# phcavelar/graph-odenet

Hardware: AMD Instinct MI355X
Metric: full-graph ODE-GCN forward+backward steps/sec at 64 RK4 evals (higher is better)
Workload: dtype f32; 1 GPU; RMAT scale-20 / 10000000 edges (+self loops, dedup) row-normalised, d=128, ODEGCN3 rk4(3/8) 16 steps = 64 f-evals fwd, adjoint bwd, Adam; one graph per GPU; nodes=1048576, nnz=10758918, nfeat=128, hidden=128, nclass=16, parallelism=dp1 (one graph per rank, 1 gradient all-reduce/step)

## Files before the change

### graph_odenet_amd/_lib.py

```python
import ctypes
import os

import torch

_HERE = os.path.dirname(os.path.abspath(__file__))
LIB_PATH = os.path.join(_HERE, "libgraphode.so")

GODE_MAX_TERMS = 8


class LinComb(ctypes.Structure):
    _fields_ = [("n", ctypes.c_int32),
                ("coef", ctypes.c_float * GODE_MAX_TERMS),
                ("ptr", ctypes.c_void_p * GODE_MAX_TERMS)]


class SpmmEpilogue(ctypes.Structure):
    _fields_ = [("bias", ctypes.c_void_p), ("relu", ctypes.c_int32), ("alpha", ctypes.c_float),
                ("pre", LinComb), ("cot", LinComb), ("Y2", ctypes.c_void_p), ("Y2_colsum", ctypes.c_void_p),
                ("cot_out", ctypes.c_void_p), ("cot_out_coef", ctypes.c_float * GODE_MAX_TERMS)]


class Graph(ctypes.Structure):
    _fields_ = [("rowptr", ctypes.c_void_p), ("col", ctypes.c_void_p), ("val", ctypes.c_void_p),
                ("items", ctypes.c_void_p), ("n_items", ctypes.c_int64),
                ("long_rows", ctypes.c_void_p), ("n_long", ctypes.c_int64), ("partial", ctypes.c_void_p),
                ("n_rows", ctypes.c_int64), ("nnz", ctypes.c_int64)]


class GcnOdeFunc(ctypes.Structure):
    _fields_ = [("A", Graph), ("AT", Graph), ("n", ctypes.c_int64), ("d", ctypes.c_int64),
                ("groups", ctypes.c_int32), ("eps", ctypes.c_float),
                ("W", ctypes.c_void_p), ("b", ctypes.c_void_p), ("gamma", ctypes.c_void_p), ("beta", ctypes.c_void_p)]


class GatProj(ctypes.Structure):
    _fields_ = [("ps", ctypes.c_void_p), ("ld_s", ctypes.c_int64), ("pt", ctypes.c_void_p), ("ld_t", ctypes.c_int64),
                ("as_", ctypes.c_void_p), ("at", ctypes.c_void_p), ("ld_a", ctypes.c_int64)]


class Rk4Workspace(ctypes.Structure):
    _fields_ = [("S", ctypes.c_void_p), ("dZ", ctypes.c_void_p), ("dS", ctypes.c_void_p), ("S2", ctypes.c_void_p),
                ("ky", ctypes.c_void_p * 4), ("ka", ctypes.c_void_p * 4), ("ktheta", ctypes.c_void_p * 4),
                ("wpart", ctypes.c_void_p), ("gpart", ctypes.c_void_p), ("bpart", ctypes.c_void_p),
                ("colsum_scratch", ctypes.c_void_p), ("X", ctypes.c_void_p * 2), ("small_part", ctypes.c_void_p),
                ("y2_colsum", ctypes.c_void_p)]


class ReduceSeg(ctypes.Structure):
    _fields_ = [("out", ctypes.c_void_p), ("part", ctypes.c_void_p), ("n_part", ctypes.c_int64), ("ld", ctypes.c_int64),
                ("col0", ctypes.c_int64), ("col_stride", ctypes.c_int64), ("len", ctypes.c_int64),
                ("w_row0", ctypes.c_void_p), ("time_len", ctypes.c_int64)]


class GatOdeFunc(ctypes.Structure):
    _fields_ = [("mt", Graph), ("ms_inc", Graph), ("mt_inc", Graph), ("src", ctypes.c_void_p), ("tgt", ctypes.c_void_p),
                ("n_edges", ctypes.c_int64), ("n", ctypes.c_int64), ("d", ctypes.c_int64), ("groups", ctypes.c_int32),
                ("eps_gn", ctypes.c_float), ("eps", ctypes.c_float), ("Wsrc", ctypes.c_void_p), ("Wtgt", ctypes.c_void_p),
                ("Wlog", ctypes.c_void_p), ("bf", ctypes.c_void_p), ("bw", ctypes.c_void_p), ("gamma", ctypes.c_void_p),
                ("beta", ctypes.c_void_p), ("heads", ctypes.c_int32), ("Wpacked", ctypes.c_void_p)]


class GatWorkspace(ctypes.Structure):
    _fields_ = [(k, ctypes.c_void_p) for k in ("X", "Ps", "Pt", "A2", "a", "amax", "wgt", "den", "logits_scratch", "dz", "da",
                                               "dPs", "dPt", "dA2", "pair", "gp", "bp")] + \
               [("wp", ctypes.c_void_p * 3), ("maxpath_scratch", ctypes.c_void_p), ("colsum_scratch", ctypes.c_void_p),
                ("zeros", ctypes.c_void_p), ("heads_scratch", ctypes.c_void_p), ("colsum_scratch2", ctypes.c_void_p),
                ("small_part", ctypes.c_void_p)]


GODE_ADAM_MAX_TENSORS = 64


class AdamArgs(ctypes.Structure):
    _fields_ = [("param", ctypes.c_void_p * GODE_ADAM_MAX_TENSORS), ("grad", ctypes.c_void_p * GODE_ADAM_MAX_TENSORS),
                ("exp_avg", ctypes.c_void_p * GODE_ADAM_MAX_TENSORS), ("exp_avg_sq", ctypes.c_void_p * GODE_ADAM_MAX_TENSORS),
                ("len", ctypes.c_int64 * GODE_ADAM_MAX_TENSORS)]


c_i64 = ctypes.c_int64
c_p = ctypes.c_void_p
c_f = ctypes.c_float
c_i = ctypes.c_int

SIGNATURES = {
    "gode_abi_version": (c_i, []),
    "gode_error_string": (ctypes.c_char_p, [c_i]),
    "gode_set_option": (c_i, [ctypes.c_char_p, c_i]),
    "gode_get_option": (c_i, [ctypes.c_char_p]),
    "gode_spmm_csr_f32": (c_i, [c_p, c_p, c_p, c_p, c_i64, c_p, c_i64, c_p, c_p, c_i64, c_p, c_i64,
                                c_i64, c_i64, ctypes.POINTER(SpmmEpilogue), c_p]),
    "gode_spmm_csr_save_f32": (c_i, [c_p, c_p, c_p, c_p, c_i64, c_p, c_i64, c_p, c_p, c_i64, c_p, c_i64,
                                     c_i64, c_i64, ctypes.POINTER(SpmmEpilogue), c_p, c_p]),
    "gode_masked_cot_parts": (c_i64, [c_i64, c_i64]),
    "gode_masked_cot_f32": (c_i, [ctypes.POINTER(LinComb), c_p, c_p, c_i64, c_i64, c_p, c_p]),
    "gode_lincomb_f32": (c_i, [c_p, ctypes.POINTER(LinComb), c_i64, c_p]),
    "gode_lincomb_multi_f32": (c_i, [c_p, c_p, c_p, ctypes.c_int32, c_p]),
    "gode_rk_errnorm_multi_f32": (c_i, [c_p, c_p, c_p, c_p, c_p, ctypes.c_int32, c_f, c_f, c_p, c_p]),
    "gode_rk_errnorm_scratch_bytes": (c_i64, []),
    "gode_rk_errnorm_f32": (c_i, [c_p, c_p, c_p, ctypes.POINTER(LinComb), c_f, c_f, c_i64, c_p, c_p]),
    "gode_rk_scaled_sumsq_f32": (c_i, [c_p, ctypes.POINTER(LinComb), c_p, c_f, c_f, c_i64, c_p, c_p]),
    "gode_gn_time_gemm_f32": (c_i, [ctypes.POINTER(LinComb), c_i64, c_i64, ctypes.c_int32, c_f, c_p, c_p,
                                    c_p, c_i64, c_i, c_f, c_p, c_p]),
    "gode_gn_time_gemm_xout_f32": (c_i, [ctypes.POINTER(LinComb), c_i64, c_i64, ctypes.c_int32, c_f, c_p, c_p,
                                         c_p, c_i64, c_i, c_f, c_p, c_p, c_p]),
    "gode_gn_time_gemm_xout_aux_f32": (c_i, [ctypes.POINTER(LinComb), c_i64, c_i64, ctypes.c_int32, c_f, c_p, c_p,
                                             c_p, c_i64, c_i, c_f, c_p, c_p, c_p, c_p, c_p]),
    "gode_gn_time_gemm_pair_f32": (c_i, [ctypes.POINTER(LinComb), c_i64, c_i64, ctypes.c_int32, c_f, c_p, c_p, c_p, c_p,
                                         c_i, c_f, c_p, c_p, c_p, c_p]),
    "gode_gemm_bwd_parts": (c_i64, [c_i64]),
    "gode_gn_time_gemm_bwd_f32": (c_i, [ctypes.POINTER(LinComb), c_i64, c_i64, ctypes.c_int32, c_f, c_p,
                                        c_p, c_i64, c_i, c_p, c_f, ctypes.POINTER(LinComb), c_p, c_p, c_p, c_p]),
    "gode_bwd_wgrad_supported": (c_i, [c_i64, c_i64, c_i64, ctypes.c_int32]),
    "gode_bwd_wgrad_parts": (c_i64, [c_i64]),
    "gode_gn_time_gemm_bwd_wgrad_f32": (c_i, [ctypes.POINTER(LinComb), c_i64, c_i64, ctypes.c_int32, c_f, c_p, c_p, c_p, c_i64, c_i,
                                              c_p, c_f, ctypes.POINTER(LinComb), c_p, c_p, c_p, c_p, c_p]),
    "gode_group_norm_parts": (c_i64, [c_i64]),
    "gode_group_norm_f32_fwd": (c_i, [c_p, c_i64, c_i64, ctypes.c_int32, c_f, c_p, c_p, c_p, c_p]),
    "gode_group_norm_f32_bwd": (c_i, [c_p, c_i64, c_i64, ctypes.c_int32, c_f, c_p, c_p, c_p, c_p, c_p, c_p]),
    "gode_rect_gemm_f32": (c_i, [c_p, c_i64, c_i64, c_i64, c_p, c_i64, c_p, c_i64, c_p]),
    "gode_rect_gemm_nt_f32": (c_i, [c_p, c_i64, c_i64, c_i64, c_p, c_i64, c_p, c_i64, c_p]),
    "gode_rect_wgrad_parts": (c_i64, [c_i64]),
    "gode_rect_wgrad_f32": (c_i, [c_p, c_i64, c_i64, c_i64, c_p, c_i64, c_i64, c_p, c_p]),
    "gode_rect_wgrad_sum_f32": (c_i, [c_p, c_i64, c_i64, c_i64, c_p, c_i64, c_i64, c_p, c_p, c_p]),
    "gode_gemm_f32": (c_i, [c_i, c_i, c_i64, c_i64, c_i64, c_p, c_i64, c_p, c_i64, c_p, c_i64, c_p, c_i, c_p, c_i64, c_p]),
    "gode_gemm_splitk_parts": (c_i64, [c_i64, c_i64, c_i64]),
    "gode_gemm_splitk_f32": (c_i, [c_i, c_i, c_i64, c_i64, c_i64, c_p, c_i64, c_p, c_i64, c_p, c_p, c_p]),
    "gode_cut_pad": (c_i64, [c_i64]),
    "gode_cut_bf16x3_f32": (c_i, [c_p, c_i64, c_i64, c_i64, c_p, c_p]),
    "gode_pgemm_workspace_bytes": (c_i64, [c_i64, c_i64, c_i64]),
    "gode_pgemm_bf16x3": (c_i, [c_i, c_i, c_i64, c_i64, c_i64, c_p, c_p, c_p, c_i64, c_p, c_i, c_p, c_i64, c_i, c_p, c_p]),
    "gode_adam_chunk": (c_i64, []),
    "gode_adam_tick_f32": (c_i, [c_p, c_f, c_f, c_p]),
    "gode_adam_f32": (c_i, [ctypes.POINTER(AdamArgs), ctypes.c_int32, c_p, c_i64, c_p, c_f, c_f, c_f, c_f, c_f, c_p]),
    "gode_gat_small_supported": (c_i, [c_i64, c_i64, ctypes.c_int32, c_i64]),
    "gode_gat_small_parts": (c_i64, [c_i64, c_i64]),
    "gode_gat_small_part_len": (c_i64, [c_i64, c_i64]),
    "gode_gat_project_small_f32": (c_i, [ctypes.POINTER(LinComb), c_i64, c_i64, ctypes.c_int32, c_f, c_p, c_p, c_p, c_p, c_p,
                                         c_i64, c_p, c_f, c_p, c_p, c_p, c_p, c_p, c_p]),
    "gode_gat_small_pack_len": (c_i64, [c_i64, c_i64]),
    "gode_gat_small_pack_f32": (c_i, [c_p, c_p, c_p, c_i64, c_i64, c_p, c_p]),
    "gode_gat_dense_vjp_small_f32": (c_i, [ctypes.POINTER(LinComb), c_i64, c_i64, ctypes.c_int32, c_f, c_p, c_p, c_p, c_p, c_p,
                                           c_i64, c_p, c_p, c_p, c_f, ctypes.POINTER(LinComb), c_p, c_p, c_p, c_p, c_p, c_i64, c_p, c_p]),
    "gode_gat_maxpath_heads_part_f32": (c_i, [c_p, c_p, c_i64, c_i64, c_p, c_p, c_p]),
    "gode_gat_heads_block_cap": (c_i64, []),
    "gode_gat_small_finish_f32": (c_i, [c_p, c_i64, c_i64, c_i64, c_f, c_p, c_p, c_p]),
    "gode_gat_small_finish_step_f32": (c_i, [c_p, c_i64, c_i64, c_i64, ctypes.c_int32, c_p, c_p, c_p, c_p, c_p]),
    "gode_gcn_small_supported": (c_i, [c_i64, c_i64, ctypes.c_int32]),
    "gode_gcn_small_parts": (c_i64, [c_i64]),
    "gode_gcn_small_part_len": (c_i64, [c_i64]),
    "gode_gcn_feval_small_f32": (c_i, [ctypes.POINTER(GcnOdeFunc), ctypes.POINTER(LinComb), c_f, c_f, ctypes.POINTER(LinComb),
                                       ctypes.POINTER(LinComb), c_p, c_p, c_p]),
    "gode_gcn_feval_small_next_f32": (c_i, [ctypes.POINTER(GcnOdeFunc), ctypes.POINTER(LinComb), c_f, c_f, ctypes.POINTER(LinComb),
                                            ctypes.POINTER(LinComb), c_p, c_p, ctypes.POINTER(LinComb), c_p, c_p]),
    "gode_gcn_vjp_small_f32": (c_i, [ctypes.POINTER(GcnOdeFunc), ctypes.POINTER(LinComb), c_p, c_f, ctypes.POINTER(LinComb),
                                     c_p, c_p, c_p]),
    "gode_gcn_vjp_small_next_f32": (c_i, [ctypes.POINTER(GcnOdeFunc), ctypes.POINTER(LinComb), c_p, c_f, ctypes.POINTER(LinComb),
                                          c_p, c_p, ctypes.POINTER(LinComb), c_p, c_p, c_p]),
    "gode_gcn_feval_small_save_f32": (c_i, [ctypes.POINTER(GcnOdeFunc), ctypes.POINTER(LinComb), c_f, c_f,
                                            ctypes.POINTER(LinComb), c_p, c_p, c_p]),
    "gode_gcn_small_finish_f32": (c_i, [ctypes.POINTER(GcnOdeFunc), c_p, c_p, c_f, c_p]),
    "gode_gcn_small_finish_multi_f32": (c_i, [ctypes.POINTER(GcnOdeFunc), c_p, ctypes.c_int32, ctypes.POINTER(c_p), ctypes.POINTER(c_f), c_p]),
    "gode_gcn_small_finish4_f32": (c_i, [ctypes.POINTER(GcnOdeFunc), c_p, c_p, c_p, c_p, c_p]),
    "gode_wgrad_parts": (c_i64, [c_i64]),
    "gode_wgrad_f32": (c_i, [ctypes.POINTER(LinComb), c_i64, c_i64, ctypes.c_int32, c_f, c_p, c_p,
                             c_p, c_i64, c_i, c_p, c_p]),
    "gode_reduce_parts_f32": (c_i, [c_p, c_p, c_i64, c_i64, c_f, c_i, c_p]),
    "gode_reduce_parts2_f32": (c_i, [c_p, c_p, c_p, c_p, c_i64, c_i64, c_f, c_i, c_p]),
    "gode_reduce_segments_f32": (c_i, [ctypes.POINTER(ReduceSeg), ctypes.c_int32, c_f, c_p, c_p]),
    "gode_colsum_parts_f32": (c_i, [c_p, c_i64, c_i64, c_p, ctypes.POINTER(c_i64), c_p]),
    "gode_colsum_scratch_bytes": (c_i64, [c_i64, c_i64]),
    "gode_spmm_y2_colsum_rows": (c_i64, [c_i64, c_i64, c_i64]),
    "gode_colsum_f32": (c_i, [c_p, c_p, c_i64, c_i64, c_f, c_i, c_p, c_p]),
    "gode_gat_logits_scratch_bytes": (c_i64, [c_i64]),
    "gode_gat_logits_f32": (c_i, [ctypes.POINTER(GatProj), c_p, c_p, c_p, c_i64, c_p, c_p, c_p, c_p]),
    "gode_gat_agg_f32_fwd": (c_i, [ctypes.POINTER(Graph), c_p, c_p, ctypes.POINTER(GatProj), c_i64, c_p, c_p, c_p, c_f,
                                   c_p, c_p, c_p, c_p]),
    "gode_gat_agg_f32_bwd": (c_i, [ctypes.POINTER(Graph), c_p, c_p, ctypes.POINTER(GatProj), c_i64, c_p, c_p, c_p, c_p,
                                   c_p, ctypes.POINTER(LinComb), c_f, c_p, c_p, c_p, c_i64, c_p, c_i64,
                                   ctypes.POINTER(ctypes.c_int32), c_p]),
    "gode_gat_maxpath_scratch_bytes": (c_i64, [c_i64]),
    "gode_gat_maxpath_f32": (c_i, [c_p, c_p, c_p, c_i64, c_p, c_p, c_i64, c_p, c_p]),
    "gode_gat_heads_scratch_bytes": (c_i64, [c_i64, c_i64]),
    "gode_gat_logits_heads_f32": (c_i, [ctypes.POINTER(GatProj), c_p, c_p, c_p, c_i64, c_i64, c_p, c_p, c_p, c_p]),
    "gode_gat_maxpath_heads_f32": (c_i, [c_p, c_p, c_i64, c_i64, c_p, c_p, c_i64, c_p, c_p]),
    "gode_gat_heads_parts": (c_i64, [c_i64]),
    "gode_gat_logits_heads_raw_f32": (c_i, [ctypes.POINTER(GatProj), c_p, c_p, c_p, c_i64, c_i64, c_p, c_p, c_p]),
    "gode_gat_agg_heads_f32_fwd": (c_i, [ctypes.POINTER(Graph), c_p, c_p, ctypes.POINTER(GatProj), c_i64, c_p, c_p, c_p, c_i64,
                                         c_i64, c_f, c_p, c_p, c_p, c_p]),
    "gode_gat_maxpath_heads_raw_f32": (c_i, [c_p, c_p, c_i64, c_i64, c_p, c_p, c_i64, c_p, c_p]),
    "gode_gat_scatter_f32": (c_i, [c_p, c_p, c_p, c_p, c_p, c_p, c_i64, c_i64, c_p, c_i64, c_p, c_i64, c_p, c_p, c_i64,
                                   c_p]),
    "gode_time_row_fixup_f32": (c_i, [c_p, c_p, c_i64, c_f, c_p, c_i, c_p]),
    "gode_time_row_fixup3_f32": (c_i, [c_p, c_p, c_i64, c_p, c_p, c_i64, c_p, c_p, c_i64, c_f, c_p, c_p]),
    "gode_edge_matvec_f32_fwd": (c_i, [c_p, c_p, c_p, c_p, c_p, c_p, c_i64, c_i64, c_i64, c_p, c_i64, c_p]),
    "gode_edge_matvec_msg_f32": (c_i, [c_p, c_p, c_p, c_i64, c_i64, c_i64, c_p, c_p]),
    "gode_edge_matvec_f32_bwd": (c_i, [c_p, c_p, c_p, c_p, c_p, c_i64, c_p, c_i64, c_i64, c_i64, c_p, c_p, c_p]),
    "gode_edge_outer_sum_f32": (c_i, [c_p, c_p, c_p, ctypes.c_int32, ctypes.POINTER(c_p), ctypes.POINTER(c_p), c_i64, c_i64, c_i64, c_i64, c_p, c_p]),
    "gode_edge_ode_supported": (c_i, [c_i64]),
    "gode_edge_ode_feval_f32": (c_i, [c_p, c_p, c_p, c_p, c_p, c_p, c_i64, c_i64, c_p, ctypes.POINTER(LinComb), c_f, c_p, c_p]),
    "gode_edge_ode_vjp_f32": (c_i, [c_p, c_p, c_p, c_p, c_p, ctypes.POINTER(LinComb), c_f, c_p, c_i64, c_i64, c_i64, c_p, c_p,
                                    c_p, c_p]),
    "gode_edge_outer_sum_acc_f32": (c_i, [c_p, c_p, c_p, ctypes.c_int32, ctypes.POINTER(c_p), ctypes.POINTER(c_p),
                                          ctypes.POINTER(c_f), c_i64, c_i64, c_i, c_p, c_p]),
    "gode_segment_attention_f32_fwd": (c_i, [c_p, c_p, c_p, c_i64, c_p, c_i64, c_i64, c_p, c_p, c_p]),
    "gode_segment_attention_f32_bwd": (c_i, [c_p, c_p, c_p, c_i64, c_p, c_p, c_p, c_i64, c_i64, c_p, c_p, c_p]),
    "gode_assign_csr_supported": (c_i, [c_i64, c_i64]),
    "gode_dense_first_nonzero_f32": (c_i, [c_p, c_i64, c_i64, c_i64, c_p, c_p]),
    "gode_assign_csr_i32": (c_i, [c_p, c_i64, c_i64, c_p, c_p, c_p, c_p, c_p]),
    "gode_set2set_supported": (c_i, [c_i64]),
    "gode_set2set_f32_fwd": (c_i, [c_p, c_p, c_p, c_i64, c_p, c_p, c_p, c_i64, c_i64, c_i64, c_i64, c_p, c_p, c_p, c_p, c_p]),
    "gode_set2set_f32_bwd": (c_i, [c_p, c_p, c_p, c_i64, c_p, c_p, c_i64, c_i64, c_i64, c_i64, c_p, c_p, c_p, c_p, c_p, c_p,
                                   c_p, c_p]),
    "gode_gcn_ode_theta_len": (c_i64, [c_i64]),
    "gode_gcn_ode_rk4_forward": (c_i, [ctypes.POINTER(GcnOdeFunc), c_p, ctypes.POINTER(c_p), ctypes.POINTER(Rk4Workspace),
                                       c_f, c_f, ctypes.c_int32, c_p]),
    "gode_gcn_ode_rk4_adjoint": (c_i, [ctypes.POINTER(GcnOdeFunc), c_p, c_p, c_p, ctypes.POINTER(c_p), ctypes.POINTER(c_p),
                                       ctypes.POINTER(Rk4Workspace), c_f, c_f, ctypes.c_int32, c_p]),
    "gode_gcn_ode_rk4_forward_save": (c_i, [ctypes.POINTER(GcnOdeFunc), c_p, c_p, c_p, ctypes.POINTER(Rk4Workspace),
                                            c_f, c_f, ctypes.c_int32, ctypes.c_int32, ctypes.c_int32, c_p]),
    "gode_gcn_ode_rk4_backprop": (c_i, [ctypes.POINTER(GcnOdeFunc), c_p, c_p, c_p, ctypes.POINTER(c_p),
                                        ctypes.POINTER(Rk4Workspace), c_p, c_f, c_f, ctypes.c_int32, ctypes.c_int32,
                                        ctypes.c_int32, c_p]),
    "gode_gcn_ode_dopri5_step_forward": (c_i, [ctypes.POINTER(GcnOdeFunc), c_p, ctypes.POINTER(c_p), c_p,
                                               ctypes.POINTER(Rk4Workspace), ctypes.c_double, ctypes.c_double, c_f, c_f,
                                               c_p, c_p, c_p]),
    "gode_gcn_ode_dopri5_step_adjoint": (c_i, [ctypes.POINTER(GcnOdeFunc), c_p, c_p, c_p, ctypes.POINTER(c_p),
                                               ctypes.POINTER(c_p), ctypes.POINTER(c_p), c_p, c_p, c_p,
                                               ctypes.POINTER(Rk4Workspace), ctypes.c_double, ctypes.c_double, c_f, c_f,
                                               c_p, c_p, c_p]),
    "gode_gcn_ode_dopri5_step_backprop": (c_i, [ctypes.POINTER(GcnOdeFunc), c_p, ctypes.POINTER(c_p), c_p, c_p,
                                                ctypes.c_double, ctypes.POINTER(ctypes.c_double), ctypes.c_double,
                                                ctypes.c_double, ctypes.c_int32, ctypes.POINTER(c_p), c_p, c_p, c_p,
                                                ctypes.POINTER(c_p), ctypes.POINTER(Rk4Workspace), c_p, c_p]),
    "gode_gat_ode_theta_len": (c_i64, [c_i64]),
    "gode_gat_ode_theta_len_heads": (c_i64, [c_i64, c_i64]),
    "gode_gat_ode_dopri5_step_forward": (c_i, [ctypes.POINTER(GatOdeFunc), c_p, ctypes.POINTER(c_p), c_p,
                                               ctypes.POINTER(GatWorkspace), ctypes.c_double, ctypes.c_double, c_f, c_f,
                                               c_p, c_p, c_p]),
    "gode_gat_ode_dopri5_step_adjoint": (c_i, [ctypes.POINTER(GatOdeFunc), c_p, c_p, c_p, c_p, ctypes.POINTER(c_p),
                                               ctypes.POINTER(c_p), ctypes.POINTER(c_p), ctypes.POINTER(c_p), c_p, c_p, c_p,
                                               c_p, ctypes.POINTER(GatWorkspace), ctypes.c_double, ctypes.c_double, c_f,
                                               c_f, c_p, c_p, c_p]),
    "gode_lstm_cell_supported": (c_i, [c_i64, c_i64, c_i64]),
    "gode_lstm_cell_f32_fwd": (c_i, [c_p] * 7 + [c_i64] * 3 + [c_p] * 4),
    "gode_lstm_cell_f32_bwd": (c_i, [c_p] * 9 + [c_i64] * 3 + [c_p] * 8),
    "gode_gru_wgrad_parts": (c_i64, [c_i64]),
    "gode_gru_cell_f32_fwd": (c_i, [c_p, c_p, c_p, c_p, c_p, c_p, c_i64, c_i64, c_p, c_p, c_p]),
    "gode_gru_cell_f32_bwd": (c_i, [c_p, c_p, c_p, c_p, c_p, c_p, c_i64, c_i64, c_p, c_p, c_p, c_p, c_p, c_p, c_p, c_p, c_p,
                                    c_p]),
    "gode_gru_wreduce_f32": (c_i, [c_p, c_i64, c_i64, c_p, c_p, c_p, c_p, c_p]),
    "gode_prof_create": (c_p, [c_i]),
    "gode_prof_destroy": (None, [c_p]),
    "gode_prof_enable": (None, [c_p]),
    "gode_prof_reset": (None, [c_p]),
    "gode_prof_count": (c_i, [c_p]),
    "gode_prof_read": (c_i, [c_p, c_p, c_p, c_p, c_p, c_i]),
    "gode_prof_kinds": (c_i, [c_p, c_p, c_i]),
}

_lib = None


class GraphodeLibraryError(RuntimeError):
    pass


def load():
    global _lib
    if _lib is not None:
        return _lib
    if not os.path.exists(LIB_PATH):
        raise GraphodeLibraryError(
            "libgraphode.so not found at %s - build it with `python __graft_entry__.py` "
            "(or `make -C graph_odenet_amd/csrc`). There is no fallback path." % LIB_PATH)
    lib = ctypes.CDLL(LIB_PATH)
    for name, (res, args) in SIGNATURES.items():
        fn = getattr(lib, name)
        fn.restype = res
        fn.argtypes = args
    if lib.gode_abi_version() != 1:
        raise GraphodeLibraryError("libgraphode.so ABI version mismatch")
    _lib = lib
    return lib


def check(rc, what):
    if rc != 0:
        msg = load().gode_error_string(rc)
        raise RuntimeError("%s failed: %s (code %d)" % (what, msg.decode() if msg else "?", rc))


def lincomb(terms):
    lc = LinComb()
    terms = [(c, t) for (c, t) in terms if t is not None]
    if len(terms) > GODE_MAX_TERMS:
        raise ValueError("too many lincomb terms")
    lc.n = len(terms)
    for j, (c, t) in enumerate(terms):
        lc.coef[j] = float(c)
        lc.ptr[j] = t.data_ptr()
    return lc


_raw_stream = getattr(torch._C, "_cuda_getCurrentRawStream", None)


def current_stream_handle(device_index=None):
    if _raw_stream is not None:
        return _raw_stream(torch.cuda.current_device() if device_index is None else device_index)
    return torch.cuda.current_stream(device_index).cuda_stream


def stream_ptr():
    return ctypes.c_void_p(current_stream_handle())


def ptr(t):
    return ctypes.c_void_p(t.data_ptr()) if t is not None else None
```

### graph_odenet_amd/csrc/api.hip

```cpp
#include "common.h"

extern "C" int gode_abi_version(void) { return GODE_ABI_VERSION; }

extern "C" const char* gode_error_string(int code) {
    switch (code) {
        case 0: return "success";
        case GODE_E_NULLPTR: return "graphode: required pointer is NULL";
        case GODE_E_SHAPE: return "graphode: invalid shape / leading dimension";
        case GODE_E_ALIGN: return "graphode: operand not 16-byte aligned";
        case GODE_E_RANGE: return "graphode: argument out of range";
        case GODE_E_UNSUPPORTED: return "graphode: unsupported configuration";
        default: break;
    }
    if (code > 0) return hipGetErrorString((hipError_t)code);
    return "graphode: unknown error";
}

#include "options.h"
#include <cstdlib>
#include <cstring>

namespace {
int env_int(const char* name, int dflt) { const char* e = getenv(name); return e ? atoi(e) : dflt; }
int g_gemm_split = -1, g_overlap = -1, g_wgrad_split = -1, g_wgrad_split_small = 0, g_bwd_pc = -1, g_fwd_pc = -1, g_small_fused = -1, g_bwd_wgrad = -1, g_y2_colsum = -1, g_rk_close_once = -1;
}

int gode_opt_gemm_split() { if (g_gemm_split < 0) { const int v = env_int("GODE_GEMM_SPLIT", 2); g_gemm_split = (v == 1 || v == 2) ? v : 0; } return g_gemm_split; }
int gode_opt_wgrad_split() {
    if (g_wgrad_split < 0) { const int v = env_int("GODE_WGRAD_SPLIT", 8); g_wgrad_split = (v == 6 || v == 8) ? v : 0; }
    return g_wgrad_split;
}
int gode_opt_wgrad_split_small() { return g_wgrad_split_small; }
int gode_opt_bwd_pc() { if (g_bwd_pc < 0) g_bwd_pc = env_int("GODE_BWD_PC", 1) != 0; return g_bwd_pc; }
int gode_opt_fwd_pc() { if (g_fwd_pc < 0) g_fwd_pc = env_int("GODE_FWD_PC", 3) & 3; return g_fwd_pc; }
int gode_opt_small_fused() { if (g_small_fused < 0) g_small_fused = env_int("GODE_SMALL_FUSED", 1) != 0; return g_small_fused; }
int gode_opt_bwd_wgrad() { if (g_bwd_wgrad < 0) g_bwd_wgrad = env_int("GODE_BWD_WGRAD", 1) != 0; return g_bwd_wgrad; }
int gode_opt_y2_colsum() { if (g_y2_colsum < 0) g_y2_colsum = env_int("GODE_Y2_COLSUM", 1) != 0; return g_y2_colsum; }
int gode_opt_rk_close_once() { if (g_rk_close_once < 0) g_rk_close_once = env_int("GODE_RK_CLOSE_ONCE", 1) != 0; return g_rk_close_once; }
int gode_opt_overlap() { if (g_overlap < 0) g_overlap = env_int("GODE_OVERLAP", 1) != 0; return g_overlap; }

extern "C" int gode_set_option(const char* name, int value) {
    if (!name) return GODE_E_NULLPTR;
    if (!strcmp(name, "gemm_split")) { if (value < 0 || value > 2) return GODE_E_UNSUPPORTED; g_gemm_split = value; return 0; }
    if (!strcmp(name, "overlap")) { g_overlap = value != 0; return 0; }
    if (!strcmp(name, "wgrad_split_small")) { g_wgrad_split_small = value != 0; return 0; }
    if (!strcmp(name, "bwd_pc")) { g_bwd_pc = value != 0; return 0; }
    if (!strcmp(name, "small_fused")) { g_small_fused = value != 0; return 0; }
    if (!strcmp(name, "bwd_wgrad")) { g_bwd_wgrad = value != 0; return 0; }
    if (!strcmp(name, "y2_colsum")) { g_y2_colsum = value != 0; return 0; }
    if (!strcmp(name, "rk_close_once")) { g_rk_close_once = value != 0; return 0; }
    if (!strcmp(name, "fwd_pc")) { if (value < 0 || value > 3) return GODE_E_UNSUPPORTED; g_fwd_pc = value; return 0; }
    if (!strcmp(name, "wgrad_split")) { if (value != 0 && value != 6 && value != 8) return GODE_E_UNSUPPORTED; g_wgrad_split = value; return 0; }
    return GODE_E_UNSUPPORTED;
}
extern "C" int gode_get_option(const char* name) {
    if (!name) return GODE_E_NULLPTR;
    if (!strcmp(name, "gemm_split")) return gode_opt_gemm_split();
    if (!strcmp(name, "overlap")) return gode_opt_overlap();
    if (!strcmp(name, "wgrad_split")) return gode_opt_wgrad_split();
    if (!strcmp(name, "wgrad_split_small")) return gode_opt_wgrad_split_small();
    if (!strcmp(name, "bwd_pc")) return gode_opt_bwd_pc();
    if (!strcmp(name, "small_fused")) return gode_opt_small_fused();
    if (!strcmp(name, "bwd_wgrad")) return gode_opt_bwd_wgrad();
    if (!strcmp(name, "y2_colsum")) return gode_opt_y2_colsum();
    if (!strcmp(name, "rk_close_once")) return gode_opt_rk_close_once();
    if (!strcmp(name, "fwd_pc")) return gode_opt_fwd_pc();
    return GODE_E_UNSUPPORTED;
}
```

### graph_odenet_amd/csrc/ode_driver.hip

```cpp
#include <map>
#include <mutex>
#include <utility>
#include "rk_driver.h"
#include "options.h"

namespace {

int spmm(const gode_graph_t& g, const float* X, float* Y, int64_t d, const gode_spmm_epilogue_t* ep, void* s) {
    return gode_spmm_csr_f32(g.rowptr, g.col, g.val, g.items, g.n_items, g.long_rows, g.n_long, g.partial,
                             X, d, Y, d, g.n_rows, d, ep, s);
}
gode_spmm_epilogue_t relu_bias_epilogue(const gode_gcn_odefunc_t* f) {
    gode_spmm_epilogue_t ep = {};
    ep.bias = f->b; ep.relu = 1; ep.alpha = 1.f;
    return ep;
}

__global__ void theta_fixup_kernel(float* ktheta, const float* W, float t, int d, int64_t off_at) {
    __shared__ float sm[4];
    float s = 0.f;
    for (int c = threadIdx.x; c < d; c += blockDim.x) s += ktheta[c] * W[c];
    s = wave_sum(s);
    if ((threadIdx.x & 63) == 0) sm[threadIdx.x >> 6] = s;
    __syncthreads();
    if (threadIdx.x == 0) ktheta[off_at] = sm[0] + sm[1] + sm[2] + sm[3];
    __syncthreads();
    for (int c = threadIdx.x; c < d; c += blockDim.x) ktheta[c] *= t;
}

int close_bias(const gode_gcn_odefunc_t* f, const gode_rk4_workspace_t* ws, float* kt, const float* src, int64_t rows,
               void* stream) {
    return gode_colsum_f32(kt + (f->d + 1) * f->d, src, rows, f->d, 1.f, 0, ws->colsum_scratch, stream);
}
int close_weight(const gode_gcn_odefunc_t* f, const gode_rk4_workspace_t* ws, float* kt, int64_t parts, float ts,
                 void* stream) {
    const int64_t d = f->d;
    GODE_TRY(gode_reduce_parts_f32(kt, ws->wpart, parts, (d + 1) * d, 1.f, 0, stream));
    hipLaunchKernelGGL(theta_fixup_kernel, dim3(1), dim3(256), 0, (hipStream_t)stream, kt, f->W, ts, (int)d,
                       gode_gcn_ode_theta_len(d) - 1);
    GODE_LAUNCH_CHECK();
    return 0;
}
int close_affine(const gode_gcn_odefunc_t* f, const gode_rk4_workspace_t* ws, float* kt, void* stream) {
    const int64_t d = f->d;
    float* kg = kt + (d + 1) * d + d;
    if (f->groups <= 0) return gode_zero_f32(kg, 2 * d, stream);
    return gode_reduce_parts2_f32(kg, ws->gpart, kg + d, ws->bpart, gode_gemm_bwd_parts(f->n), d, 1.f, 0, stream);
}

int stage_finish_merged(const gode_gcn_odefunc_t* f, const gode_rk4_workspace_t* ws, float* kt, float ts, void* stream) {
    const int64_t n = f->n, d = f->d, nW = (d + 1) * d, P = gode_gcn_ode_theta_len(d);
    int64_t cparts = 0;
    GODE_TRY(gode_colsum_parts_f32(ws->dZ, n, d, (float*)ws->colsum_scratch, &cparts, stream));
    const int64_t gp = gode_gemm_bwd_parts(n);
    gode_reduce_seg_t sg[4] = {};
    sg[0] = {kt, ws->wpart, gode_wgrad_parts(n), nW, 0, 1, nW, f->W, d};
    sg[1] = {kt + nW, (const float*)ws->colsum_scratch, cparts, d, 0, 1, d, nullptr, 0};
    sg[2] = {kt + nW + d, ws->gpart, gp, d, 0, 1, d, nullptr, 0};
    sg[3] = {kt + nW + 2 * d, ws->bpart, gp, d, 0, 1, d, nullptr, 0};
    GODE_TRY(gode_reduce_segments_f32(sg, f->groups > 0 ? 4 : 2, ts, kt + (P - 1), stream));
    if (f->groups <= 0) GODE_TRY(gode_zero_f32(kt + nW + d, 2 * d, stream));
    return 0;
}

bool fused_small(const gode_gcn_odefunc_t* f) {
    return gode_opt_small_fused() && gode_gcn_small_supported(f->n, f->d, f->groups);
}

bool close_once_route(const gode_gcn_odefunc_t* f) {
    return gode_opt_rk_close_once() && !fused_small(f) && f->n > kMergedFinishMaxRows && f->d == 128;
}

int gf_last_stage(const gode_gcn_odefunc_t* f, const gode_lincomb_t& xin, const gode_lincomb_t& pre, float t, float* S,
                  float* x_out, float* p_out, bool* formed, void* stream) {
    *formed = false;
    bool distinct = p_out != S && p_out != x_out;
    for (int j = 0; j < xin.n; ++j) distinct = distinct && p_out != xin.ptr[j];
    if (distinct && xin.n == pre.n) {
        const int rc = gode_gn_time_gemm_xout_aux_f32(&xin, f->n, f->d, f->groups, f->eps, f->gamma, f->beta, f->W, f->d, 1, t, S,
                                                      x_out, pre.coef, p_out, stream);
        if (rc != GODE_E_UNSUPPORTED) { *formed = rc == 0; return rc; }
    }
    return gode_gn_time_gemm_xout_f32(&xin, f->n, f->d, f->groups, f->eps, f->gamma, f->beta, f->W, f->d, 1, t, S, x_out, stream);
}

struct StepClose { gode_lincomb_t pre; float alpha; bool once; };

int feval_large(const gode_gcn_odefunc_t* f, const gode_lincomb_t& xin, float t, float* S, float* out,
                const StepClose* close, float* k_save, void* stream) {
    const int64_t d = f->d;
    bool p_formed = false;
    if (close && close->once) {
        GODE_TRY(gf_last_stage(f, xin, close->pre, t, S, nullptr, out, &p_formed, stream));
    } else {
        GODE_TRY(gode_gn_time_gemm_f32(&xin, f->n, d, f->groups, f->eps, f->gamma, f->beta, f->W, d, 1, t, S, stream));
    }
    gode_spmm_epilogue_t ep = relu_bias_epilogue(f);
    if (close) { ep.pre = p_formed ? one_term(out) : close->pre; ep.alpha = close->alpha; }
    if (!k_save) return spmm(f->A, S, out, d, &ep, stream);
    const gode_graph_t& g = f->A;
    return gode_spmm_csr_save_f32(g.rowptr, g.col, g.val, g.items, g.n_items, g.long_rows, g.n_long, g.partial,
                                  S, d, out, d, g.n_rows, d, &ep, k_save, stream);
}

int rk4_forward_step(const gode_gcn_odefunc_t* f, const gode_rk4_workspace_t* ws, const float* y, float* const* k,
                     float* ynext, bool keep_k4, double t, double h, bool fused, bool close_once, void* stream) {
    for (int s = 0; s < 4; ++s) {
        const gode_lincomb_t xin = stage_terms(y, k, s, h);
        const float ts = (float)(t + C38[s] * h);
        if (s < 3) {
            if (fused) GODE_TRY(gode_gcn_feval_small_f32(f, &xin, ts, 1.f, nullptr, nullptr, nullptr, k[s], stream));
            else GODE_TRY(feval_large(f, xin, ts, ws->S, k[s], nullptr, nullptr, stream));
            continue;
        }
        const StepClose close = {combine_terms(y, k, h), (float)(h * B38[3]), close_once};
        if (!fused) GODE_TRY(feval_large(f, xin, ts, ws->S, ynext, &close, keep_k4 ? k[3] : nullptr, stream));
        else if (keep_k4) GODE_TRY(gode_gcn_feval_small_save_f32(f, &xin, ts, close.alpha, &close.pre, ynext, k[3], stream));
        else GODE_TRY(gode_gcn_feval_small_f32(f, &xin, ts, close.alpha, &close.pre, nullptr, nullptr, ynext, stream));
    }
    return 0;
}

}

extern "C" int64_t gode_gcn_ode_theta_len(int64_t d) { return (d + 1) * d + 3 * d + 1; }

extern "C" int gode_gcn_ode_rk4_forward(const gode_gcn_odefunc_t* f, float* y, float** result,
                                        const gode_rk4_workspace_t* ws, float t0, float t1, int32_t n_steps,
                                        void* stream)
{
    if (!f || !y || !ws || !result) return GODE_E_NULLPTR;
    if (n_steps <= 0 || f->n <= 0 || f->d <= 0) return GODE_E_SHAPE;
    if (!ws->S || !ws->ky[0] || !ws->ky[1] || !ws->ky[2] || !ws->ky[3]) return GODE_E_NULLPTR;
    const double h = ((double)t1 - (double)t0) / n_steps;
    float* cur = y;
    float* k[4] = {ws->ky[0], ws->ky[1], ws->ky[2], ws->ky[3]};
    const bool fused = fused_small(f);
    const bool close_once = close_once_route(f);
    for (int i = 0; i < n_steps; ++i) {
        GODE_TRY(rk4_forward_step(f, ws, cur, k, k[3], false, (double)t0 + i * h, h, fused, close_once, stream));
        float* tmp = cur; cur = k[3]; k[3] = tmp;
    }
    *result = cur;
    return 0;
}

namespace {

struct Overlap {
    hipStream_t side = nullptr;
    hipEvent_t sp = nullptr, gf = nullptr, spt = nullptr, wg = nullptr;
    bool ok = false;
};
Overlap* overlap_ctx(hipStream_t caller) {
    static std::mutex mu;
    static std::map<std::pair<int, hipStream_t>, Overlap*> ctxs;
    int dev = 0;
    if (hipGetDevice(&dev) != hipSuccess) return nullptr;
    std::lock_guard<std::mutex> lk(mu);
    auto key = std::make_pair(dev, caller);
    auto it = ctxs.find(key);
    if (it != ctxs.end()) return it->second;
    Overlap* c = new Overlap();
    if (hipStreamCreateWithFlags(&c->side, hipStreamNonBlocking) == hipSuccess) {
        bool ok = true;
        for (hipEvent_t* ev : {&c->sp, &c->gf, &c->spt, &c->wg})
            ok = ok && hipEventCreateWithFlags(ev, hipEventDisableTiming) == hipSuccess;
        c->ok = ok;
    }
    ctxs[key] = c;
    return c;
}

int rk4_adjoint_small(const gode_gcn_odefunc_t* f, const gode_rk4_workspace_t* ws, float* y, float* a, float* theta,
                      float** y_result, float** a_result, float t0, double h, int32_t n_steps, void* stream) {
    float* ycur = y; float* acur = a;
    float* ky[4] = {ws->ky[0], ws->ky[1], ws->ky[2], ws->ky[3]};
    float* ka[4] = {ws->ka[0], ws->ka[1], ws->ka[2], ws->ka[3]};
    const int64_t slot = gode_gcn_small_parts(f->n) * gode_gcn_small_part_len(f->d);
    const float hb3 = (float)(h * B38[3]);
    for (int i = 0; i < n_steps; ++i) {
        float stage_t[4];
        const gode_lincomb_t ypre = combine_terms(ycur, ky, h), apre = combine_terms(acur, ka, h);
        for (int s = 0; s < 4; ++s) {
            stage_t[s] = (float)((double)t0 + i * h + C38[s] * h);
            const gode_lincomb_t yin = stage_terms(ycur, ky, s, h);
            const gode_lincomb_t cot = negated(stage_terms(acur, ka, s, h));
            GODE_TRY(gode_gcn_feval_small_f32(f, &yin, stage_t[s], s == 3 ? hb3 : 1.f, s == 3 ? &ypre : nullptr,
                                              &cot, ws->dZ, ky[s], stream));
            GODE_TRY(gode_gcn_vjp_small_f32(f, &yin, ws->dZ, s == 3 ? hb3 : 1.f, s == 3 ? &apre : nullptr,
                                            ka[s], ws->small_part + s * slot, stream));
        }
        const float wb[4] = {(float)(h * B38[0]), (float)(h * B38[1]), (float)(h * B38[2]), hb3};
        GODE_TRY(gode_gcn_small_finish4_f32(f, ws->small_part, theta, wb, stage_t, stream));
        float* tmp = ycur; ycur = ky[3]; ky[3] = tmp;
        tmp = acur; acur = ka[3]; ka[3] = tmp;
    }
    *y_result = ycur;
    *a_result = acur;
    return 0;
}

}

extern "C" int gode_gcn_ode_rk4_adjoint(const gode_gcn_odefunc_t* f, float* y, float* a, float* theta,
                                        float** y_result, float** a_result,
                                        const gode_rk4_workspace_t* ws, float t0, float t1, int32_t n_steps,
                                        void* stream)
{
    if (!f || !y || !a || !theta || !ws || !y_result || !a_result) return GODE_E_NULLPTR;
    if (n_steps <= 0 || f->n <= 0 || f->d <= 0) return GODE_E_SHAPE;
    for (int s = 0; s < 4; ++s) if (!ws->ky[s] || !ws->ka[s] || !ws->ktheta[s]) return GODE_E_NULLPTR;
    if (!ws->S || !ws->dZ || !ws->dS || !ws->wpart || !ws->colsum_scratch) return GODE_E_NULLPTR;
    if (f->groups > 0 && (!ws->gpart || !ws->bpart)) return GODE_E_NULLPTR;
    const int64_t n = f->n, d = f->d;
    const double h = ((double)t1 - (double)t0) / n_steps;
    if (fused_small(f) && ws->small_part != nullptr)
        return rk4_adjoint_small(f, ws, y, a, theta, y_result, a_result, t0, h, n_steps, stream);
    hipStream_t hs = (hipStream_t)stream;
    const bool small = f->n <= kMergedFinishMaxRows;
    Overlap* ov = (!small && ws->S2 != nullptr && gode_opt_overlap()) ? overlap_ctx(hs) : nullptr;
    const bool two = ov != nullptr && ov->ok;
    void* side = two ? (void*)ov->side : stream;
    float* Sbuf[2] = {ws->S, two ? ws->S2 : ws->S};
    float* ycur = y; float* acur = a;
    float* ky[4] = {ws->ky[0], ws->ky[1], ws->ky[2], ws->ky[3]};
    float* ka[4] = {ws->ka[0], ws->ka[1], ws->ka[2], ws->ka[3]};
    const int64_t wparts = gode_wgrad_parts(n);
    const int total = 4 * n_steps;
    const bool bw = !small && gode_bwd_wgrad_supported(n, d, d, f->groups) && gode_bwd_wgrad_parts(n) <= wparts;
    const int64_t y2rows = (bw && ws->y2_colsum && gode_opt_y2_colsum())
        ? gode_spmm_y2_colsum_rows(f->A.items ? f->A.n_items : f->A.n_rows, f->A.items ? f->A.n_long : 0, d) : 0;

    const bool mat = ws->X[0] != nullptr && ws->X[1] != nullptr;
    auto x_out_of = [&](int g) -> float* { return (mat && (g % 4) >= 2) ? ws->X[g & 1] : nullptr; };
    auto stage_time = [&](int g) { return (float)((double)t0 + (g / 4) * h + C38[g % 4] * h); };

    const bool close_once = bw && close_once_route(f);
    bool py_formed = false;
    auto gf = [&](int g, void* st) -> int {
        const gode_lincomb_t yin = stage_terms(ycur, ky, g % 4, h);
        if (g % 4 == 3 && close_once)
            return gf_last_stage(f, yin, combine_terms(ycur, ky, h), stage_time(g), Sbuf[g & 1], x_out_of(g), ky[3], &py_formed, st);
        return gode_gn_time_gemm_xout_f32(&yin, n, d, f->groups, f->eps, f->gamma, f->beta, f->W, d, 1, stage_time(g),
                                          Sbuf[g & 1], x_out_of(g), st);
    };
    GODE_TRY(gf(0, stream));
    bool wg_pending = false;
    for (int g = 0; g < total; ++g) {
        const int s = g % 4;
        const float ts = stage_time(g);
        const gode_lincomb_t yin = x_out_of(g) ? one_term(x_out_of(g)) : stage_terms(ycur, ky, s, h);
        const gode_lincomb_t ain = stage_terms(acur, ka, s, h);
        gode_spmm_epilogue_t ep = relu_bias_epilogue(f);
        ep.cot = negated(ain);
        ep.Y2 = ws->dZ;
        if (y2rows > 0) ep.Y2_colsum = ws->y2_colsum;
        gode_lincomb_t apre; apre.n = 0;
        if (s == 3) {
            ep.pre = py_formed ? one_term(ky[3]) : combine_terms(ycur, ky, h);
            ep.alpha = (float)(h * B38[3]);
            apre = combine_terms(acur, ka, h);
            if (close_once && ain.n == apre.n) {
                ep.cot_out = ka[3];
                for (int j = 0; j < apre.n; ++j) ep.cot_out_coef[j] = apre.coef[j];
                apre = one_term(ka[3]);
            }
            py_formed = false;
        }
        if (two && g > 0) GODE_HIP(hipStreamWaitEvent(hs, ov->gf, 0));
        GODE_TRY(spmm(f->A, Sbuf[g & 1], ky[s], d, &ep, stream));
        if (s == 3) { float* tmp = ycur; ycur = ky[3]; ky[3] = tmp; }
        if (two && wg_pending) GODE_HIP(hipStreamWaitEvent(hs, ov->wg, 0));
        GODE_TRY(spmm(f->AT, ws->dZ, ws->dS, d, nullptr, stream));
        if (two) {
            GODE_HIP(hipEventRecord(ov->spt, hs));
            GODE_HIP(hipStreamWaitEvent(ov->side, ov->spt, 0));
        }
        float* kt = ws->ktheta[s];
        const float out_scale = s == 3 ? (float)(h * B38[3]) : 1.f;
        float* gpart = f->groups > 0 ? ws->gpart : nullptr;
        float* bpart = f->groups > 0 ? ws->bpart : nullptr;
        if (bw) {
            if (two) GODE_HIP(hipStreamWaitEvent(ov->side, ov->spt, 0));
            GODE_TRY(close_bias(f, ws, kt, y2rows > 0 ? ws->y2_colsum : ws->dZ, y2rows > 0 ? y2rows : n, side));
            GODE_TRY(gode_gn_time_gemm_bwd_wgrad_f32(&yin, n, d, f->groups, f->eps, f->gamma, f->beta, f->W, d, 1, ws->dS,
                                                     out_scale, s == 3 ? &apre : nullptr, ka[s], gpart, bpart, ws->wpart, stream));
            if (two) {
                GODE_HIP(hipEventRecord(ov->sp, hs));
                GODE_HIP(hipStreamWaitEvent(ov->side, ov->sp, 0));
            }
            GODE_TRY(close_weight(f, ws, kt, gode_bwd_wgrad_parts(n), ts, side));
            GODE_TRY(close_affine(f, ws, kt, side));
            if (two) { GODE_HIP(hipEventRecord(ov->wg, ov->side)); wg_pending = true; }
            if (g + 1 < total) {
                GODE_TRY(gf(g + 1, stream));
                if (two) GODE_HIP(hipEventRecord(ov->gf, hs));
            }
            if (two) { GODE_HIP(hipStreamWaitEvent(hs, ov->wg, 0)); wg_pending = false; }
        } else {
            GODE_TRY(gode_wgrad_f32(&yin, n, d, f->groups, f->eps, f->gamma, f->beta, ws->dS, d, 1, ws->wpart, side));
            if (!small) GODE_TRY(close_weight(f, ws, kt, wparts, ts, side));
            if (two) { GODE_HIP(hipEventRecord(ov->wg, ov->side)); wg_pending = true; }
            if (g + 1 < total) {
                GODE_TRY(gf(g + 1, side));
                if (two) GODE_HIP(hipEventRecord(ov->gf, ov->side));
            }
            GODE_TRY(gode_gn_time_gemm_bwd_f32(&yin, n, d, f->groups, f->eps, f->gamma, f->W, d, 1, ws->dS, out_scale,
                                               s == 3 ? &apre : nullptr, ka[s], gpart, bpart, stream));
            if (small) {
                GODE_TRY(stage_finish_merged(f, ws, kt, ts, stream));
            } else {
                GODE_TRY(close_bias(f, ws, kt, ws->dZ, n, stream));
                GODE_TRY(close_affine(f, ws, kt, stream));
            }
        }
        if (s == 3) {
            if (two) { GODE_HIP(hipStreamWaitEvent(hs, ov->wg, 0)); wg_pending = false; }
            gode_lincomb_t tc = one_term(theta);
            tc.n = 5;
            for (int q = 0; q < 4; ++q) { tc.coef[1 + q] = (float)(h * B38[q]); tc.ptr[1 + q] = ws->ktheta[q]; }
            GODE_TRY(gode_lincomb_f32(theta, &tc, gode_gcn_ode_theta_len(d), stream));
            float* tmp = acur; acur = ka[3]; ka[3] = tmp;
        }
    }
    if (two) {
        GODE_HIP(hipEventRecord(ov->gf, ov->side));
        GODE_HIP(hipStreamWaitEvent(hs, ov->gf, 0));
    }
    *y_result = ycur;
    *a_result = acur;
    return 0;
}

namespace {

int dp_eval_forward(const gode_gcn_odefunc_t* f, const gode_rk4_workspace_t* ws, const gode_lincomb_t* yin, float t,
                    float* k_out, const gode_lincomb_t* next, float* x_next, void* stream) {
    if (fused_small(f)) return gode_gcn_feval_small_next_f32(f, yin, t, 1.f, nullptr, nullptr, nullptr, k_out, next, x_next, stream);
    return feval_large(f, *yin, t, ws->S, k_out, nullptr, nullptr, stream);
}

int dp_eval_adjoint(const gode_gcn_odefunc_t* f, const gode_rk4_workspace_t* ws, gode_lincomb_t yin,
                    const gode_lincomb_t& ain, float t, float* ky, float* ka, float* kth, const gode_lincomb_t* next,
                    float* x_next, int part_slot, void* stream) {
    const int64_t n = f->n, d = f->d;
    if (fused_small(f) && ws->small_part) {
        const gode_lincomb_t cot = negated(ain);
        GODE_TRY(gode_gcn_feval_small_next_f32(f, &yin, t, 1.f, nullptr, &cot, ws->dZ, ky, next, x_next, stream));
        float* part = ws->small_part + (part_slot > 0 ? part_slot : 0) * gode_gcn_small_parts(n) * gode_gcn_small_part_len(d);
        GODE_TRY(gode_gcn_vjp_small_f32(f, &yin, ws->dZ, 1.f, nullptr, ka, part, stream));
        if (part_slot >= 0) return 0;
        return gode_gcn_small_finish_f32(f, part, kth, t, stream);
    }
    float* xo = (yin.n >= 3 && ws->X[0]) ? ws->X[0] : nullptr;
    GODE_TRY(gode_gn_time_gemm_xout_f32(&yin, n, d, f->groups, f->eps, f->gamma, f->beta, f->W, d, 1, t, ws->S, xo, stream));
    if (xo) yin = one_term(xo);
    gode_spmm_epilogue_t ep = relu_bias_epilogue(f);
    ep.cot = negated(ain);
    ep.Y2 = ws->dZ;
    GODE_TRY(spmm(f->A, ws->S, ky, d, &ep, stream));
    GODE_TRY(spmm(f->AT, ws->dZ, ws->dS, d, nullptr, stream));
    GODE_TRY(gode_gn_time_gemm_bwd_f32(&yin, n, d, f->groups, f->eps, f->gamma, f->W, d, 1, ws->dS, 1.f, nullptr, ka,
                                       f->groups > 0 ? ws->gpart : nullptr, f->groups > 0 ? ws->bpart : nullptr, stream));
    GODE_TRY(gode_wgrad_f32(&yin, n, d, f->groups, f->eps, f->gamma, f->beta, ws->dS, d, 1, ws->wpart, stream));
    if (n <= kMergedFinishMaxRows) return stage_finish_merged(f, ws, kth, t, stream);
    GODE_TRY(close_weight(f, ws, kth, gode_wgrad_parts(n), t, stream));
    GODE_TRY(close_bias(f, ws, kth, ws->dZ, n, stream));
    return close_affine(f, ws, kth, stream);
}

}

extern "C" int gode_gcn_ode_dopri5_step_forward(const gode_gcn_odefunc_t* f, const float* y, float* const* k, float* y1,
                                                const gode_rk4_workspace_t* ws, double t, double h, float rtol,
                                                float atol, double* sums, void* err_scratch, void* stream)
{
    if (!f || !y || !k || !y1 || !ws || !sums || !err_scratch) return GODE_E_NULLPTR;
    if (f->n <= 0 || f->d <= 0) return GODE_E_SHAPE;
    for (int s = 0; s < 7; ++s) if (!k[s]) return GODE_E_NULLPTR;
    if (!ws->S) return GODE_E_NULLPTR;
    const int64_t nd = f->n * f->d;
    const bool chain = fused_small(f) && ws->X[0] && ws->X[1];
    for (int s = 1; s < 7; ++s) {
        gode_lincomb_t yin = dp_terms(y, k, DPA[s], s, h, true);
        if (chain && s >= 2) yin = one_term(ws->X[s & 1]);
        gode_lincomb_t nxt; nxt.n = 0;
        if (chain && s < 6) nxt = dp_terms(y, k, DPA[s + 1], s + 1, h, true);
        GODE_TRY(dp_eval_forward(f, ws, &yin, (float)(t + DPC[s] * h), k[s], nxt.n > 0 ? &nxt : nullptr,
                                 nxt.n > 0 ? ws->X[(s + 1) & 1] : nullptr, stream));
    }
    gode_lincomb_t sol = dp_terms(y, k, DPB, 7, h, true);
    GODE_TRY(gode_lincomb_f32(y1, &sol, nd, stream));
    gode_lincomb_t err = dp_terms(nullptr, k, DPE, 7, h, false);
    return gode_rk_errnorm_f32(sums, y, y1, &err, rtol, atol, nd, err_scratch, stream);
}

extern "C" int gode_gcn_ode_dopri5_step_adjoint(const gode_gcn_odefunc_t* f, const float* y, const float* a,
                                                const float* theta, float* const* ky, float* const* ka,
                                                float* const* kth, float* y1, float* a1, float* theta1,
                                                const gode_rk4_workspace_t* ws, double t, double h, float rtol,
                                                float atol, double* sums , void* err_scratch, void* stream)
{
    if (!f || !y || !a || !theta || !ky || !ka || !kth || !y1 || !a1 || !theta1 || !ws || !sums || !err_scratch)
        return GODE_E_NULLPTR;
    if (f->n <= 0 || f->d <= 0) return GODE_E_SHAPE;
    for (int s = 0; s < 7; ++s) if (!ky[s] || !ka[s] || !kth[s]) return GODE_E_NULLPTR;
    if (!ws->S || !ws->dZ || !ws->dS || !ws->wpart || !ws->colsum_scratch) return GODE_E_NULLPTR;
    if (f->groups > 0 && (!ws->gpart || !ws->bpart)) return GODE_E_NULLPTR;
    const int64_t nd = f->n * f->d, P = gode_gcn_ode_theta_len(f->d);
    const bool fused = fused_small(f) && ws->small_part;
    const bool chain = fused && ws->X[0] && ws->X[1];
    for (int s = 1; s < 7; ++s) {
        gode_lincomb_t yin = dp_terms(y, ky, DPA[s], s, h, true);
        if (chain && s >= 2) yin = one_term(ws->X[s & 1]);
        gode_lincomb_t ain = dp_terms(a, ka, DPA[s], s, h, true);
        gode_lincomb_t nxt; nxt.n = 0;
        if (chain && s < 6) nxt = dp_terms(y, ky, DPA[s + 1], s + 1, h, true);
        GODE_TRY(dp_eval_adjoint(f, ws, yin, ain, (float)(t + DPC[s] * h), ky[s], ka[s], kth[s], nxt.n > 0 ? &nxt : nullptr,
                                 nxt.n > 0 ? ws->X[(s + 1) & 1] : nullptr, fused ? s - 1 : -1, stream));
    }
    if (fused) {
        float* kout[6]; float tsv[6];
        for (int s = 1; s < 7; ++s) { kout[s - 1] = kth[s]; tsv[s - 1] = (float)(t + DPC[s] * h); }
        GODE_TRY(gode_gcn_small_finish_multi_f32(f, ws->small_part, 6, kout, tsv, stream));
    }
    gode_lincomb_t sy = dp_terms(y, ky, DPB, 7, h, true), sa = dp_terms(a, ka, DPB, 7, h, true),
                   st = dp_terms(theta, kth, DPB, 7, h, true);
    {
        float* outs[3] = {y1, a1, theta1};
        const gode_lincomb_t sols[3] = {sy, sa, st};
        const int64_t lens[3] = {nd, nd, P};
        GODE_TRY(gode_lincomb_multi_f32(outs, sols, lens, 3, stream));
    }
    const gode_lincomb_t errs[4] = {dp_terms(nullptr, ky, DPE, 7, h, false), dp_terms(nullptr, ka, DPE, 7, h, false),
                                    dp_terms(nullptr, kth, DPE, 7, h, false, P - 1), dp_terms(nullptr, kth, DPE, 7, h, false)};
    const float* e0[4] = {y, a, theta + (P - 1), theta};
    const float* e1[4] = {y1, a1, theta1 + (P - 1), theta1};
    const int64_t ens[4] = {nd, nd, 1, P - 1};
    return gode_rk_errnorm_multi_f32(sums, e0, e1, errs, ens, 4, rtol, atol, err_scratch, stream);
}

namespace {

struct SweepRoute {
    bool small;
    bool bw;
    int64_t wparts, cparts;
    float* cot_colpart;
    float* gpart; float* bpart;
};
SweepRoute sweep_route(const gode_gcn_odefunc_t* f, const gode_rk4_workspace_t* ws, float* cot_colpart) {
    SweepRoute r;
    r.small = f->n <= kMergedFinishMaxRows;
    r.wparts = gode_wgrad_parts(f->n);
    r.bw = !r.small && gode_bwd_wgrad_supported(f->n, f->d, f->d, f->groups) && gode_bwd_wgrad_parts(f->n) <= r.wparts;
    r.cparts = (!r.small && cot_colpart) ? gode_masked_cot_parts(f->n, f->d) : 0;
    r.cot_colpart = cot_colpart;
    r.gpart = f->groups > 0 ? ws->gpart : nullptr;
    r.bpart = f->groups > 0 ? ws->bpart : nullptr;
    return r;
}

int sweep_stage(const gode_gcn_odefunc_t* f, const gode_rk4_workspace_t* ws, const SweepRoute& r, const gode_lincomb_t& cot,
                const float* k, const gode_lincomb_t& yin, const gode_lincomb_t* pre, float* ybar, float* kt, float ts,
                void* stream) {
    const int64_t n = f->n, d = f->d;
    GODE_TRY(gode_masked_cot_f32(&cot, k, ws->dZ, n, d, r.cparts > 0 ? r.cot_colpart : nullptr, stream));
    GODE_TRY(spmm(f->AT, ws->dZ, ws->dS, d, nullptr, stream));
    if (r.bw) {
        GODE_TRY(gode_gn_time_gemm_bwd_wgrad_f32(&yin, n, d, f->groups, f->eps, f->gamma, f->beta, f->W, d, 1, ws->dS,
                                                 1.f, pre, ybar, r.gpart, r.bpart, ws->wpart, stream));
    } else {
        GODE_TRY(gode_gn_time_gemm_bwd_f32(&yin, n, d, f->groups, f->eps, f->gamma, f->W, d, 1, ws->dS, 1.f,
                                           pre, ybar, r.gpart, r.bpart, stream));
        GODE_TRY(gode_wgrad_f32(&yin, n, d, f->groups, f->eps, f->gamma, f->beta, ws->dS, d, 1, ws->wpart, stream));
        if (r.small) return stage_finish_merged(f, ws, kt, ts, stream);
    }
    GODE_TRY(close_weight(f, ws, kt, r.bw ? gode_bwd_wgrad_parts(n) : r.wparts, ts, stream));
    GODE_TRY(close_bias(f, ws, kt, r.cparts > 0 ? r.cot_colpart : ws->dZ, r.cparts > 0 ? r.cparts : n, stream));
    return close_affine(f, ws, kt, stream);
}

int add_stage_parts(float* theta, float* const* kt, int count, int64_t len, void* stream) {
    gode_lincomb_t tc = one_term(theta);
    for (int q = 0; q < count; ++q) { tc.coef[tc.n] = 1.f; tc.ptr[tc.n] = kt[q]; ++tc.n; }
    return gode_lincomb_f32(theta, &tc, len, stream);
}

}

extern "C" int gode_gcn_ode_rk4_forward_save(const gode_gcn_odefunc_t* f, const float* y0, float* y_end, float* save,
                                             const gode_rk4_workspace_t* ws, float t0, float t1, int32_t n_steps,
                                             int32_t step_begin, int32_t step_end, void* stream)
{
    if (!f || !y0 || !y_end || !save || !ws) return GODE_E_NULLPTR;
    if (n_steps <= 0 || f->n <= 0 || f->d <= 0) return GODE_E_SHAPE;
    if (step_begin < 0 || step_end > n_steps || step_begin >= step_end) return GODE_E_SHAPE;
    if (!ws->S) return GODE_E_NULLPTR;
    const int64_t nd = f->n * f->d;
    const double h = ((double)t1 - (double)t0) / n_steps;
    const bool fused = fused_small(f);
    const bool close_once = close_once_route(f);
    if (y0 != save) {
        const gode_lincomb_t c = one_term(y0);
        GODE_TRY(gode_lincomb_f32(save, &c, nd, stream));
    }
    for (int i = step_begin; i < step_end; ++i) {
        float* rec = save + (int64_t)(i - step_begin) * 5 * nd;
        float* k[4] = {rec + nd, rec + 2 * nd, rec + 3 * nd, rec + 4 * nd};
        float* ynext = (i + 1 < step_end) ? rec + 5 * nd : y_end;
        GODE_TRY(rk4_forward_step(f, ws, rec, k, ynext, true, (double)t0 + i * h, h, fused, close_once, stream));
    }
    return 0;
}

extern "C" int gode_gcn_ode_rk4_backprop(const gode_gcn_odefunc_t* f, const float* save, float* a, float* theta,
                                         float** a_result, const gode_rk4_workspace_t* ws, float* cot_colpart,
                                         float t0, float t1, int32_t n_steps, int32_t step_begin, int32_t step_end,
                                         void* stream)
{
    if (!f || !save || !a || !theta || !a_result || !ws) return GODE_E_NULLPTR;
    if (n_steps <= 0 || f->n <= 0 || f->d <= 0) return GODE_E_SHAPE;
    if (step_begin < 0 || step_end > n_steps || step_begin >= step_end) return GODE_E_SHAPE;
    for (int s = 0; s < 4; ++s) if (!ws->ka[s] || !ws->ktheta[s]) return GODE_E_NULLPTR;
    if (!ws->dZ || !ws->dS || !ws->wpart || !ws->colsum_scratch) return GODE_E_NULLPTR;
    if (f->groups > 0 && (!ws->gpart || !ws->bpart)) return GODE_E_NULLPTR;
    const int64_t n = f->n, d = f->d, nd = n * d;
    const double h = ((double)t1 - (double)t0) / n_steps;
    float* acur = a;
    float* yb[4] = {ws->ka[0], ws->ka[1], ws->ka[2], ws->ka[3]};
    auto record = [&](int i) { return save + (int64_t)(i - step_begin) * 5 * nd; };
    const bool fused = fused_small(f) && ws->small_part != nullptr;
    if (fused) {
        const int64_t slot = gode_gcn_small_parts(n) * gode_gcn_small_part_len(d);
// ... 119 lines not shown
```

### graph_odenet_amd/csrc/options.h

```cpp
#pragma once
int gode_opt_gemm_split();
int gode_opt_overlap();
int gode_opt_wgrad_split();
int gode_opt_wgrad_split_small();
int gode_opt_bwd_pc();
int gode_opt_fwd_pc();
int gode_opt_small_fused();
int gode_opt_bwd_wgrad();
int gode_opt_y2_colsum();
int gode_opt_rk_close_once();
```

### graph_odenet_amd/csrc/prof.h

```cpp
#pragma once
#include <hip/hip_runtime.h>
#include <stdint.h>
int  gode_prof_begin(hipStream_t s, int64_t d, int64_t rows, int64_t extra, int kind = 0);
void gode_prof_end(hipStream_t s, int slot);
```

### graph_odenet_amd/csrc/prof.hip

```cpp
#include "common.h"
#include "prof.h"
#include <vector>

struct GodeProf {
    int capacity;
    int count;
    std::vector<hipEvent_t> ev;
    std::vector<int64_t> d, rows, extra;
    std::vector<int32_t> kind;
};

static GodeProf* volatile g_prof = nullptr;

extern "C" void* gode_prof_create(int capacity) {
    if (capacity <= 0) return nullptr;
    GodeProf* p = new GodeProf();
    p->capacity = capacity; p->count = 0;
    p->ev.resize(2 * (size_t)capacity); p->d.resize(capacity); p->rows.resize(capacity); p->extra.resize(capacity); p->kind.resize(capacity);
    for (auto& e : p->ev) if (hipEventCreate(&e) != hipSuccess) { delete p; return nullptr; }
    return p;
}
extern "C" void gode_prof_destroy(void* prof) {
    GodeProf* p = (GodeProf*)prof;
    if (!p) return;
    if (g_prof == p) g_prof = nullptr;
    for (auto& e : p->ev) (void)hipEventDestroy(e);
    delete p;
}
extern "C" void gode_prof_enable(void* prof) { g_prof = (GodeProf*)prof; }
extern "C" void gode_prof_reset(void* prof) { if (prof) ((GodeProf*)prof)->count = 0; }
extern "C" int gode_prof_count(void* prof) { return prof ? ((GodeProf*)prof)->count : 0; }

extern "C" int gode_prof_read(void* prof, float* ms, int64_t* d, int64_t* rows, int64_t* extra, int max_n) {
    GodeProf* p = (GodeProf*)prof;
    if (!p || !ms) return GODE_E_NULLPTR;
    int n = p->count < max_n ? p->count : max_n;
    for (int i = 0; i < n; ++i) {
        hipError_t e = hipEventSynchronize(p->ev[2 * i + 1]);
        if (e != hipSuccess) return (int)e;
        e = hipEventElapsedTime(&ms[i], p->ev[2 * i], p->ev[2 * i + 1]);
        if (e != hipSuccess) return (int)e;
        if (d) d[i] = p->d[i];
        if (rows) rows[i] = p->rows[i];
        if (extra) extra[i] = p->extra[i];
    }
    return n;
}

extern "C" int gode_prof_kinds(void* prof, int32_t* kinds, int max_n) {
    GodeProf* p = (GodeProf*)prof;
    if (!p || !kinds) return GODE_E_NULLPTR;
    const int n = p->count < max_n ? p->count : max_n;
    for (int i = 0; i < n; ++i) kinds[i] = p->kind[i];
    return n;
}

int gode_prof_begin(hipStream_t s, int64_t d, int64_t rows, int64_t extra, int kind) {
    GodeProf* p = g_prof;
    if (!p || p->count >= p->capacity) return -1;
    hipStreamCaptureStatus cs = hipStreamCaptureStatusNone;
    if (hipStreamIsCapturing(s, &cs) != hipSuccess || cs != hipStreamCaptureStatusNone) return -1;
    const int i = p->count;
    p->d[i] = d; p->rows[i] = rows; p->extra[i] = extra; p->kind[i] = kind;
    (void)hipEventRecord(p->ev[2 * i], s);
    return i;
}
void gode_prof_end(hipStream_t s, int slot) {
    GodeProf* p = g_prof;
    if (!p || slot < 0) return;
    (void)hipEventRecord(p->ev[2 * slot + 1], s);
    p->count = slot + 1;
}
```

### graph_odenet_amd/csrc/spmm.hip

```cpp
#include "common.h"
#include "prof.h"

namespace {

struct Epilogue {
    const float* bias;
    int relu;
    float alpha;
    LinComb pre;
    LinComb cot;
    float* Y2;
    float* colpart;
    int64_t colpart_row0;
    float* K;
    float* Y3;
    float c3[GODE_MAX_TERMS];
};

template <int LPR, bool OUT3 = false>
__device__ __forceinline__ float4 epilogue_store4(const Epilogue& ep, float4 z, int row, int lane,
                                                  int64_t d, float* Y, int64_t ldy) {
    if (ep.bias) {
        const float4 b = *reinterpret_cast<const float4*>(ep.bias + lane * 4);
        z.x += b.x; z.y += b.y; z.z += b.z; z.w += b.w;
    }
    float4 y = z;
    if (ep.relu) { y.x = fmaxf(z.x, 0.f); y.y = fmaxf(z.y, 0.f); y.z = fmaxf(z.z, 0.f); y.w = fmaxf(z.w, 0.f); }
    if (ep.K) *reinterpret_cast<float4*>(ep.K + (int64_t)row * d + lane * 4) = y;
    if (ep.pre.n > 0) {
        const float4 p = lc_load4(ep.pre, (int64_t)row * d + lane * 4);
        y.x = fmaf(ep.alpha, y.x, p.x); y.y = fmaf(ep.alpha, y.y, p.y);
        y.z = fmaf(ep.alpha, y.z, p.z); y.w = fmaf(ep.alpha, y.w, p.w);
    } else if (ep.alpha != 1.f) {
        y.x *= ep.alpha; y.y *= ep.alpha; y.z *= ep.alpha; y.w *= ep.alpha;
    }
    *reinterpret_cast<float4*>(Y + (int64_t)row * ldy + lane * 4) = y;
    if (ep.Y2) {
        const int64_t o = (int64_t)row * d + lane * 4;
        float4 g;
        if (OUT3) {
            float4 g3;
            lc_load4_pair(ep.cot, ep.c3, o, g, g3);
            *reinterpret_cast<float4*>(ep.Y3 + o) = g3;
        } else {
            g = lc_load4(ep.cot, o);
        }
        g.x = z.x > 0.f ? g.x : 0.f; g.y = z.y > 0.f ? g.y : 0.f;
        g.z = z.z > 0.f ? g.z : 0.f; g.w = z.w > 0.f ? g.w : 0.f;
        *reinterpret_cast<float4*>(ep.Y2 + o) = g;
        return g;
    }
    return make_float4(0.f, 0.f, 0.f, 0.f);
}

template <int LPR>
__device__ __forceinline__ void block_colsum_store(const float4 g, float* __restrict__ colpart_row) {
    __shared__ float4 cs[256];
    cs[threadIdx.x] = g;
    __syncthreads();
    if (threadIdx.x < LPR) {
        float4 t = cs[threadIdx.x];
#pragma unroll
        for (int r = 1; r < 256 / LPR; ++r) {
            const float4 a = cs[r * LPR + threadIdx.x];
            t.x += a.x; t.y += a.y; t.z += a.z; t.w += a.w;
        }
        *reinterpret_cast<float4*>(colpart_row + 4 * threadIdx.x) = t;
    }
}

template <int LPR, bool OUT3 = false>
__global__ __launch_bounds__(256) void spmm_vec4_kernel(
    const int* __restrict__ rowptr, const int* __restrict__ col, const float* __restrict__ val,
    const int4* __restrict__ items, int n_items, float* __restrict__ partial,
    const float* __restrict__ X, int64_t ldx, float* __restrict__ Y, int64_t ldy, Epilogue ep)
{
    constexpr int U = 4;
    const int64_t tid = (int64_t)blockIdx.x * blockDim.x + threadIdx.x;
    const int gid = (int)(tid / LPR);
    const int lane = threadIdx.x & (LPR - 1);
    const bool active = gid < n_items;
    int row = 0, b = 0, e = 0, slot = -1;
    if (active) {
        if (items) { const int4 it = items[gid]; row = it.x; b = it.y; e = it.z; slot = it.w; }
        else { row = gid; b = rowptr[gid]; e = rowptr[gid + 1]; }
    }
    const int len = e - b;
    float4 acc = make_float4(0.f, 0.f, 0.f, 0.f);
    const float* Xl = X + lane * 4;

    for (int base = 0; __any(base < len); base += LPR) {
        int c = 0; float v = 0.f;
        if (base + lane < len) {
            c = col[b + base + lane];
            v = val ? val[b + base + lane] : 1.f;
        }
        const int cnt = len - base;
        for (int k = 0; k < LPR; k += U) {
            if (!__any(k < cnt)) break;
            int cc[U]; float vv[U]; float4 xv[U];
#pragma unroll
            for (int u = 0; u < U; ++u) {
                cc[u] = __shfl(c, k + u, LPR);
                vv[u] = __shfl(v, k + u, LPR);
            }
#pragma unroll
            for (int u = 0; u < U; ++u) {
                xv[u] = make_float4(0.f, 0.f, 0.f, 0.f);
                if (k + u < cnt && k + u < LPR)
                    xv[u] = *reinterpret_cast<const float4*>(Xl + (int64_t)cc[u] * ldx);
            }
#pragma unroll
            for (int u = 0; u < U; ++u) {
                acc.x = fmaf(vv[u], xv[u].x, acc.x); acc.y = fmaf(vv[u], xv[u].y, acc.y);
                acc.z = fmaf(vv[u], xv[u].z, acc.z); acc.w = fmaf(vv[u], xv[u].w, acc.w);
            }
        }
    }
    if (ep.colpart) {
        float4 g = make_float4(0.f, 0.f, 0.f, 0.f);
        if (active) {
            if (slot < 0) g = epilogue_store4<LPR, OUT3>(ep, acc, row, lane, (int64_t)LPR * 4, Y, ldy);
            else *reinterpret_cast<float4*>(partial + (int64_t)slot * (LPR * 4) + lane * 4) = acc;
        }
        block_colsum_store<LPR>(g, ep.colpart + (int64_t)blockIdx.x * (LPR * 4));
        return;
    }
    if (!active) return;
    if (slot < 0) epilogue_store4<LPR, OUT3>(ep, acc, row, lane, (int64_t)LPR * 4, Y, ldy);
    else *reinterpret_cast<float4*>(partial + (int64_t)slot * (LPR * 4) + lane * 4) = acc;
}

template <int LPR, bool OUT3 = false>
__global__ __launch_bounds__(256) void spmm_vec4_wave_kernel(
    const int* __restrict__ rowptr, const int* __restrict__ col, const float* __restrict__ val,
    const int4* __restrict__ items, int n_items, float* __restrict__ partial,
    const float* __restrict__ X, int64_t ldx, float* __restrict__ Y, int64_t ldy, Epilogue ep)
{
    const int gid = (int)(((int64_t)blockIdx.x * blockDim.x + threadIdx.x) >> 6);
    const int wl = threadIdx.x & 63;
    const int lane = wl & (LPR - 1), sub = wl / LPR;
    if (gid >= n_items) return;
    int row, b, e, slot = -1;
    if (items) { const int4 it = items[gid]; row = it.x; b = it.y; e = it.z; slot = it.w; }
    else { row = gid; b = rowptr[gid]; e = rowptr[gid + 1]; }
    const int len = e - b;
    float4 acc = make_float4(0.f, 0.f, 0.f, 0.f);
    const float* Xl = X + lane * 4;
    for (int base = sub * LPR; base - sub * LPR < len; base += 64) {
        int c = 0; float v = 0.f;
        if (base + lane < len) {
            c = col[b + base + lane];
            v = val ? val[b + base + lane] : 1.f;
        }
        const int cnt = len - base;
        constexpr int U = LPR < 4 ? LPR : 4;
        for (int k = 0; k < LPR; k += U) {
            if (!__any(k < cnt)) break;
            int cc[U]; float vv[U]; float4 xv[U];
#pragma unroll
            for (int u = 0; u < U; ++u) { cc[u] = __shfl(c, k + u, LPR); vv[u] = __shfl(v, k + u, LPR); }
#pragma unroll
            for (int u = 0; u < U; ++u) {
                xv[u] = make_float4(0.f, 0.f, 0.f, 0.f);
                if (k + u < cnt) xv[u] = *reinterpret_cast<const float4*>(Xl + (int64_t)cc[u] * ldx);
            }
#pragma unroll
            for (int u = 0; u < U; ++u) {
                acc.x = fmaf(vv[u], xv[u].x, acc.x); acc.y = fmaf(vv[u], xv[u].y, acc.y);
                acc.z = fmaf(vv[u], xv[u].z, acc.z); acc.w = fmaf(vv[u], xv[u].w, acc.w);
            }
        }
    }
#pragma unroll
    for (int off = LPR; off < 64; off <<= 1) {
        acc.x += __shfl_xor(acc.x, off, 64); acc.y += __shfl_xor(acc.y, off, 64);
        acc.z += __shfl_xor(acc.z, off, 64); acc.w += __shfl_xor(acc.w, off, 64);
    }
    if (sub != 0) return;
    if (slot < 0) epilogue_store4<LPR, OUT3>(ep, acc, row, lane, (int64_t)LPR * 4, Y, ldy);
    else *reinterpret_cast<float4*>(partial + (int64_t)slot * (LPR * 4) + lane * 4) = acc;
}

template <int LPR, bool OUT3 = false>
__global__ __launch_bounds__(256) void spmm_finish_vec4_kernel(
    const int4* __restrict__ long_rows, int n_long, const float* __restrict__ partial,
    float* __restrict__ Y, int64_t ldy, Epilogue ep)
{
    const int64_t tid = (int64_t)blockIdx.x * blockDim.x + threadIdx.x;
    const int gid = (int)(tid / LPR);
    const int lane = threadIdx.x & (LPR - 1);
    const bool active = gid < n_long;
    if (!active && !ep.colpart) return;
    const int4 lr = active ? long_rows[gid] : make_int4(0, 0, 0, 0);
    float4 acc = make_float4(0.f, 0.f, 0.f, 0.f);
    int s = lr.y;
    for (; s + 3 < lr.z; s += 4) {
        const float4 p0 = *reinterpret_cast<const float4*>(partial + (int64_t)s * (LPR * 4) + lane * 4);
        const float4 p1 = *reinterpret_cast<const float4*>(partial + (int64_t)(s + 1) * (LPR * 4) + lane * 4);
        const float4 p2 = *reinterpret_cast<const float4*>(partial + (int64_t)(s + 2) * (LPR * 4) + lane * 4);
        const float4 p3 = *reinterpret_cast<const float4*>(partial + (int64_t)(s + 3) * (LPR * 4) + lane * 4);
        acc.x += p0.x; acc.y += p0.y; acc.z += p0.z; acc.w += p0.w;
        acc.x += p1.x; acc.y += p1.y; acc.z += p1.z; acc.w += p1.w;
        acc.x += p2.x; acc.y += p2.y; acc.z += p2.z; acc.w += p2.w;
        acc.x += p3.x; acc.y += p3.y; acc.z += p3.z; acc.w += p3.w;
    }
    for (; s < lr.z; ++s) {
        const float4 p = *reinterpret_cast<const float4*>(partial + (int64_t)s * (LPR * 4) + lane * 4);
        acc.x += p.x; acc.y += p.y; acc.z += p.z; acc.w += p.w;
    }
    if (ep.colpart) {
        float4 g = make_float4(0.f, 0.f, 0.f, 0.f);
        if (active) g = epilogue_store4<LPR, OUT3>(ep, acc, lr.x, lane, (int64_t)LPR * 4, Y, ldy);
        block_colsum_store<LPR>(g, ep.colpart + (ep.colpart_row0 + blockIdx.x) * (LPR * 4));
        return;
    }
    epilogue_store4<LPR, OUT3>(ep, acc, lr.x, lane, (int64_t)LPR * 4, Y, ldy);
}

__device__ __forceinline__ void epilogue_store1(const Epilogue& ep, float z, int row, int c, int64_t d,
                                                float* Y, int64_t ldy) {
    if (ep.bias) z += ep.bias[c];
    float y = ep.relu ? fmaxf(z, 0.f) : z;
    if (ep.K) ep.K[(int64_t)row * d + c] = y;
    if (ep.pre.n > 0) y = fmaf(ep.alpha, y, lc_load1(ep.pre, (int64_t)row * d + c));
    else y *= ep.alpha;
    Y[(int64_t)row * ldy + c] = y;
    if (ep.Y2) {
        const int64_t o = (int64_t)row * d + c;
        const float g = lc_load1(ep.cot, o);
        ep.Y2[o] = z > 0.f ? g : 0.f;
        if (ep.Y3) {
            float g3 = 0.f;
#pragma unroll
            for (int j = 0; j < GODE_MAX_TERMS; ++j)
                if (j < ep.cot.n) g3 = fmaf(ep.c3[j], ep.cot.ptr[j][o], g3);
            ep.Y3[o] = g3;
        }
    }
}

__global__ __launch_bounds__(256) void spmm_generic_kernel(
    const int* __restrict__ rowptr, const int* __restrict__ col, const float* __restrict__ val,
    const int4* __restrict__ items, int n_items, float* __restrict__ partial,
    const float* __restrict__ X, int64_t ldx, float* __restrict__ Y, int64_t ldy, int d, int G, Epilogue ep)
{
    const int64_t tid = (int64_t)blockIdx.x * blockDim.x + threadIdx.x;
    const int gid = (int)(tid / G);
    const int lane = threadIdx.x & (G - 1);
    if (gid >= n_items) return;
    int row, b, e, slot = -1;
    if (items) { const int4 it = items[gid]; row = it.x; b = it.y; e = it.z; slot = it.w; }
    else { row = gid; b = rowptr[gid]; e = rowptr[gid + 1]; }
    for (int c = lane; c < d; c += G) {
        float acc = 0.f;
        int j = b;
        for (; j + 4 <= e; j += 4) {
            const int c0 = col[j], c1 = col[j + 1], c2 = col[j + 2], c3 = col[j + 3];
            const float x0 = X[(int64_t)c0 * ldx + c], x1 = X[(int64_t)c1 * ldx + c], x2 = X[(int64_t)c2 * ldx + c],
                        x3 = X[(int64_t)c3 * ldx + c];
            float v0 = 1.f, v1 = 1.f, v2 = 1.f, v3 = 1.f;
            if (val) { v0 = val[j]; v1 = val[j + 1]; v2 = val[j + 2]; v3 = val[j + 3]; }
            acc = fmaf(v0, x0, acc); acc = fmaf(v1, x1, acc); acc = fmaf(v2, x2, acc); acc = fmaf(v3, x3, acc);
        }
        for (; j < e; ++j) {
            const float v = val ? val[j] : 1.f;
            acc = fmaf(v, X[(int64_t)col[j] * ldx + c], acc);
        }
        if (slot < 0) epilogue_store1(ep, acc, row, c, d, Y, ldy);
        else partial[(int64_t)slot * d + c] = acc;
    }
}

__global__ __launch_bounds__(256) void spmv_wave_kernel(
    const int* __restrict__ rowptr, const int* __restrict__ col, const float* __restrict__ val,
    const int4* __restrict__ items, int n_items, float* __restrict__ partial,
    const float* __restrict__ X, int64_t ldx, float* __restrict__ Y, int64_t ldy, Epilogue ep)
{
    const int gid = (int)(((int64_t)blockIdx.x * blockDim.x + threadIdx.x) >> 6);
    const int lane = threadIdx.x & 63;
    if (gid >= n_items) return;
    int row, b, e, slot = -1;
    if (items) { const int4 it = items[gid]; row = it.x; b = it.y; e = it.z; slot = it.w; }
    else { row = gid; b = rowptr[gid]; e = rowptr[gid + 1]; }
    float acc = 0.f;
    for (int j = b + lane; j < e; j += 64) acc = fmaf(val ? val[j] : 1.f, X[(int64_t)col[j] * ldx], acc);
    acc = wave_sum(acc);
    if (lane == 0) {
        if (slot < 0) epilogue_store1(ep, acc, row, 0, 1, Y, ldy);
        else partial[slot] = acc;
    }
}

__global__ __launch_bounds__(256) void spmm_finish_generic_kernel(
    const int4* __restrict__ long_rows, int n_long, const float* __restrict__ partial,
    float* __restrict__ Y, int64_t ldy, int d, int G, Epilogue ep)
{
    const int64_t tid = (int64_t)blockIdx.x * blockDim.x + threadIdx.x;
    const int gid = (int)(tid / G);
    const int lane = threadIdx.x & (G - 1);
    if (gid >= n_long) return;
    const int4 lr = long_rows[gid];
    for (int c = lane; c < d; c += G) {
        float acc = 0.f;
        for (int s = lr.y; s < lr.z; ++s) acc += partial[(int64_t)s * d + c];
        epilogue_store1(ep, acc, lr.x, c, d, Y, ldy);
    }
}

template <int LPR, bool OUT3>
int launch_vec4(const int* rowptr, const int* col, const float* val, const int4* items, int n_items,
                const int4* long_rows, int n_long, float* partial, const float* X, int64_t ldx,
                float* Y, int64_t ldy, const Epilogue& ep, hipStream_t s) {
    if (LPR < 64 && n_items > 0 && n_items <= 65536) {
        if (ep.colpart) return GODE_E_UNSUPPORTED;
        const int64_t wb = ((int64_t)n_items * 64 + 255) / 256;
        const int slot = gode_prof_begin(s, (int64_t)LPR * 4, n_items, (int64_t)ep.pre.n + ep.cot.n + (ep.Y2 ? 1 : 0) + (ep.Y3 ? 1 : 0));
        hipLaunchKernelGGL((spmm_vec4_wave_kernel<LPR, OUT3>), dim3((unsigned)wb), dim3(256), 0, s,
                           rowptr, col, val, items, n_items, partial, X, ldx, Y, ldy, ep);
        gode_prof_end(s, slot);
        GODE_LAUNCH_CHECK();
        if (n_long > 0) {
            const int64_t b2 = ((int64_t)n_long * LPR + 255) / 256;
            hipLaunchKernelGGL((spmm_finish_vec4_kernel<LPR, OUT3>), dim3((unsigned)b2), dim3(256), 0, s,
                               long_rows, n_long, partial, Y, ldy, ep);
            GODE_LAUNCH_CHECK();
        }
        return 0;
    }
    const int64_t threads = (int64_t)n_items * LPR;
    const int64_t blocks = (threads + 255) / 256;
    if (blocks > 0) {
        const int slot = gode_prof_begin(s, (int64_t)LPR * 4, n_items, (int64_t)ep.pre.n + ep.cot.n + (ep.Y2 ? 1 : 0) + (ep.Y3 ? 1 : 0));
        hipLaunchKernelGGL((spmm_vec4_kernel<LPR, OUT3>), dim3((unsigned)blocks), dim3(256), 0, s,
                           rowptr, col, val, items, n_items, partial, X, ldx, Y, ldy, ep);
        gode_prof_end(s, slot);
        GODE_LAUNCH_CHECK();
    }
    if (n_long > 0) {
        const int64_t b2 = ((int64_t)n_long * LPR + 255) / 256;
        Epilogue ep2 = ep;
        ep2.colpart_row0 = blocks;
        hipLaunchKernelGGL((spmm_finish_vec4_kernel<LPR, OUT3>), dim3((unsigned)b2), dim3(256), 0, s,
                           long_rows, n_long, partial, Y, ldy, ep2);
        GODE_LAUNCH_CHECK();
    }
    return 0;
}

}

extern "C" int64_t gode_spmm_y2_colsum_rows(int64_t n_items, int64_t n_long, int64_t d)
{
    if (n_items <= 0 || n_long < 0 || d <= 0 || d % 4) return 0;
    const int64_t lpr = d / 4;
    if (lpr > 64 || (lpr & (lpr - 1))) return 0;
    if (lpr < 64 && n_items <= 65536) return 0;
    return (n_items * lpr + 255) / 256 + (n_long * lpr + 255) / 256;
}

namespace {

int spmm_csr_impl(const int32_t* rowptr, const int32_t* col, const float* val,
                  const int32_t* items, int64_t n_items,
                  const int32_t* long_rows, int64_t n_long, float* partial,
                  const float* X, int64_t ldx, float* Y, int64_t ldy,
                  int64_t n_rows, int64_t d,
                  const gode_spmm_epilogue_t* epi, float* K, void* stream)
{
    if (n_rows < 0 || d <= 0 || ldx < d || ldy < d) return GODE_E_SHAPE;
    if (n_rows == 0) return 0;
    if (!rowptr || !col || !X || !Y) return GODE_E_NULLPTR;
    if (n_rows > INT32_MAX || d > (1 << 20)) return GODE_E_RANGE;
    if (!items) { n_items = n_rows; n_long = 0; }
    if (n_items < 0 || n_items > INT32_MAX || n_long < 0 || n_long > INT32_MAX) return GODE_E_RANGE;
    if (n_long > 0 && (!long_rows || !partial)) return GODE_E_NULLPTR;
    if (n_items * 64 >= ((int64_t)1 << 32)) return GODE_E_RANGE;
    const float* bias = epi ? epi->bias : nullptr;
    float* Y2 = epi ? epi->Y2 : nullptr;
    const gode_lincomb_t* cot = (epi && Y2) ? &epi->cot : nullptr;
    const gode_lincomb_t* pre = (epi && epi->pre.n > 0) ? &epi->pre : nullptr;
    if (Y2) { int rc = check_lincomb(cot, true); if (rc) return rc; }
    if (pre) { int rc = check_lincomb(pre, true); if (rc) return rc; }
    hipStream_t s = (hipStream_t)stream;

    Epilogue ep;
    ep.bias = bias; ep.relu = epi ? epi->relu : 0; ep.alpha = epi ? epi->alpha : 1.f;
    ep.pre = make_lincomb(pre); ep.cot = make_lincomb(cot); ep.Y2 = Y2;
    ep.colpart = (epi && Y2) ? epi->Y2_colsum : nullptr; ep.colpart_row0 = 0;
    ep.K = K;
    ep.Y3 = (epi && Y2) ? epi->cot_out : nullptr;
    for (int j = 0; j < GODE_MAX_TERMS; ++j) ep.c3[j] = (ep.Y3 && j < ep.cot.n) ? epi->cot_out_coef[j] : 0.f;
    if (ep.Y3) {
        if (ep.Y3 == Y || ep.Y3 == Y2 || ep.Y3 == K) return GODE_E_RANGE;
        for (int j = 0; j < ep.cot.n; ++j) if (ep.Y3 == ep.cot.ptr[j]) return GODE_E_RANGE;
    }
    if (ep.colpart && ((((uintptr_t)ep.colpart) & 15) || gode_spmm_y2_colsum_rows(n_items, n_long, d) == 0)) return GODE_E_UNSUPPORTED;

    const bool al = !(((uintptr_t)X) & 15) && !(((uintptr_t)Y) & 15) && (ldx % 4 == 0) && (ldy % 4 == 0) &&
                    (!bias || !(((uintptr_t)bias) & 15)) && (!partial || !(((uintptr_t)partial) & 15)) &&
                    (!Y2 || (!(((uintptr_t)Y2) & 15) && lincomb_aligned16(cot))) && lincomb_aligned16(pre) &&
                    !(((uintptr_t)K) & 15) && !(((uintptr_t)ep.Y3) & 15);
    const int4* it4 = reinterpret_cast<const int4*>(items);
    const int4* lr4 = reinterpret_cast<const int4*>(long_rows);
    if (al && d % 4 == 0) {
        switch (d / 4) {
#define GODE_CASE(L) case L: return ep.Y3 ? launch_vec4<L, true>(rowptr, col, val, it4, (int)n_items, lr4, (int)n_long, partial, X, ldx, Y, ldy, ep, s) \
                                        : launch_vec4<L, false>(rowptr, col, val, it4, (int)n_items, lr4, (int)n_long, partial, X, ldx, Y, ldy, ep, s);
            GODE_CASE(1) GODE_CASE(2) GODE_CASE(4) GODE_CASE(8) GODE_CASE(16) GODE_CASE(32) GODE_CASE(64)
#undef GODE_CASE
            default: break;
        }
    }
    if (ep.colpart) return GODE_E_UNSUPPORTED;
    int G = 1; while (G < d && G < 64) G <<= 1;
    if (d == 1 && it4 != nullptr) {
        const int64_t blocks = ((int64_t)n_items * 64 + 255) / 256;
        const int slot = gode_prof_begin(s, 1, n_items, (int64_t)ep.pre.n + ep.cot.n + (ep.Y2 ? 1 : 0) + (ep.Y3 ? 1 : 0));
        hipLaunchKernelGGL(spmv_wave_kernel, dim3((unsigned)blocks), dim3(256), 0, s,
                           rowptr, col, val, it4, (int)n_items, partial, X, ldx, Y, ldy, ep);
        gode_prof_end(s, slot);
        GODE_LAUNCH_CHECK();
    } else {
        const int64_t blocks = ((int64_t)n_items * G + 255) / 256;
        hipLaunchKernelGGL(spmm_generic_kernel, dim3((unsigned)blocks), dim3(256), 0, s,
                           rowptr, col, val, it4, (int)n_items, partial, X, ldx, Y, ldy, (int)d, G, ep);
        GODE_LAUNCH_CHECK();
    }
    if (n_long > 0) {
        const int64_t b2 = ((int64_t)n_long * G + 255) / 256;
        hipLaunchKernelGGL(spmm_finish_generic_kernel, dim3((unsigned)b2), dim3(256), 0, s,
                           lr4, (int)n_long, partial, Y, ldy, (int)d, G, ep);
        GODE_LAUNCH_CHECK();
    }
    return 0;
}

}

extern "C" int gode_spmm_csr_f32(const int32_t* rowptr, const int32_t* col, const float* val,
                                 const int32_t* items, int64_t n_items,
                                 const int32_t* long_rows, int64_t n_long, float* partial,
                                 const float* X, int64_t ldx, float* Y, int64_t ldy,
                                 int64_t n_rows, int64_t d,
                                 const gode_spmm_epilogue_t* epi, void* stream)
{
    return spmm_csr_impl(rowptr, col, val, items, n_items, long_rows, n_long, partial, X, ldx, Y, ldy, n_rows, d, epi,
                         nullptr, stream);
}

extern "C" int gode_spmm_csr_save_f32(const int32_t* rowptr, const int32_t* col, const float* val,
                                      const int32_t* items, int64_t n_items,
                                      const int32_t* long_rows, int64_t n_long, float* partial,
                                      const float* X, int64_t ldx, float* Y, int64_t ldy,
                                      int64_t n_rows, int64_t d,
                                      const gode_spmm_epilogue_t* epi, float* K, void* stream)
{
    if (n_rows < 0 || d <= 0 || ldx < d || ldy < d) return GODE_E_SHAPE;
    if (n_rows > 0 && !K) return GODE_E_NULLPTR;
    return spmm_csr_impl(rowptr, col, val, items, n_items, long_rows, n_long, partial, X, ldx, Y, ldy, n_rows, d, epi,
                         K, stream);
}
```

### graph_odenet_amd/gcn_ode.py

```python
import ctypes

import torch

from . import _lib, ops
from .graph import as_graph
from .solver import Field


def _graph_struct(g, d):
    gs = _lib.Graph()
    gs.rowptr, gs.col = g.rowptr.data_ptr(), g.col.data_ptr()
    gs.val = g.val.data_ptr() if g.val is not None else None
    gs.items, gs.n_items = (g.items.data_ptr() if g.items is not None else None), g.n_items
    gs.long_rows = g.long_rows.data_ptr() if g.long_rows is not None else None
    gs.n_long = g.n_long
    part = g.partial(d)
    gs.partial = part.data_ptr() if part is not None else None
    gs.n_rows, gs.nnz = g.n_rows, g.nnz
    return gs


class _Shared:

    def __init__(self, graph, d, device):
        n = graph.n_rows
        self.S = torch.empty(n, d, dtype=torch.float32, device=device)
        self.dZ = None
        self.dS = None
        self.n = n
        self.d = d
        self.device = device
        self._ky = self._ka = self._kt = None
        self._parts = None
        self.y2_rows = 0
        if not getattr(graph, "is_partitioned", False) and hasattr(graph, "n_items"):
            self.y2_rows = _lib.load().gode_spmm_y2_colsum_rows(graph.n_items if graph.items is not None else n, graph.n_long, d)
        self._y2_colsum = None
        self._X2 = None

    @property
    def X2(self):
        if self._X2 is None:
            self._X2 = [torch.empty_like(self.S), torch.empty_like(self.S)]
        return self._X2

    def bwd(self):
        if self.dZ is None:
            self.dZ = torch.empty_like(self.S)
            self.dS = torch.empty_like(self.S)
        return self.dZ, self.dS

    def stage_buffers(self, adjoint):
        if self._ky is None:
            self._ky = [torch.empty_like(self.S) for _ in range(4)]
        if adjoint and self._ka is None:
            lib = _lib.load()
            P = lib.gode_gcn_ode_theta_len(self.d)
            self._ka = [torch.empty_like(self.S) for _ in range(4)]
            self._kt = [torch.empty(P, dtype=torch.float32, device=self.device) for _ in range(4)]
            nW = (self.d + 1) * self.d
            self._parts = (torch.empty(lib.gode_wgrad_parts(self.n) * nW, dtype=torch.float32, device=self.device),
                           torch.empty(lib.gode_gemm_bwd_parts(self.n) * self.d, dtype=torch.float32, device=self.device),
                           torch.empty(lib.gode_gemm_bwd_parts(self.n) * self.d, dtype=torch.float32, device=self.device),
                           torch.empty(max(lib.gode_colsum_scratch_bytes(self.n, self.d), 16), dtype=torch.uint8,
                                       device=self.device))
        return self._ky, self._ka, self._kt, self._parts

    def workspace_struct(self, adjoint, groups=0):
        ky, ka, kt, parts = self.stage_buffers(adjoint)
        ws = _lib.Rk4Workspace()
        ws.S = self.S.data_ptr()
        for i in range(4):
            ws.ky[i] = ky[i].data_ptr()
        if not adjoint and _lib.load().gode_gcn_small_supported(self.n, self.d, int(groups)):
            ws.X[0], ws.X[1] = self.X2[0].data_ptr(), self.X2[1].data_ptr()
        if adjoint:
            dZ, dS = self.bwd()
            ws.dZ, ws.dS = dZ.data_ptr(), dS.data_ptr()
            if getattr(self, "S2", None) is None:
                self.S2 = torch.empty_like(self.S)
            ws.S2 = self.S2.data_ptr()
            for i in range(4):
                ws.ka[i] = ka[i].data_ptr()
                ws.ktheta[i] = kt[i].data_ptr()
            ws.wpart, ws.gpart, ws.bpart, ws.colsum_scratch = (p.data_ptr() for p in parts)
            ws.X[0], ws.X[1] = self.X2[0].data_ptr(), self.X2[1].data_ptr()
            sp = self.small_part(groups)
            ws.small_part = sp.data_ptr() if sp is not None else None
            if self.y2_rows > 0:
                if self._y2_colsum is None:
                    self._y2_colsum = torch.empty(self.y2_rows, self.d, dtype=torch.float32, device=self.device)
                ws.y2_colsum = self._y2_colsum.data_ptr()
        return ws

    def cot_colpart(self):
        rows = _lib.load().gode_masked_cot_parts(self.n, self.d)
        if rows <= 0:
            return None
        if getattr(self, "_cot_colpart", None) is None:
            self._cot_colpart = torch.empty(rows, self.d, dtype=torch.float32, device=self.device)
        return self._cot_colpart

    def small_part(self, groups):
        lib = _lib.load()
        if not lib.gode_gcn_small_supported(self.n, self.d, int(groups)):
            return None
        if getattr(self, "_small_part", None) is None:
            self._small_part = torch.empty(7 * lib.gode_gcn_small_parts(self.n) * lib.gode_gcn_small_part_len(self.d),
                                           dtype=torch.float32, device=self.device)
        return self._small_part


def _func_struct(spec):
    fs = _lib.GcnOdeFunc()
    fs.A = _graph_struct(spec.graph, spec.d)
    fs.AT = _graph_struct(spec.graph.transpose(), spec.d)
    fs.n, fs.d, fs.groups, fs.eps = spec.graph.n_rows, spec.d, spec.groups, spec.eps
    fs.W, fs.b = spec.W.data_ptr(), spec.b.data_ptr()
    fs.gamma, fs.beta = spec.gamma.data_ptr(), spec.beta.data_ptr()
    return fs


def _by_ptr(ptr_value, candidates):
    for t in candidates:
        if t.data_ptr() == ptr_value:
            return t
    raise RuntimeError("rk4 driver returned an unknown buffer")


RELABEL_MIN_OPERAND_BYTES = 64 << 20
RELABEL_MIN_NNZ = 1 << 21
RELABEL_MIN_IMBALANCE = 2.0
NODE_ORDERS = ("auto", "given", "degree")


def gather_imbalance(graph, d, inverse=None):
    m = max(8, min(4096, (32 << 10) // (4 * d)))
    col = graph.col.to(torch.int64)
    rp = graph.rowptr.to(torch.int64)
    deg = rp[1:] - rp[:-1]
    rows = torch.arange(graph.n_rows, device=col.device)
    if inverse is not None:
        col, rows = inverse[col], inverse
    h_a = torch.bincount(col % m, minlength=m)
    h_t = torch.zeros(m, dtype=torch.int64, device=col.device).index_add_(0, rows % m, deg)
    h = torch.stack([h_a, h_t]).tolist()
    return max(max(hh) * m / max(sum(hh), 1) for hh in h)


def tuned_graph(graph, d, node_order="auto"):
    if node_order not in NODE_ORDERS:
        raise ValueError("node_order must be one of %s, got %r" % (NODE_ORDERS, node_order))
    cache = graph.__dict__.setdefault("_tuned", {})
    hit = cache.get((d, node_order))
    if hit is not None:
        return hit
    res = (graph, None, None)
    info = {"node_order": node_order, "renumbered": False}
    square = graph.n_rows == graph.n_cols and not getattr(graph, "is_partitioned", False)
    big = graph.n_rows * d * 4 >= RELABEL_MIN_OPERAND_BYTES and graph.nnz >= RELABEL_MIN_NNZ
    if square and node_order != "given" and (node_order == "degree" or big) \
            and not torch.cuda.is_current_stream_capturing():
        order = graph.degree_order()
        inverse = torch.empty_like(order)
        inverse[order] = torch.arange(graph.n_rows, device=graph.device)
        take = node_order == "degree"
        if not take:
            given, hubs = gather_imbalance(graph, d), gather_imbalance(graph, d, inverse)
            info.update(imbalance_given=round(given, 4), imbalance_hubs_first=round(hubs, 4))
            take = given >= RELABEL_MIN_IMBALANCE and hubs <= 0.5 * given
        if take:
            res = (graph.relabel(order), order, inverse)
            info["renumbered"] = True
    graph.__dict__.setdefault("_tuned_info", {})[(d, node_order)] = info
    cache[(d, node_order)] = res
    return res


class GcnOdeSpec:

    def __init__(self, graph, W, b, gamma, beta, groups, eps):
        self.graph, self.W, self.b, self.gamma, self.beta = graph, W, b, gamma, beta
        self.groups, self.eps = int(groups), float(eps)
        self.d = W.shape[1]
        if W.shape[0] != self.d + 1:
            raise ValueError("GcnOdeSpec: weight must be (d+1) x d, got %s" % (tuple(W.shape),))
        if graph.n_rows != graph.n_cols:
            raise ValueError("GcnOdeSpec: adjacency must be square")


def small_fused(spec):
    lib = _lib.load()
    return bool(lib.gode_get_option(b"small_fused") == 1 and not getattr(spec.graph, "is_partitioned", False)
                and lib.gode_gcn_small_supported(spec.graph.n_rows, spec.d, spec.groups))


def _feval_small(spec, t, terms, out, pre=None, alpha=1.0, cot=None, out2=None, next_terms=None, x_next=None):
    lib = _lib.load()
    fs = _func_struct(spec)
    lx = _lib.lincomb(terms)
    lp = _lib.lincomb(pre) if pre is not None else None
    lc = _lib.lincomb(cot) if cot is not None else None
    ln = _lib.lincomb(next_terms) if next_terms is not None else None
    _lib.check(lib.gode_gcn_feval_small_next_f32(ctypes.byref(fs), ctypes.byref(lx), float(t), float(alpha),
                                                 ctypes.byref(lp) if lp is not None else None,
                                                 ctypes.byref(lc) if lc is not None else None,
                                                 _lib.ptr(out2) if cot is not None else None, _lib.ptr(out),
                                                 ctypes.byref(ln) if ln is not None else None,
                                                 _lib.ptr(x_next) if ln is not None else None, _lib.stream_ptr()),
               "gode_gcn_feval_small_next_f32")


class _PackedParams:

    def _theta_len(self):
        return (self.s.d + 1) * self.s.d + 3 * self.s.d + 1

    def _packed_state(self, th, y, a):
        d = self.s.d
        nW = (d + 1) * d
        comps = [y, a, th[nW + 3 * d:], th[:nW].view(d + 1, d), th[nW:nW + d], th[nW + d:nW + 2 * d],
                 th[nW + 2 * d:nW + 3 * d]]
        comps[2]._gode_packed = th
        return comps

    def _in_params_order(self, comps):
        m = {"W": comps[3], "b": comps[4], "gamma": comps[5], "beta": comps[6]}
        return [m[k] for k in self.params_order]

    def packed_grads(self, device):
        return torch.zeros(self._theta_len(), dtype=torch.float32, device=device)

    def packed_param_grads(self, theta):
        return self._in_params_order(self._packed_state(theta, None, None))


class GcnOdeField(_PackedParams, Field):
    n_components = 1
    fused = True

    def __init__(self, spec, shared, params_order):
        self.s, self.w = spec, shared
        self.params_order = params_order
        self.token = ("gcn", id(spec.graph))

    def eval(self, t, terms, out):
        s, w = self.s, self.w
        if small_fused(s):
            return _feval_small(s, t, terms[0], out[0])
        ops.gn_time_gemm(terms[0], w.n, s.d, s.groups, s.eps, s.gamma, s.beta, s.W, True, t, out=w.S)
        ops.spmm(s.graph, w.S, bias=s.b, relu=True, out=out[0])

    def rk4_native(self, comps, t0, t1, n_steps):
        lib = _lib.load()
        s, w = self.s, self.w
        ky = w.stage_buffers(False)[0]
        fs, ws = _func_struct(s), w.workspace_struct(False, s.groups)
        res = ctypes.c_void_p()
        _lib.check(lib.gode_gcn_ode_rk4_forward(ctypes.byref(fs), _lib.ptr(comps[0]), ctypes.byref(res), ctypes.byref(ws),
                                                float(t0), float(t1), int(n_steps), _lib.stream_ptr()),
                   "gode_gcn_ode_rk4_forward")
        out = _by_ptr(res.value, [comps[0]] + ky)
        if out is not comps[0]:
            comps[0].copy_(out)
        return 4 * n_steps

    def rk4_forward_save(self, y0, y_end, save, t0, t1, n_steps, i0, i1):
        lib = _lib.load()
        s, w = self.s, self.w
        fs, ws = _func_struct(s), w.workspace_struct(False, s.groups)
        _lib.check(lib.gode_gcn_ode_rk4_forward_save(ctypes.byref(fs), _lib.ptr(y0), _lib.ptr(y_end), _lib.ptr(save),
                                                     ctypes.byref(ws), float(t0), float(t1), int(n_steps), int(i0), int(i1),
                                                     _lib.stream_ptr()), "gode_gcn_ode_rk4_forward_save")

    def rk4_backprop(self, save, a, theta, t0, t1, n_steps, i0, i1):
        lib = _lib.load()
        s, w = self.s, self.w
        ka = w.stage_buffers(True)[1]
        fs, ws = _func_struct(s), w.workspace_struct(True, s.groups)
        res = ctypes.c_void_p()
        _lib.check(lib.gode_gcn_ode_rk4_backprop(ctypes.byref(fs), _lib.ptr(save), _lib.ptr(a), _lib.ptr(theta),
                                                 ctypes.byref(res), ctypes.byref(ws), _lib.ptr(w.cot_colpart()),
                                                 float(t0), float(t1), int(n_steps), int(i0), int(i1), _lib.stream_ptr()),
                   "gode_gcn_ode_rk4_backprop")
        return _by_ptr(res.value, [a] + ka)

    def eval_combine(self, t, terms, pre, coef, out):
        s, w = self.s, self.w
        if small_fused(s):
            _feval_small(s, t, terms[0], out[0], pre=pre[0], alpha=coef)
            return (0,)
        ops.gn_time_gemm(terms[0], w.n, s.d, s.groups, s.eps, s.gamma, s.beta, s.W, True, t, out=w.S)
        ops.spmm(s.graph, w.S, bias=s.b, relu=True, out=out[0], pre_terms=pre[0], alpha=coef)
        return (0,)

    def dopri5_step_native(self, y, kk, y1, t, h, rtol, atol):
        lib = _lib.load()
        s, w = self.s, self.w
        fs, ws = _func_struct(s), w.workspace_struct(False, s.groups)
        kptr = (ctypes.c_void_p * 7)(*[kk[i][0].data_ptr() for i in range(7)])
        sums = torch.empty(1, dtype=torch.float64, device=y[0].device)
        sc = ops._scratch(y[0].device, lib.gode_rk_errnorm_scratch_bytes())
        _lib.check(lib.gode_gcn_ode_dopri5_step_forward(ctypes.byref(fs), _lib.ptr(y[0]), kptr, _lib.ptr(y1[0]),
                                                        ctypes.byref(ws), float(t), float(h), float(rtol), float(atol),
                                                        _lib.ptr(sums), _lib.ptr(sc), _lib.stream_ptr()),
                   "gode_gcn_ode_dopri5_step_forward")
        return sums

    def dopri5_backprop_work(self, like):
        lib = _lib.load()
        P = lib.gode_gcn_ode_theta_len(self.s.d)
        return {"ybar": [torch.empty_like(like) for _ in range(7)],
                "pairs": [(torch.empty_like(like), torch.empty_like(like)) for _ in range(2)],
                "ktheta": [torch.empty(P, dtype=torch.float32, device=like.device) for _ in range(7)]}

    def dopri5_step_backprop(self, y, k, g, kbar7, wy, wk, t, h, first, work, turn, theta):
        lib = _lib.load()
        s, w = self.s, self.w
        w.stage_buffers(True)
        fs, ws = _func_struct(s), w.workspace_struct(True, s.groups)
        arr = lambda ts: (ctypes.c_void_p * 7)(*[x.data_ptr() for x in ts])
        ybar_n, kbar1 = work["pairs"][turn]
# ... 218 lines not shown
```

### graph_odenet_amd/graph.py

```python
import weakref

import torch

DEFAULT_SPLIT = None


def auto_split(nnz):
    return 256 if nnz >= (1 << 20) else 1024


class CSRGraph:

    def __init__(self, rowptr, col, val, n_rows, n_cols, split=DEFAULT_SPLIT, records=True):
        self.rowptr = rowptr.to(torch.int32).contiguous()
        self.col = col.to(torch.int32).contiguous()
        self.val = None if val is None else val.to(torch.float32).contiguous()
        self.n_rows = int(n_rows)
        self.n_cols = int(n_cols)
        self.nnz = int(self.col.numel())
        self.device = self.col.device
        self.split = int(split) if split is not None else auto_split(self.nnz)
        if records:
            self._build_items()
        else:
            self.items, self.n_items, self.long_rows, self.n_long, self.n_slots = None, self.n_rows, None, 0, 0
        self._partial = {}
        self._T = None

    def _build_items(self):
        dev = self.device
        n = self.n_rows
        rp = self.rowptr.to(torch.int64)
        deg = rp[1:] - rp[:-1]
        L = self.split
        nseg = torch.clamp((deg + L - 1) // L, min=1)
        total = int(nseg.sum().item()) if n > 0 else 0
        rows = torch.repeat_interleave(torch.arange(n, device=dev, dtype=torch.int64), nseg)
        first = torch.cumsum(nseg, 0) - nseg
        k = torch.arange(total, device=dev, dtype=torch.int64) - first[rows]
        begin = rp[rows] + k * L
        end = torch.minimum(begin + L, rp[rows + 1])
        is_long = nseg[rows] > 1
        slot = torch.where(is_long, torch.cumsum(is_long.to(torch.int64), 0) - 1,
                           torch.full_like(rows, -1))
        self.n_slots = int(is_long.sum().item()) if total > 0 else 0
        items = torch.stack([rows, begin, end, slot], 1)
        order = torch.argsort(end - begin, descending=True, stable=True)
        self.items = items[order].to(torch.int32).contiguous()
        self.n_items = total
        long_rows = torch.nonzero(nseg > 1).flatten()
        self.n_long = int(long_rows.numel())
        if self.n_long:
            long_first = torch.cumsum(nseg[long_rows], 0) - nseg[long_rows]
            lr = torch.stack([long_rows, long_first, long_first + nseg[long_rows],
                              torch.zeros_like(long_rows)], 1)
            self.long_rows = lr.to(torch.int32).contiguous()
        else:
            self.long_rows = None

    def partial(self, d):
        if self.n_slots == 0:
            return None
        buf = self._partial.get(d)
        if buf is None:
            buf = torch.empty(self.n_slots * d, dtype=torch.float32, device=self.device)
            self._partial[d] = buf
        return buf

    def transpose(self):
        if self._T is None:
            rp = self.rowptr.to(torch.int64)
            rows = torch.repeat_interleave(torch.arange(self.n_rows, device=self.device), rp[1:] - rp[:-1])
            self._T = from_coo(self.col.to(torch.int64), rows, self.val, self.n_cols, self.n_rows,
                               split=self.split, coalesce=False)
            self._T._T = self
        return self._T

    def degree_order(self):
        rp = self.rowptr.to(torch.int64)
        deg = rp[1:] - rp[:-1]
        deg = deg + torch.bincount(self.col.to(torch.int64), minlength=self.n_cols)[: self.n_rows]
        return torch.argsort(deg, descending=True, stable=True)

    def relabel(self, order):
        if self.n_rows != self.n_cols:
            raise ValueError("relabel: square matrices only")
        order = order.to(torch.int64)
        new_id = torch.empty_like(order)
        new_id[order] = torch.arange(self.n_rows, device=self.device)

        def one(g):
            rp = g.rowptr.to(torch.int64)
            deg = (rp[1:] - rp[:-1])[order]
            rowptr = torch.zeros(g.n_rows + 1, dtype=torch.int64, device=g.device)
            rowptr[1:] = torch.cumsum(deg, 0)
            idx = torch.repeat_interleave(rp[order] - rowptr[:-1], deg) + torch.arange(g.nnz, device=g.device)
            return CSRGraph(rowptr, new_id[g.col.to(torch.int64)[idx]], None if g.val is None else g.val[idx],
                            g.n_rows, g.n_cols, split=g.split)
        out, out_t = one(self), one(self.transpose())
        out._T, out_t._T = out_t, out
        return out

    def to_dense(self):
        rp = self.rowptr.to(torch.int64)
        rows = torch.repeat_interleave(torch.arange(self.n_rows, device=self.device), rp[1:] - rp[:-1])
        out = torch.zeros(self.n_rows, self.n_cols, dtype=torch.float32, device=self.device)
        v = self.val if self.val is not None else torch.ones(self.nnz, device=self.device)
        out.index_put_((rows, self.col.to(torch.int64)), v, accumulate=True)
        return out

    def algorithmic_bytes(self, d):
        per = 4 + (4 if self.val is not None else 0) + 4 * d
        return self.nnz * per + (self.n_rows + 1) * 4 + self.n_rows * d * 4


def from_coo(rows, cols, vals, n_rows, n_cols, split=DEFAULT_SPLIT, coalesce=True):
    rows = rows.to(torch.int64)
    cols = cols.to(torch.int64)
    key = rows * n_cols + cols
    if coalesce:
        ukey, inv = torch.unique(key, sorted=True, return_inverse=True)
        if ukey.numel() != key.numel():
            if vals is None:
                vals = torch.ones(key.numel(), dtype=torch.float32, device=key.device)
            vals = torch.zeros(ukey.numel(), dtype=torch.float32, device=key.device).index_add_(0, inv, vals.float())
        elif vals is not None:
            vals = torch.empty_like(vals, dtype=torch.float32).index_copy_(0, inv, vals.float())
        key = ukey
    else:
        order = torch.argsort(key, stable=True)
        key = key[order]
        if vals is not None:
            vals = vals[order]
    r = key // n_cols
    c = key % n_cols
    counts = torch.bincount(r, minlength=n_rows)
    rowptr = torch.zeros(n_rows + 1, dtype=torch.int64, device=key.device)
    rowptr[1:] = torch.cumsum(counts, 0)
    return CSRGraph(rowptr, c, vals, n_rows, n_cols, split=split)


_cache = {}


def _evict(key):
    _cache.pop(key, None)


def as_graph(adj, split=DEFAULT_SPLIT):
    if isinstance(adj, CSRGraph) or getattr(adj, "is_partitioned", False):
        return adj
    if not torch.is_tensor(adj):
        raise TypeError("adjacency must be a torch tensor (sparse COO or dense) or CSRGraph")
    key = id(adj)
    hit = _cache.get(key)
    if hit is not None and hit[0]() is adj and hit[2] == adj._version:
        return hit[1]
    if adj.dim() != 2:
        raise ValueError("adjacency must be 2-D, got shape %s" % (tuple(adj.shape),))
    if adj.is_sparse:
        idx = adj._indices()
        vals = adj._values()
        g = from_coo(idx[0], idx[1], vals, adj.shape[0], adj.shape[1], split=split)
    elif adj.layout == torch.sparse_csr:
        g = CSRGraph(adj.crow_indices(), adj.col_indices(), adj.values(), adj.shape[0], adj.shape[1], split=split)
    else:
        nz = torch.nonzero(adj)
        g = from_coo(nz[:, 0], nz[:, 1], adj[nz[:, 0], nz[:, 1]], adj.shape[0], adj.shape[1], split=split)
    try:
        ref = weakref.ref(adj, lambda _r, k=key: _evict(k))
        _cache[key] = (ref, g, adj._version)
    except TypeError:
        pass
    return g


RECORDS_MIN_NNZ = 1 << 16


def csr_from_assignment(index, n_rows, vals=None, split=DEFAULT_SPLIT, records=None):
    idx = index.to(torch.int64)
    e = idx.numel()
    if records is None:
        records = e >= RECORDS_MIN_NNZ
    if idx.is_cuda and not records and n_rows > 0:
        from . import _lib
        lib = _lib.load()
        if lib.gode_assign_csr_supported(e, n_rows):
            idx = idx.contiguous()
            rowptr = torch.empty(n_rows + 1, dtype=torch.int32, device=idx.device)
            order = torch.empty(e, dtype=torch.int32, device=idx.device)
            v_in = None if vals is None else vals.to(torch.float32).contiguous()
            v = None if vals is None else torch.empty(e, dtype=torch.float32, device=idx.device)
            _lib.check(lib.gode_assign_csr_i32(_lib.ptr(idx), e, n_rows, _lib.ptr(rowptr), _lib.ptr(order), _lib.ptr(v_in),
                                               _lib.ptr(v), _lib.stream_ptr()), "gode_assign_csr_i32")
            return CSRGraph(rowptr, order, v, n_rows, e, split=split, records=False)
    order = torch.argsort(idx, stable=True)
    counts = torch.zeros(n_rows, dtype=torch.int64, device=idx.device).index_add_(
        0, idx, torch.ones(e, dtype=torch.int64, device=idx.device))
    rowptr = torch.zeros(n_rows + 1, dtype=torch.int64, device=idx.device)
    rowptr[1:] = torch.cumsum(counts, 0)
    v = None if vals is None else vals.to(torch.float32)[order]
    return CSRGraph(rowptr, order, v, n_rows, e, split=split, records=records)


def incidence_from_index(index, n_rows, split=DEFAULT_SPLIT):
    return csr_from_assignment(index, n_rows, None, split=split)
```

### graph_odenet_amd/ops.py

```python
import ctypes

import torch

from . import _lib
from ._lib import check, lincomb, ptr, stream_ptr


def _need(t, name, dtype=torch.float32):
    if t is None:
        return
    if not t.is_cuda:
        raise RuntimeError("graph_odenet_amd: %s must live on the GPU (got %s); there is no CPU path" % (name, t.device))
    if t.dtype != dtype:
        raise TypeError("graph_odenet_amd: %s must be %s, got %s" % (name, dtype, t.dtype))
    if not t.is_contiguous():
        raise ValueError("graph_odenet_amd: %s must be contiguous" % name)


def _need_terms(terms, name):
    n = None
    for c, t in terms:
        _need(t, name)
        if n is None:
            n = t.numel()
        elif t.numel() != n:
            raise ValueError("graph_odenet_amd: %s terms differ in size" % name)
    return n


def spmm(graph, X, bias=None, relu=False, out=None, cot_terms=None, out2=None, pre_terms=None, alpha=1.0, out2_colsum=None,
         cot_out=None, cot_out_coefs=None):
    lib = _lib.load()
    _need(X, "X")
    _need(bias, "bias")
    if getattr(graph, "is_partitioned", False):
        if X.dim() != 2 or X.shape[0] != graph.n_cols:
            raise ValueError("spmm: X has shape %s, this rank owns %d rows" % (tuple(X.shape), graph.n_cols))
        X, graph = graph.gather(X), graph.local
    if X.dim() != 2 or X.shape[0] != graph.n_cols:
        raise ValueError("spmm: X has shape %s, graph is %d x %d" % (tuple(X.shape), graph.n_rows, graph.n_cols))
    d = X.shape[1]
    if bias is not None and bias.numel() != d:
        raise ValueError("spmm: bias has %d elements, expected %d" % (bias.numel(), d))
    ldy = d
    if out is None:
        out = torch.empty(graph.n_rows, d, dtype=torch.float32, device=X.device)
    else:
        if tuple(out.shape) != (graph.n_rows, d):
            raise ValueError("spmm: out has wrong shape")
        if out.is_contiguous():
            _need(out, "out")
        else:
            if not out.is_cuda or out.dtype != torch.float32 or out.stride(1) != 1 or out.stride(0) < d:
                raise ValueError("spmm: out must be contiguous or a unit-stride column block of a row-major matrix")
            ldy = out.stride(0)
    ep = None
    if bias is not None or relu or cot_terms is not None or pre_terms is not None or alpha != 1.0:
        ep = _lib.SpmmEpilogue()
        ep.bias = bias.data_ptr() if bias is not None else None
        ep.relu = 1 if relu else 0
        ep.alpha = float(alpha)
        if pre_terms is not None:
            if _need_terms(pre_terms, "pre") != graph.n_rows * d:
                raise ValueError("spmm: pre terms have wrong size")
            ep.pre = lincomb(pre_terms)
        if cot_terms is not None:
            if _need_terms(cot_terms, "cot") != graph.n_rows * d:
                raise ValueError("spmm: cotangent terms have wrong size")
            ep.cot = lincomb(cot_terms)
            if out2 is None:
                out2 = torch.empty(graph.n_rows, d, dtype=torch.float32, device=X.device)
            _need(out2, "out2")
            ep.Y2 = out2.data_ptr()
            if out2_colsum is not None:
                _need(out2_colsum, "out2_colsum")
                if out2_colsum.numel() != spmm_y2_colsum_rows(graph, d) * d or out2_colsum.numel() == 0:
                    raise ValueError("spmm: out2_colsum must be spmm_y2_colsum_rows(graph, d) x d (and the shape must support it)")
                ep.Y2_colsum = out2_colsum.data_ptr()
            if cot_out is not None:
                _need(cot_out, "cot_out")
                if cot_out.numel() != graph.n_rows * d or cot_out_coefs is None or len(cot_out_coefs) != len(cot_terms):
                    raise ValueError("spmm: cot_out must be n_rows x d with one coefficient per cotangent term")
                ep.cot_out = cot_out.data_ptr()
                for j, cj in enumerate(cot_out_coefs):
                    ep.cot_out_coef[j] = float(cj)
        elif cot_out is not None:
            raise ValueError("spmm: cot_out needs cot_terms")
    partial = graph.partial(d)
    rc = lib.gode_spmm_csr_f32(ptr(graph.rowptr), ptr(graph.col), ptr(graph.val),
                               ptr(graph.items), graph.n_items,
                               ptr(graph.long_rows), graph.n_long, ptr(partial),
                               ptr(X), d, ptr(out), ldy, graph.n_rows, d,
                               ctypes.byref(ep) if ep is not None else None, stream_ptr())
    check(rc, "gode_spmm_csr_f32")
    return (out, out2) if cot_terms is not None else out


def spmm_y2_colsum_rows(graph, d):
    return int(_lib.load().gode_spmm_y2_colsum_rows(graph.n_items if graph.items is not None else graph.n_rows, graph.n_long, int(d)))


def lincomb_(out, terms):
    lib = _lib.load()
    _need(out, "out")
    if _need_terms(terms, "lincomb") != out.numel():
        raise ValueError("lincomb: size mismatch")
    lc = lincomb(terms)
    check(lib.gode_lincomb_f32(ptr(out), ctypes.byref(lc), out.numel(), stream_ptr()), "gode_lincomb_f32")
    return out


def lincomb_multi_(outs, terms_list):
    lib = _lib.load()
    k = len(outs)
    if k != len(terms_list) or not 1 <= k <= 4:
        raise ValueError("lincomb_multi: one term list per output, at most four")
    lcs = (_lib.LinComb * k)()
    ptrs = (ctypes.c_void_p * k)()
    ns = (ctypes.c_int64 * k)()
    for c, (out, terms) in enumerate(zip(outs, terms_list)):
        _need(out, "out")
        if _need_terms(terms, "lincomb") != out.numel():
            raise ValueError("lincomb_multi: size mismatch in component %d" % c)
        lcs[c] = lincomb(terms)
        ptrs[c] = out.data_ptr()
        ns[c] = out.numel()
    check(lib.gode_lincomb_multi_f32(ptrs, lcs, ns, k, stream_ptr()), "gode_lincomb_multi_f32")
    return outs


_red_scratch = {}
_retired = []


def _scratch(device, nbytes):
    key = (device, _lib.current_stream_handle(device.index if device.index is not None else torch.cuda.current_device()))
    buf = _red_scratch.get(key)
    if buf is None or buf.numel() < nbytes:
        if buf is not None:
            _retired.append(buf)
        buf = torch.empty(max(nbytes, 1 << 20), dtype=torch.uint8, device=device)
        _red_scratch[key] = buf
    return buf


def rk_error_sumsq(y0, y1, err_terms, rtol, atol, out=None):
    lib = _lib.load()
    _need(y0, "y0"); _need(y1, "y1")
    n = y0.numel()
    if _need_terms(err_terms, "err") != n or y1.numel() != n:
        raise ValueError("rk_error_sumsq: size mismatch")
    if out is None:
        out = torch.empty(1, dtype=torch.float64, device=y0.device)
    sc = _scratch(y0.device, lib.gode_rk_errnorm_scratch_bytes())
    lc = lincomb(err_terms)
    check(lib.gode_rk_errnorm_f32(ptr(out), ptr(y0), ptr(y1), ctypes.byref(lc), float(rtol), float(atol), n,
                                  ptr(sc), stream_ptr()), "gode_rk_errnorm_f32")
    return out


def rk_scaled_sumsq(terms, y, rtol, atol, out=None):
    lib = _lib.load()
    _need(y, "y")
    n = y.numel()
    if _need_terms(terms, "terms") != n:
        raise ValueError("rk_scaled_sumsq: size mismatch")
    if out is None:
        out = torch.empty(1, dtype=torch.float64, device=y.device)
    sc = _scratch(y.device, lib.gode_rk_errnorm_scratch_bytes())
    lc = lincomb(terms)
    check(lib.gode_rk_scaled_sumsq_f32(ptr(out), ctypes.byref(lc), ptr(y), float(rtol), float(atol), n,
                                       ptr(sc), stream_ptr()), "gode_rk_scaled_sumsq_f32")
    return out


def gn_time_gemm(x_terms, n_rows, d_in, groups, eps, gamma, beta, W, has_time, t, out=None, x_out=None, aux_coefs=None,
                 aux_out=None):
    lib = _lib.load()
    _need(W, "W"); _need(gamma, "gamma"); _need(beta, "beta")
    if _need_terms(x_terms, "x") != n_rows * d_in:
        raise ValueError("gn_time_gemm: x terms have wrong size")
    if W.dim() != 2 or W.shape[0] != d_in + (1 if has_time else 0):
        raise ValueError("gn_time_gemm: W has shape %s" % (tuple(W.shape),))
    d_out = W.shape[1]
    if out is None:
        out = torch.empty(n_rows, d_out, dtype=torch.float32, device=W.device)
    _need(out, "out")
    lc = lincomb(x_terms)
    if x_out is not None:
        _need(x_out, "x_out")
        if x_out.numel() != n_rows * d_in:
            raise ValueError("gn_time_gemm: x_out has wrong size")
    if aux_out is not None:
        _need(aux_out, "aux_out")
        if aux_out.numel() != n_rows * d_in or aux_coefs is None or len(aux_coefs) != len(x_terms):
            raise ValueError("gn_time_gemm: aux_out must be n_rows x d_in with one coefficient per term")
        ac = (ctypes.c_float * len(aux_coefs))(*[float(c) for c in aux_coefs])
        check(lib.gode_gn_time_gemm_xout_aux_f32(ctypes.byref(lc), n_rows, d_in, groups, float(eps), ptr(gamma), ptr(beta),
                                                 ptr(W), d_out, 1 if has_time else 0, float(t), ptr(out), ptr(x_out),
                                                 ac, ptr(aux_out), stream_ptr()), "gode_gn_time_gemm_xout_aux_f32")
        return out
    check(lib.gode_gn_time_gemm_xout_f32(ctypes.byref(lc), n_rows, d_in, groups, float(eps), ptr(gamma), ptr(beta),
                                         ptr(W), d_out, 1 if has_time else 0, float(t), ptr(out), ptr(x_out),
                                         stream_ptr()), "gode_gn_time_gemm_xout_f32")
    return out


def gn_time_gemm_pair(x_terms, n_rows, d, groups, eps, gamma, beta, Wa, Wb, has_time, t, out_a, out_b, x_out=None):
    lib = _lib.load()
    for tns, nm in ((Wa, "Wa"), (Wb, "Wb"), (gamma, "gamma"), (beta, "beta"), (out_a, "out_a"), (out_b, "out_b"), (x_out, "x_out")):
        _need(tns, nm)
    if _need_terms(x_terms, "x") != n_rows * d:
        raise ValueError("gn_time_gemm_pair: x terms have wrong size")
    k = d + (1 if has_time else 0)
    if tuple(Wa.shape) != (k, d) or tuple(Wb.shape) != (k, d) or out_a.numel() != n_rows * d or out_b.numel() != n_rows * d:
        raise ValueError("gn_time_gemm_pair: weights must be (%d, %d) and outputs n x d" % (k, d))
    lc = lincomb(x_terms)
    check(lib.gode_gn_time_gemm_pair_f32(ctypes.byref(lc), n_rows, d, groups, float(eps), ptr(gamma), ptr(beta), ptr(Wa), ptr(Wb),
                                         1 if has_time else 0, float(t), ptr(out_a), ptr(out_b), ptr(x_out), stream_ptr()),
          "gode_gn_time_gemm_pair_f32")


def gat_small_supported(n_rows, d, groups, heads=1):
    lib = _lib.load()
    return bool(lib.gode_get_option(b"small_fused")) and bool(lib.gode_gat_small_supported(n_rows, d, groups, heads))


def gat_small_part(n_rows, d, heads, device):
    lib = _lib.load()
    return torch.empty(lib.gode_gat_small_parts(n_rows, d), lib.gode_gat_small_part_len(d, heads), dtype=torch.float32, device=device)


def gat_small_pack(Wsrc, Wtgt, Wlog, heads, out=None):
    lib = _lib.load()
    _need(Wsrc, "Wsrc"); _need(Wtgt, "Wtgt"); _need(Wlog, "Wlog"); _need(out, "packed")
    d = Wsrc.shape[1]
    n = lib.gode_gat_small_pack_len(d, heads)
    if out is None:
        out = torch.empty(n, dtype=torch.float32, device=Wsrc.device)
    elif out.numel() != n:
        raise ValueError("gat_small_pack: packed buffer must hold %d floats" % n)
    check(lib.gode_gat_small_pack_f32(ptr(Wsrc), ptr(Wtgt), ptr(Wlog), d, heads, ptr(out), stream_ptr()), "gode_gat_small_pack_f32")
    return out


def gat_project_small(x_terms, n_rows, d, groups, eps, gamma, beta, Wsrc, Wtgt, Wlog, heads, pt_bias, t, Ps, Pt, A2, x_out=None,
                      packed=None):
    lib = _lib.load()
    for tns, nm in ((gamma, "gamma"), (beta, "beta"), (Wsrc, "Wsrc"), (Wtgt, "Wtgt"), (Wlog, "Wlog"), (pt_bias, "pt_bias"),
                    (Ps, "Ps"), (Pt, "Pt"), (A2, "A2"), (x_out, "x_out")):
        _need(tns, nm)
    if _need_terms(x_terms, "x") != n_rows * d:
        raise ValueError("gat_project_small: x terms have wrong size")
    if tuple(Wsrc.shape) != (d + 1, d) or tuple(Wtgt.shape) != (d + 1, d) or tuple(Wlog.shape) != (d + 1, 2 * heads):
        raise ValueError("gat_project_small: weights must be (d+1) x d, (d+1) x d, (d+1) x 2H")
    if Ps.numel() != n_rows * d or Pt.numel() != n_rows * d or A2.numel() != n_rows * 2 * heads or \
            (x_out is not None and x_out.numel() != n_rows * d) or (pt_bias is not None and pt_bias.numel() != d):
        raise ValueError("gat_project_small: output buffers have wrong size")
    lc = lincomb(x_terms)
    check(lib.gode_gat_project_small_f32(ctypes.byref(lc), n_rows, d, groups, float(eps), ptr(gamma), ptr(beta), ptr(Wsrc), ptr(Wtgt),
                                         ptr(Wlog), heads, ptr(pt_bias), float(t), ptr(Ps), ptr(Pt), ptr(A2), ptr(x_out),
                                         ptr(packed), stream_ptr()), "gode_gat_project_small_f32")


def gat_dense_vjp_small(x_terms, n_rows, d, groups, eps, gamma, beta, Wsrc, Wtgt, Wlog, heads, dPs, dPt, dA2, ka, part,
                        out_scale=1.0, pre_terms=None, maxfix=None, packed=None):
    lib = _lib.load()
    for tns, nm in ((gamma, "gamma"), (beta, "beta"), (Wsrc, "Wsrc"), (Wtgt, "Wtgt"), (Wlog, "Wlog"), (dPs, "dPs"), (dPt, "dPt"),
                    (dA2, "dA2"), (ka, "ka"), (part, "part")):
        _need(tns, nm)
    if _need_terms(x_terms, "x") != n_rows * d:
        raise ValueError("gat_dense_vjp_small: x terms have wrong size")
    if tuple(Wsrc.shape) != (d + 1, d) or tuple(Wtgt.shape) != (d + 1, d) or tuple(Wlog.shape) != (d + 1, 2 * heads):
        raise ValueError("gat_dense_vjp_small: weights must be (d+1) x d, (d+1) x d, (d+1) x 2H")
    if dPs.numel() != n_rows * d or dPt.numel() != n_rows * d or dA2.numel() != n_rows * 2 * heads or ka.numel() != n_rows * d or \
            part.numel() != lib.gode_gat_small_parts(n_rows, d) * lib.gode_gat_small_part_len(d, heads):
        raise ValueError("gat_dense_vjp_small: buffers have wrong size")
    lc = lincomb(x_terms)
    pre = None
    if pre_terms:
        if _need_terms(pre_terms, "pre") != n_rows * d:
            raise ValueError("gat_dense_vjp_small: pre terms have wrong size")
        pre = lincomb(pre_terms)
    check(lib.gode_gat_dense_vjp_small_f32(ctypes.byref(lc), n_rows, d, groups, float(eps), ptr(gamma), ptr(beta), ptr(Wsrc), ptr(Wtgt),
                                           ptr(Wlog), heads, ptr(dPs), ptr(dPt), ptr(dA2), float(out_scale),
                                           ctypes.byref(pre) if pre is not None else None, ptr(ka), ptr(part),
                                           ptr(maxfix[0]) if maxfix else None, ptr(maxfix[1]) if maxfix else None,
                                           ptr(maxfix[2]) if maxfix else None, maxfix[1].numel() if maxfix else 0, ptr(packed),
                                           stream_ptr()),
          "gode_gat_dense_vjp_small_f32")


def gat_small_finish(part, n_rows, d, heads, t, ktheta, kat):
    lib = _lib.load()
    _need(part, "part"); _need(ktheta, "ktheta"); _need(kat, "kat")
    if part.numel() != lib.gode_gat_small_parts(n_rows, d) * lib.gode_gat_small_part_len(d, heads) or \
            ktheta.numel() != lib.gode_gat_ode_theta_len_heads(d, heads) or kat.numel() != 1:
        raise ValueError("gat_small_finish: buffers have wrong size")
    check(lib.gode_gat_small_finish_f32(ptr(part), n_rows, d, heads, float(t), ptr(ktheta), ptr(kat), stream_ptr()),
          "gode_gat_small_finish_f32")


def gat_small_finish_step(parts, n_rows, d, heads, ts, ws, theta, at):
    lib = _lib.load()
    _need(parts, "parts"); _need(theta, "theta"); _need(at, "a_t")
    k = len(ts)
    if parts.numel() < k * lib.gode_gat_small_parts(n_rows, d) * lib.gode_gat_small_part_len(d, heads) or \
            theta.numel() != lib.gode_gat_ode_theta_len_heads(d, heads) or at.numel() != 1:
        raise ValueError("gat_small_finish_step: buffers have wrong size")
    tsa, wsa = (ctypes.c_float * 4)(*([float(v) for v in ts] + [0.0] * (4 - k))), (ctypes.c_float * 4)(*([float(v) for v in ws] + [0.0] * (4 - k)))
    check(lib.gode_gat_small_finish_step_f32(ptr(parts), n_rows, d, heads, k, tsa, wsa, ptr(theta), ptr(at), stream_ptr()),
          "gode_gat_small_finish_step_f32")


def gn_time_gemm_bwd(x_terms, n_rows, d_in, groups, eps, gamma, W, has_time, dS, out_scale=1.0, out=None,
                     want_affine_grads=True, pre_terms=None, parts=None):
    lib = _lib.load()
    _need(W, "W"); _need(gamma, "gamma"); _need(dS, "dS")
    if _need_terms(x_terms, "x") != n_rows * d_in:
        raise ValueError("gn_time_gemm_bwd: x terms have wrong size")
    d_out = W.shape[1]
    if out is None:
        out = torch.empty(n_rows, d_in, dtype=torch.float32, device=W.device)
    _need(out, "out")
    dg = db = None
    if want_affine_grads and groups > 0:
        n_part = lib.gode_gemm_bwd_parts(n_rows)
        if parts is not None:
            dg, db = parts
            _need(dg, "dgamma parts"); _need(db, "dbeta parts")
            if dg.numel() != n_part * d_in or db.numel() != n_part * d_in:
                raise ValueError("gn_time_gemm_bwd: partial buffers have wrong size")
        else:
            dg = torch.empty(n_part, d_in, dtype=torch.float32, device=W.device)
            db = torch.empty(n_part, d_in, dtype=torch.float32, device=W.device)
    lc = lincomb(x_terms)
    pre = None
    if pre_terms is not None:
        if _need_terms(pre_terms, "pre") != n_rows * d_in:
            raise ValueError("gn_time_gemm_bwd: pre terms have wrong size")
        pre = lincomb(pre_terms)
    check(lib.gode_gn_time_gemm_bwd_f32(ctypes.byref(lc), n_rows, d_in, groups, float(eps), ptr(gamma), ptr(W),
                                        d_out, 1 if has_time else 0, ptr(dS), float(out_scale),
                                        ctypes.byref(pre) if pre is not None else None, ptr(out),
                                        ptr(dg), ptr(db), stream_ptr()), "gode_gn_time_gemm_bwd_f32")
    return out, dg, db


def bwd_wgrad_supported(n_rows, d, groups):
    return bool(_lib.load().gode_bwd_wgrad_supported(n_rows, d, d, groups))


def gn_time_gemm_bwd_wgrad(x_terms, n_rows, d, groups, eps, gamma, beta, W, has_time, dS, out_scale=1.0, out=None,
                           pre_terms=None, parts=None, wpart=None):
    lib = _lib.load()
    _need(W, "W"); _need(gamma, "gamma"); _need(beta, "beta"); _need(dS, "dS")
    if _need_terms(x_terms, "x") != n_rows * d:
        raise ValueError("gn_time_gemm_bwd_wgrad: x terms have wrong size")
    if out is None:
        out = torch.empty(n_rows, d, dtype=torch.float32, device=W.device)
    _need(out, "out")
    dg = db = None
    if groups > 0:
        n_part = lib.gode_gemm_bwd_parts(n_rows)
        if parts is not None:
            dg, db = parts
        else:
            dg = torch.empty(n_part, d, dtype=torch.float32, device=W.device)
            db = torch.empty(n_part, d, dtype=torch.float32, device=W.device)
    K = d + (1 if has_time else 0)
    npw = lib.gode_bwd_wgrad_parts(n_rows)
    if wpart is None:
        wpart = torch.empty(npw, K * d, dtype=torch.float32, device=W.device)
    elif wpart.numel() < npw * K * d:
        raise ValueError("gn_time_gemm_bwd_wgrad: weight-gradient partial buffer too small")
    lc = lincomb(x_terms)
    pre = lincomb(pre_terms) if pre_terms is not None else None
    check(lib.gode_gn_time_gemm_bwd_wgrad_f32(ctypes.byref(lc), n_rows, d, groups, float(eps), ptr(gamma), ptr(beta), ptr(W), d,
                                              1 if has_time else 0, ptr(dS), float(out_scale),
                                              ctypes.byref(pre) if pre is not None else None, ptr(out), ptr(dg), ptr(db),
                                              ptr(wpart), stream_ptr()), "gode_gn_time_gemm_bwd_wgrad_f32")
    return out, dg, db, wpart.view(-1)[:npw * K * d].view(npw, K * d)


def wgrad(x_terms, n_rows, d_in, groups, eps, gamma, beta, dS, has_time, part=None):
    lib = _lib.load()
    _need(dS, "dS"); _need(gamma, "gamma"); _need(beta, "beta")
    if _need_terms(x_terms, "x") != n_rows * d_in:
        raise ValueError("wgrad: x terms have wrong size")
    d_out = dS.shape[1]
# ... 716 lines not shown
```

### include/graphode.h

```cpp
#ifndef GRAPHODE_H
#define GRAPHODE_H

#include <stdint.h>

#ifdef __cplusplus
extern "C" {
#endif

#define GODE_ABI_VERSION 1

#define GODE_E_NULLPTR  (-1)
#define GODE_E_SHAPE    (-2)
#define GODE_E_ALIGN    (-3)
#define GODE_E_RANGE    (-4)
#define GODE_E_UNSUPPORTED (-5)

#define GODE_MAX_TERMS 8

typedef struct gode_lincomb {
    int32_t      n;
    float        coef[GODE_MAX_TERMS];
    const float* ptr[GODE_MAX_TERMS];
} gode_lincomb_t;

int         gode_abi_version(void);
int         gode_set_option(const char* name, int value);
int         gode_get_option(const char* name);
const char* gode_error_string(int code);

typedef struct gode_spmm_epilogue {
    const float*   bias;
    int32_t        relu;
    float          alpha;
    gode_lincomb_t pre;
    gode_lincomb_t cot;
    float*         Y2;
    float*         Y2_colsum;
    float*         cot_out;
    float          cot_out_coef[GODE_MAX_TERMS];
} gode_spmm_epilogue_t;

int64_t gode_spmm_y2_colsum_rows(int64_t n_items, int64_t n_long, int64_t d);

int gode_spmm_csr_f32(const int32_t* rowptr, const int32_t* col, const float* val,
                      const int32_t* items, int64_t n_items,
                      const int32_t* long_rows, int64_t n_long, float* partial,
                      const float* X, int64_t ldx, float* Y, int64_t ldy,
                      int64_t n_rows, int64_t d,
                      const gode_spmm_epilogue_t* epi ,
                      void* stream);
int gode_spmm_csr_save_f32(const int32_t* rowptr, const int32_t* col, const float* val,
                           const int32_t* items, int64_t n_items,
                           const int32_t* long_rows, int64_t n_long, float* partial,
                           const float* X, int64_t ldx, float* Y, int64_t ldy,
                           int64_t n_rows, int64_t d,
                           const gode_spmm_epilogue_t* epi , float* K,
                           void* stream);

int64_t gode_masked_cot_parts(int64_t n_rows, int64_t d);
int gode_masked_cot_f32(const gode_lincomb_t* cot , const float* k, float* dZ, int64_t n_rows, int64_t d,
                        float* colpart , void* stream);

int gode_lincomb_f32(float* out, const gode_lincomb_t* lc , int64_t n, void* stream);
int gode_lincomb_multi_f32(float* const* outs , const gode_lincomb_t* lcs ,
                           const int64_t* ns , int32_t count, void* stream);

int64_t gode_rk_errnorm_scratch_bytes(void);
int gode_rk_errnorm_f32(double* out, const float* y0, const float* y1,
                        const gode_lincomb_t* elc , float rtol, float atol,
                        int64_t n, void* scratch, void* stream);
int gode_rk_errnorm_multi_f32(double* out, const float* const* y0 , const float* const* y1,
                              const gode_lincomb_t* elcs , const int64_t* ns, int32_t count, float rtol,
                              float atol, void* scratch, void* stream);

int gode_rk_scaled_sumsq_f32(double* out, const gode_lincomb_t* lc , const float* y,
                             float rtol, float atol, int64_t n, void* scratch, void* stream);

int gode_gn_time_gemm_f32(const gode_lincomb_t* xin , int64_t n_rows, int64_t d_in,
                          int32_t groups, float eps, const float* gamma, const float* beta,
                          const float* W, int64_t d_out, int has_time, float t,
                          float* S, void* stream);
int gode_gn_time_gemm_xout_f32(const gode_lincomb_t* xin , int64_t n_rows, int64_t d_in,
                               int32_t groups, float eps, const float* gamma, const float* beta,
                               const float* W, int64_t d_out, int has_time, float t,
                               float* S, float* x_out, void* stream);
int gode_gn_time_gemm_xout_aux_f32(const gode_lincomb_t* xin , int64_t n_rows, int64_t d_in,
                                   int32_t groups, float eps, const float* gamma, const float* beta,
                                   const float* W, int64_t d_out, int has_time, float t,
                                   float* S, float* x_out , const float* aux_coef ,
                                   float* aux_out, void* stream);

int gode_gn_time_gemm_pair_f32(const gode_lincomb_t* xin , int64_t n_rows, int64_t d, int32_t groups, float eps,
                               const float* gamma, const float* beta, const float* Wa, const float* Wb,
                               int has_time, float t, float* Sa, float* Sb, float* x_out, void* stream);

int64_t gode_gemm_bwd_parts(int64_t n_rows);
int gode_gn_time_gemm_bwd_f32(const gode_lincomb_t* xin , int64_t n_rows, int64_t d_in,
                              int32_t groups, float eps, const float* gamma,
                              const float* W, int64_t d_out, int has_time,
                              const float* dS, float out_scale,
                              const gode_lincomb_t* pre , float* dx,
                              float* dgamma_part, float* dbeta_part, void* stream);

int gode_bwd_wgrad_supported(int64_t n_rows, int64_t d_in, int64_t d_out, int32_t groups);
int64_t gode_bwd_wgrad_parts(int64_t n_rows);
int gode_gn_time_gemm_bwd_wgrad_f32(const gode_lincomb_t* xin , int64_t n_rows, int64_t d_in, int32_t groups,
                                    float eps, const float* gamma, const float* beta, const float* W, int64_t d_out,
                                    int has_time, const float* dS, float out_scale, const gode_lincomb_t* pre ,
                                    float* dx, float* dgamma_part, float* dbeta_part, float* dW_part, void* stream);

#define GODE_MAX_REDUCE_SEGS 8
typedef struct gode_reduce_seg {
    float* out; const float* part;
    int64_t n_part, ld, col0, col_stride, len;
    const float* w_row0; int64_t time_len;
} gode_reduce_seg_t;
int gode_reduce_segments_f32(const gode_reduce_seg_t* segs, int32_t n_segs, float t, float* at , void* stream);
int gode_colsum_parts_f32(const float* X, int64_t n_rows, int64_t d, float* scratch, int64_t* n_parts , void* stream);

int64_t gode_group_norm_parts(int64_t n_rows);
int gode_group_norm_f32_fwd(const float* x, int64_t n_rows, int64_t d, int32_t groups, float eps,
                            const float* gamma , const float* beta , float* y, void* stream);
int gode_group_norm_f32_bwd(const float* x, int64_t n_rows, int64_t d, int32_t groups, float eps,
                            const float* gamma , const float* dy, float* dx,
                            float* dgamma_part , float* dbeta_part , void* stream);

int64_t gode_wgrad_parts(int64_t n_rows);
int gode_wgrad_f32(const gode_lincomb_t* xin , int64_t n_rows, int64_t d_in,
                   int32_t groups, float eps, const float* gamma, const float* beta,
                   const float* dS, int64_t d_out, int has_time,
                   float* dW_part, void* stream);

int gode_rect_gemm_f32(const float* X, int64_t ldx, int64_t n_rows, int64_t K, const float* W, int64_t M,
                       float* S, int64_t lds, void* stream);
int gode_rect_gemm_nt_f32(const float* dS, int64_t ldds, int64_t n_rows, int64_t M, const float* W, int64_t K,
                          float* dX, int64_t lddx, void* stream);
int64_t gode_rect_wgrad_parts(int64_t n_rows);
int gode_rect_wgrad_f32(const float* X, int64_t ldx, int64_t n_rows, int64_t K, const float* dS, int64_t ldds,
                        int64_t M, float* part, void* stream);
int gode_rect_wgrad_sum_f32(const float* X, int64_t ldx, int64_t n_rows, int64_t K, const float* dS, int64_t ldds, int64_t M,
                            float* part, float* dW, void* stream);

int gode_gemm_f32(int trans_a, int trans_b, int64_t M, int64_t N, int64_t K, const float* A, int64_t lda,
                  const float* B, int64_t ldb, float* C, int64_t ldc, const float* bias, int relu,
                  const float* mask, int64_t ldmask, void* stream);
int64_t gode_gemm_splitk_parts(int64_t M, int64_t N, int64_t K);
int gode_gemm_splitk_f32(int trans_a, int trans_b, int64_t M, int64_t N, int64_t K, const float* A, int64_t lda,
                         const float* B, int64_t ldb, float* part, float* C , void* stream);

int64_t gode_cut_pad(int64_t n);
int gode_cut_bf16x3_f32(const float* X, int64_t ld, int64_t R, int64_t C, void* planes, void* stream);
int64_t gode_pgemm_workspace_bytes(int64_t M, int64_t N, int64_t K);
int gode_pgemm_bf16x3(int trans_a, int trans_b, int64_t M, int64_t N, int64_t K, const void* A_planes,
                      const void* B_planes, float* C, int64_t ldc, const float* bias, int relu,
                      const float* mask, int64_t ldmask, int products, void* workspace, void* stream);

#define GODE_ADAM_MAX_TENSORS 64
typedef struct gode_adam_args {
    float*       param[GODE_ADAM_MAX_TENSORS];
    const float* grad[GODE_ADAM_MAX_TENSORS];
    float*       exp_avg[GODE_ADAM_MAX_TENSORS];
    float*       exp_avg_sq[GODE_ADAM_MAX_TENSORS];
    int64_t      len[GODE_ADAM_MAX_TENSORS];
} gode_adam_args_t;
int64_t gode_adam_chunk(void);
int gode_adam_tick_f32(float* state, float beta1, float beta2, void* stream);
int gode_adam_f32(const gode_adam_args_t* args , int32_t n_tensors, const void* chunks, int64_t n_chunks,
                  const float* state, float lr, float beta1, float beta2, float eps, float weight_decay, void* stream);

int gode_reduce_parts_f32(float* out, const float* part, int64_t n_part, int64_t len,
                          float scale, int accumulate, void* stream);
int gode_reduce_parts2_f32(float* out_a, const float* part_a, float* out_b, const float* part_b,
                           int64_t n_part, int64_t len, float scale, int accumulate, void* stream);

int gode_colsum_f32(float* out, const float* X, int64_t n_rows, int64_t d, float scale,
                    int accumulate, float* scratch , void* stream);
int64_t gode_colsum_scratch_bytes(int64_t n_rows, int64_t d);

int64_t gode_gat_logits_scratch_bytes(int64_t n_edges);

typedef struct gode_graph {
    const int32_t* rowptr; const int32_t* col; const float* val;
    const int32_t* items;  int64_t n_items;
    const int32_t* long_rows; int64_t n_long; float* partial;
    int64_t n_rows; int64_t nnz;
} gode_graph_t;

typedef struct gode_gat_proj {
    const float* ps; int64_t ld_s;
    const float* pt; int64_t ld_t;
    const float* as; const float* at;
    int64_t ld_a;
} gode_gat_proj_t;
int gode_gat_logits_f32(const gode_gat_proj_t* proj, const float* bw, const int32_t* src, const int32_t* tgt,
                        int64_t n_edges, float* a, float* amax, float* scratch, void* stream);
int gode_gat_agg_f32_fwd(const gode_graph_t* mt, const int32_t* src, const int32_t* tgt,
                         const gode_gat_proj_t* proj, int64_t o, const float* bf, const float* a, const float* amax,
                         float eps, float* out, float* w_out, float* den_out, void* stream);
int gode_gat_agg_f32_bwd(const gode_graph_t* mt, const int32_t* src, const int32_t* tgt,
                         const gode_gat_proj_t* proj, int64_t o, const float* bf, const float* w, const float* den,
                         const float* out, const float* dout, const gode_lincomb_t* cot, float cot_scale,
                         float* dz, float* da, float* dpt, int64_t ld_dpt, float* dat, int64_t ld_dat,
                         int32_t* did_target_sums, void* stream);
int64_t gode_gat_maxpath_scratch_bytes(int64_t n_edges);
int gode_gat_maxpath_f32(const float* a, const float* amax, float* da, int64_t n_edges, const int32_t* tgt,
                         float* dat, int64_t ld_dat, void* scratch, void* stream);
int64_t gode_gat_heads_scratch_bytes(int64_t n_edges, int64_t heads);
int gode_gat_logits_heads_f32(const gode_gat_proj_t* proj, const float* bw ,
                              const int32_t* src, const int32_t* tgt, int64_t n_edges, int64_t heads, float* a,
                              float* hmax, void* scratch, void* stream);
int gode_gat_maxpath_heads_f32(const float* a, float* da, int64_t n_edges, int64_t heads, const int32_t* tgt,
                               float* dat, int64_t ld_dat, void* scratch, void* stream);
int64_t gode_gat_heads_parts(int64_t n_edges);
int gode_gat_logits_heads_raw_f32(const gode_gat_proj_t* proj, const float* bw, const int32_t* src, const int32_t* tgt,
                                  int64_t n_edges, int64_t heads, float* a, void* scratch, void* stream);
int gode_gat_agg_heads_f32_fwd(const gode_graph_t* mt, const int32_t* src, const int32_t* tgt, const gode_gat_proj_t* proj,
                               int64_t o, const float* bf, const float* a, const void* scratch, int64_t n_edges,
                               int64_t heads, float eps, float* out, float* w_out, float* den_out, void* stream);
int gode_gat_maxpath_heads_raw_f32(const float* a, float* da, int64_t n_edges, int64_t heads, const int32_t* tgt,
                                   float* dat, int64_t ld_dat, void* scratch, void* stream);
int gode_gat_maxpath_heads_part_f32(const float* a, const float* da, int64_t n_edges, int64_t heads, const int32_t* tgt,
                                    void* scratch, void* stream);
int64_t gode_gat_heads_block_cap(void);
int gode_gat_scatter_f32(const int32_t* rowptr_src, const int32_t* eid_src, const int32_t* rowptr_tgt,
                         const int32_t* eid_tgt, const float* dz, const float* da, int64_t o, int64_t n_rows,
                         float* dps, int64_t ld_s, float* dpt, int64_t ld_t, float* das, float* dat, int64_t ld_a,
                         void* stream);
int gode_time_row_fixup_f32(float* g_row0, const float* w_row0, int64_t len, float t, float* at, int accumulate,
                            void* stream);
int gode_time_row_fixup3_f32(float* g0, const float* w0, int64_t l0, float* g1, const float* w1, int64_t l1,
                             float* g2, const float* w2, int64_t l2, float t, float* at, void* stream);

int gode_edge_matvec_f32_fwd(const int32_t* rowptr, const int32_t* eid, const float* val,
                             const int32_t* src, const float* A, const float* X, int64_t ldx,
                             int64_t h, int64_t n_rows, float* out, int64_t ldo, void* stream);
int gode_edge_matvec_msg_f32(const int32_t* src, const float* A, const float* X, int64_t ldx, int64_t h,
                             int64_t n_edges, float* msg, void* stream);
int gode_edge_matvec_f32_bwd(const int32_t* edge_row, const float* edge_val, const int32_t* src,
                             const float* A, const float* X, int64_t ldx, const float* dM, int64_t ldm,
                             int64_t h, int64_t n_edges, float* dA, float* dxe, void* stream);
int gode_edge_outer_sum_f32(const int32_t* edge_row, const float* edge_val , const int32_t* src, int32_t n_terms,
                            const float* const* dM , const float* const* X , int64_t ldx, int64_t ldm,
                            int64_t h, int64_t n_edges, float* dA, void* stream);

int gode_segment_attention_f32_fwd(const int32_t* segptr, const int32_t* perm, const float* x, int64_t ldx,
                                   const float* q, int64_t n_seg, int64_t h, float* a, float* r, void* stream);
int gode_segment_attention_f32_bwd(const int32_t* segptr, const int32_t* perm, const float* x, int64_t ldx,
                                   const float* q, const float* a, const float* dr, int64_t n_seg, int64_t h,
                                   float* dx, float* dq, void* stream);
int gode_assign_csr_supported(int64_t n_entries, int64_t n_rows);
int gode_dense_first_nonzero_f32(const float* M, int64_t ld, int64_t n_rows, int64_t n_cols, int64_t* index, void* stream);
int gode_assign_csr_i32(const int64_t* index, int64_t n_entries, int64_t n_rows, int32_t* rowptr, int32_t* order,
                        const float* vals, float* vals_out, void* stream);

int gode_set2set_supported(int64_t H);
int gode_set2set_f32_fwd(const int32_t* segptr, const int32_t* perm, const float* x, int64_t ldx, const float* Wt,
                         const float* b_ih, const float* b_hh, int64_t n_graphs, int64_t H, int64_t steps, int64_t n_nodes,
                         float* qs, float* cs, float* gates, float* att, void* stream);
int gode_set2set_f32_bwd(const int32_t* segptr, const int32_t* perm, const float* x, int64_t ldx, const float* w_ih,
                         const float* w_hh, int64_t n_graphs, int64_t H, int64_t steps, int64_t n_nodes, const float* qs,
                         const float* cs, const float* gates, const float* att, const float* dq_final, float* dx,
                         float* DG, void* stream);


typedef struct gode_gcn_odefunc {
    gode_graph_t A, AT;
    int64_t n, d;
    int32_t groups; float eps;
    const float* W;
    const float* b; const float* gamma; const float* beta;
} gode_gcn_odefunc_t;

typedef struct gode_rk4_workspace {
    float* S; float* dZ; float* dS;
    float* S2;
    float* ky[4]; float* ka[4];
    float* ktheta[4];
    float* wpart;
    float* gpart; float* bpart;
    float* colsum_scratch;
    float* X[2];
    float* small_part;
    float* y2_colsum;
} gode_rk4_workspace_t;

int     gode_gcn_small_supported(int64_t n_rows, int64_t d, int32_t groups);
int64_t gode_gcn_small_parts(int64_t n_rows);
int64_t gode_gcn_small_part_len(int64_t d);
int gode_gcn_feval_small_f32(const gode_gcn_odefunc_t* f, const gode_lincomb_t* xin , float t, float alpha,
                             const gode_lincomb_t* pre , const gode_lincomb_t* cot ,
                             float* Y2 , float* out, void* stream);
int gode_gcn_feval_small_next_f32(const gode_gcn_odefunc_t* f, const gode_lincomb_t* xin , float t, float alpha,
                                  const gode_lincomb_t* pre , const gode_lincomb_t* cot ,
                                  float* Y2 , float* out, const gode_lincomb_t* next , float* x_next,
                                  void* stream);
int gode_gcn_vjp_small_f32(const gode_gcn_odefunc_t* f, const gode_lincomb_t* xin , const float* dZ,
                           float out_scale, const gode_lincomb_t* pre , float* ka, float* part,
                           void* stream);
int gode_gcn_vjp_small_next_f32(const gode_gcn_odefunc_t* f, const gode_lincomb_t* xin , const float* dZ,
                                float out_scale, const gode_lincomb_t* pre , float* ka, float* part,
                                const gode_lincomb_t* cot_next , const float* k_next, float* dZ_next,
                                void* stream);
int gode_gcn_feval_small_save_f32(const gode_gcn_odefunc_t* f, const gode_lincomb_t* xin , float t, float alpha,
                                  const gode_lincomb_t* pre , float* out, float* k, void* stream);
int gode_gcn_small_finish_f32(const gode_gcn_odefunc_t* f, const float* part, float* ktheta, float t, void* stream);
int gode_gcn_small_finish_multi_f32(const gode_gcn_odefunc_t* f, const float* part, int32_t n_stages,
                                    float* const* ktheta , const float* ts , void* stream);
int gode_gcn_small_finish4_f32(const gode_gcn_odefunc_t* f, const float* part, float* theta, const float* wb ,
                               const float* ts , void* stream);

int64_t gode_gcn_ode_theta_len(int64_t d);
int gode_gcn_ode_rk4_forward(const gode_gcn_odefunc_t* f, float* y, float** result,
                             const gode_rk4_workspace_t* ws, float t0, float t1, int32_t n_steps, void* stream);
int gode_gcn_ode_rk4_adjoint(const gode_gcn_odefunc_t* f, float* y, float* a, float* theta,
                             float** y_result, float** a_result,
                             const gode_rk4_workspace_t* ws, float t0, float t1, int32_t n_steps, void* stream);

int gode_gcn_ode_rk4_forward_save(const gode_gcn_odefunc_t* f, const float* y0, float* y_end, float* save,
                                  const gode_rk4_workspace_t* ws, float t0, float t1, int32_t n_steps,
                                  int32_t step_begin, int32_t step_end, void* stream);
int gode_gcn_ode_rk4_backprop(const gode_gcn_odefunc_t* f, const float* save, float* a, float* theta, float** a_result,
                              const gode_rk4_workspace_t* ws, float* cot_colpart , float t0, float t1,
                              int32_t n_steps, int32_t step_begin, int32_t step_end, void* stream);

int gode_gcn_ode_dopri5_step_forward(const gode_gcn_odefunc_t* f, const float* y, float* const* k , float* y1,
                                     const gode_rk4_workspace_t* ws, double t, double h, float rtol, float atol,
                                     double* sums, void* err_scratch, void* stream);
int gode_gcn_ode_dopri5_step_adjoint(const gode_gcn_odefunc_t* f, const float* y, const float* a, const float* theta,
                                     float* const* ky , float* const* ka , float* const* ktheta ,
                                     float* y1, float* a1, float* theta1, const gode_rk4_workspace_t* ws,
                                     double t, double h, float rtol, float atol, double* sums ,
                                     void* err_scratch, void* stream);

int gode_gcn_ode_dopri5_step_backprop(const gode_gcn_odefunc_t* f, const float* y, float* const* k ,
                                      const float* g, const float* kbar7 , double wy,
                                      const double* wk , double t, double h, int32_t first,
                                      float* const* ybar , float* ybar_n, float* kbar1, float* theta,
                                      float* const* ktheta , const gode_rk4_workspace_t* ws,
                                      float* cot_colpart , void* stream);

typedef struct gode_gat_odefunc {
    gode_graph_t mt;
    gode_graph_t ms_inc, mt_inc;
    const int32_t* src; const int32_t* tgt; int64_t n_edges;
    int64_t n, d; int32_t groups; float eps_gn; float eps;
    const float* Wsrc; const float* Wtgt; const float* Wlog;
    const float* bf; const float* bw; const float* gamma; const float* beta;
    int32_t heads;
    const float* Wpacked;
} gode_gat_odefunc_t;

typedef struct gode_gat_workspace {
    float* X; float* Ps; float* Pt; float* A2;
    float* a; float* amax; float* wgt; float* den;
    void* logits_scratch;
    float* dz; float* da;
    float* dPs; float* dPt; float* dA2; float* pair;
    float* gp; float* bp;
    float* wp[3];
    void* maxpath_scratch; void* colsum_scratch;
    const float* zeros; void* heads_scratch;
    void* colsum_scratch2;
    float* small_part;
} gode_gat_workspace_t;

int     gode_gat_small_supported(int64_t n_rows, int64_t d, int32_t groups, int64_t heads);
int64_t gode_gat_small_parts(int64_t n_rows, int64_t d);
int64_t gode_gat_small_part_len(int64_t d, int64_t heads);
int gode_gat_project_small_f32(const gode_lincomb_t* xin, int64_t n_rows, int64_t d, int32_t groups, float eps,
                               const float* gamma, const float* beta, const float* Wsrc, const float* Wtgt,
                               const float* Wlog, int64_t heads, const float* pt_bias, float t, float* Ps, float* Pt,
                               float* A2, float* x_out, const float* packed , void* stream);
int gode_gat_dense_vjp_small_f32(const gode_lincomb_t* xin, int64_t n_rows, int64_t d, int32_t groups, float eps,
                                 const float* gamma, const float* beta, const float* Wsrc, const float* Wtgt,
                                 const float* Wlog, int64_t heads, const float* dPs, const float* dPt, const float* dA2,
                                 float out_scale, const gode_lincomb_t* pre, float* ka, float* part,
                                 const void* maxpath_scratch , const int32_t* esrc, const int32_t* etgt, int64_t n_edges,
                                 const float* packed , void* stream);
int gode_gat_small_finish_f32(const float* part, int64_t n_rows, int64_t d, int64_t heads, float t, float* ktheta,
                              float* kat, void* stream);
int gode_gat_small_finish_step_f32(const float* part, int64_t n_rows, int64_t d, int64_t heads, int32_t n_slots,
                                   const float* ts , const float* w , float* theta, float* at,
                                   void* stream);
int64_t gode_gat_small_pack_len(int64_t d, int64_t heads);
int gode_gat_small_pack_f32(const float* Wsrc, const float* Wtgt, const float* Wlog, int64_t d, int64_t heads, float* packed,
                            void* stream);

int64_t gode_gat_ode_theta_len(int64_t d);
int64_t gode_gat_ode_theta_len_heads(int64_t d, int64_t heads);
int gode_gat_ode_dopri5_step_forward(const gode_gat_odefunc_t* f, const float* y, float* const* k , float* y1,
                                     const gode_gat_workspace_t* ws, double t, double h, float rtol, float atol,
                                     double* sums, void* err_scratch, void* stream);
int gode_gat_ode_dopri5_step_adjoint(const gode_gat_odefunc_t* f, const float* y, const float* a, const float* a_t,
                                     const float* theta, float* const* ky, float* const* ka, float* const* ka_t,
                                     float* const* ktheta, float* y1, float* a1, float* a_t1, float* theta1,
                                     const gode_gat_workspace_t* ws, double t, double h, float rtol, float atol,
                                     double* sums , void* err_scratch, void* stream);

int gode_lstm_cell_supported(int64_t B, int64_t I, int64_t H);
int gode_lstm_cell_f32_fwd(const float* x, const float* h, const float* c, const float* w_ih, const float* w_hh,
                           const float* b_ih, const float* b_hh, int64_t B, int64_t I, int64_t H, float* h_out,
                           float* c_out, float* gates, void* stream);
int gode_lstm_cell_f32_bwd(const float* x, const float* h, const float* c, const float* w_ih, const float* w_hh,
                           const float* gates, const float* c_out, const float* dh_out, const float* dc_out, int64_t B,
                           int64_t I, int64_t H, float* dx, float* dh, float* dc, float* dw_ih, float* dw_hh,
                           float* db_ih, float* db_hh, void* stream);
int64_t gode_gru_wgrad_parts(int64_t n);
int gode_gru_cell_f32_fwd(const float* x, const float* m, const float* w_ih, const float* w_hh, const float* b_ih,
                          const float* b_hh, int64_t n, int64_t h, float* out, float* gates, void* stream);
int gode_gru_cell_f32_bwd(const float* x, const float* m, const float* w_ih, const float* w_hh, const float* gates,
                          const float* dout, int64_t n, int64_t h, float* dx, float* dm, float* dgi, float* dgh,
                          float* part, float* dw_ih, float* dw_hh, float* db_ih, float* db_hh, void* stream);
int gode_gru_wreduce_f32(const float* part, int64_t n_part, int64_t h, float* dw_ih, float* dw_hh, float* db_ih,
                         float* db_hh, void* stream);

int gode_edge_ode_supported(int64_t h);
int gode_edge_ode_feval_f32(const int32_t* rowptr, const int32_t* eid, const float* val, const int32_t* src,
                            const float* A, const float* S, int64_t h, int64_t n_rows, const float* bias,
                            const gode_lincomb_t* pre , float alpha, float* out, void* stream);
int gode_edge_ode_vjp_f32(const int32_t* ms_rowptr, const int32_t* ms_eid, const int32_t* edge_row,
                          const float* edge_val, const float* A, const gode_lincomb_t* cot , float cot_scale,
                          const float* fout, int64_t h, int64_t n_rows, int64_t n_edges, float* dM, float* dS,
                          float* dxe, void* stream);
int gode_edge_outer_sum_acc_f32(const int32_t* edge_row, const float* edge_val, const int32_t* src, int32_t n_terms,
                                const float* const* dM , const float* const* X ,
                                const float* w , int64_t h, int64_t n_edges, int accumulate, float* dA,
                                void* stream);

#define GODE_PROF_SPMM     0
#define GODE_PROF_GEMM_FWD 1
#define GODE_PROF_GEMM_BWD 2
#define GODE_PROF_WGRAD    3
#define GODE_PROF_BWD_WGRAD 4
#define GODE_PROF_EDGE_FEVAL 5
#define GODE_PROF_EDGE_VJP   6
#define GODE_PROF_EDGE_OUTER_STEP  7
#define GODE_PROF_EDGE_OUTER_STAGE 8
#define GODE_PROF_FORM_FP32  (0 << 8)
#define GODE_PROF_FORM_SPLIT (1 << 8)
#define GODE_PROF_FORM_PC    (2 << 8)
void* gode_prof_create(int capacity);
void  gode_prof_destroy(void* prof);
void  gode_prof_enable(void* prof );
void  gode_prof_reset(void* prof);
int   gode_prof_count(void* prof);
int   gode_prof_read(void* prof, float* ms , int64_t* d ,
                     int64_t* rows , int64_t* extra , int max_n);
int   gode_prof_kinds(void* prof, int32_t* kinds , int max_n);

#ifdef __cplusplus
}
#endif
#endif
```

Before: 4.072 steps/s.

## Reduce split-row SpMM segments inside the block instead of a separate finish pass

```diff
diff --git a/graph_odenet_amd/_lib.py b/graph_odenet_amd/_lib.py
--- a/graph_odenet_amd/_lib.py
+++ b/graph_odenet_amd/_lib.py
@@ -25,7 +25,8 @@
     _fields_ = [("rowptr", ctypes.c_void_p), ("col", ctypes.c_void_p), ("val", ctypes.c_void_p),
                 ("items", ctypes.c_void_p), ("n_items", ctypes.c_int64),
                 ("long_rows", ctypes.c_void_p), ("n_long", ctypes.c_int64), ("partial", ctypes.c_void_p),
-                ("n_rows", ctypes.c_int64), ("nnz", ctypes.c_int64)]
+                ("n_rows", ctypes.c_int64), ("nnz", ctypes.c_int64),
+                ("n_close", ctypes.c_int64), ("long_far", ctypes.c_void_p), ("n_long_far", ctypes.c_int64)]
 
 
 class GcnOdeFunc(ctypes.Structure):
@@ -92,6 +93,8 @@
                                 c_i64, c_i64, ctypes.POINTER(SpmmEpilogue), c_p]),
     "gode_spmm_csr_save_f32": (c_i, [c_p, c_p, c_p, c_p, c_i64, c_p, c_i64, c_p, c_p, c_i64, c_p, c_i64,
                                      c_i64, c_i64, ctypes.POINTER(SpmmEpilogue), c_p, c_p]),
+    "gode_spmm_close_supported": (c_i, [c_i64, c_i64]),
+    "gode_spmm_graph_f32": (c_i, [ctypes.POINTER(Graph), c_p, c_i64, c_p, c_i64, c_i64, ctypes.POINTER(SpmmEpilogue), c_p, c_p]),
     "gode_masked_cot_parts": (c_i64, [c_i64, c_i64]),
     "gode_masked_cot_f32": (c_i, [ctypes.POINTER(LinComb), c_p, c_p, c_i64, c_i64, c_p, c_p]),
     "gode_lincomb_f32": (c_i, [c_p, ctypes.POINTER(LinComb), c_i64, c_p]),
@@ -255,6 +258,7 @@
     "gode_prof_enable": (None, [c_p]),
     "gode_prof_reset": (None, [c_p]),
     "gode_prof_count": (c_i, [c_p]),
+    "gode_prof_finish_launches": (c_i, [c_p]),
     "gode_prof_read": (c_i, [c_p, c_p, c_p, c_p, c_p, c_i]),
     "gode_prof_kinds": (c_i, [c_p, c_p, c_i]),
 }
diff --git a/graph_odenet_amd/csrc/api.hip b/graph_odenet_amd/csrc/api.hip
--- a/graph_odenet_amd/csrc/api.hip
+++ b/graph_odenet_amd/csrc/api.hip
@@ -22,7 +22,7 @@
 
 namespace {
 int env_int(const char* name, int dflt) { const char* e = getenv(name); return e ? atoi(e) : dflt; }
-int g_gemm_split = -1, g_overlap = -1, g_wgrad_split = -1, g_wgrad_split_small = 0, g_bwd_pc = -1, g_fwd_pc = -1, g_small_fused = -1, g_bwd_wgrad = -1, g_y2_colsum = -1, g_rk_close_once = -1;
+int g_gemm_split = -1, g_overlap = -1, g_wgrad_split = -1, g_wgrad_split_small = 0, g_bwd_pc = -1, g_fwd_pc = -1, g_small_fused = -1, g_bwd_wgrad = -1, g_y2_colsum = -1, g_rk_close_once = -1, g_spmm_close_in_block = -1;
 }
 
 int gode_opt_gemm_split() { if (g_gemm_split < 0) { const int v = env_int("GODE_GEMM_SPLIT", 2); g_gemm_split = (v == 1 || v == 2) ? v : 0; } return g_gemm_split; }
@@ -37,6 +37,7 @@
 int gode_opt_bwd_wgrad() { if (g_bwd_wgrad < 0) g_bwd_wgrad = env_int("GODE_BWD_WGRAD", 1) != 0; return g_bwd_wgrad; }
 int gode_opt_y2_colsum() { if (g_y2_colsum < 0) g_y2_colsum = env_int("GODE_Y2_COLSUM", 1) != 0; return g_y2_colsum; }
 int gode_opt_rk_close_once() { if (g_rk_close_once < 0) g_rk_close_once = env_int("GODE_RK_CLOSE_ONCE", 1) != 0; return g_rk_close_once; }
+int gode_opt_spmm_close_in_block() { if (g_spmm_close_in_block < 0) g_spmm_close_in_block = env_int("GODE_SPMM_CLOSE_IN_BLOCK", 1) != 0; return g_spmm_close_in_block; }
 int gode_opt_overlap() { if (g_overlap < 0) g_overlap = env_int("GODE_OVERLAP", 1) != 0; return g_overlap; }
 
 extern "C" int gode_set_option(const char* name, int value) {
@@ -49,6 +50,7 @@
     if (!strcmp(name, "bwd_wgrad")) { g_bwd_wgrad = value != 0; return 0; }
     if (!strcmp(name, "y2_colsum")) { g_y2_colsum = value != 0; return 0; }
     if (!strcmp(name, "rk_close_once")) { g_rk_close_once = value != 0; return 0; }
+    if (!strcmp(name, "spmm_close_in_block")) { g_spmm_close_in_block = value != 0; return 0; }
     if (!strcmp(name, "fwd_pc")) { if (value < 0 || value > 3) return GODE_E_UNSUPPORTED; g_fwd_pc = value; return 0; }
     if (!strcmp(name, "wgrad_split")) { if (value != 0 && value != 6 && value != 8) return GODE_E_UNSUPPORTED; g_wgrad_split = value; return 0; }
     return GODE_E_UNSUPPORTED;
@@ -64,6 +66,7 @@
     if (!strcmp(name, "bwd_wgrad")) return gode_opt_bwd_wgrad();
     if (!strcmp(name, "y2_colsum")) return gode_opt_y2_colsum();
     if (!strcmp(name, "rk_close_once")) return gode_opt_rk_close_once();
+    if (!strcmp(name, "spmm_close_in_block")) return gode_opt_spmm_close_in_block();
     if (!strcmp(name, "fwd_pc")) return gode_opt_fwd_pc();
     return GODE_E_UNSUPPORTED;
 }
diff --git a/graph_odenet_amd/csrc/ode_driver.hip b/graph_odenet_amd/csrc/ode_driver.hip
--- a/graph_odenet_amd/csrc/ode_driver.hip
+++ b/graph_odenet_amd/csrc/ode_driver.hip
@@ -7,8 +7,7 @@
 namespace {
 
 int spmm(const gode_graph_t& g, const float* X, float* Y, int64_t d, const gode_spmm_epilogue_t* ep, void* s) {
-    return gode_spmm_csr_f32(g.rowptr, g.col, g.val, g.items, g.n_items, g.long_rows, g.n_long, g.partial,
-                             X, d, Y, d, g.n_rows, d, ep, s);
+    return gode_spmm_graph_f32(&g, X, d, Y, d, d, ep, nullptr, s);
 }
 gode_spmm_epilogue_t relu_bias_epilogue(const gode_gcn_odefunc_t* f) {
     gode_spmm_epilogue_t ep = {};
@@ -98,9 +97,7 @@
     gode_spmm_epilogue_t ep = relu_bias_epilogue(f);
     if (close) { ep.pre = p_formed ? one_term(out) : close->pre; ep.alpha = close->alpha; }
     if (!k_save) return spmm(f->A, S, out, d, &ep, stream);
-    const gode_graph_t& g = f->A;
-    return gode_spmm_csr_save_f32(g.rowptr, g.col, g.val, g.items, g.n_items, g.long_rows, g.n_long, g.partial,
-                                  S, d, out, d, g.n_rows, d, &ep, k_save, stream);
+    return gode_spmm_graph_f32(&f->A, S, d, out, d, d, &ep, k_save, stream);
 }
 
 int rk4_forward_step(const gode_gcn_odefunc_t* f, const gode_rk4_workspace_t* ws, const float* y, float* const* k,
@@ -230,7 +227,7 @@
     const int total = 4 * n_steps;
     const bool bw = !small && gode_bwd_wgrad_supported(n, d, d, f->groups) && gode_bwd_wgrad_parts(n) <= wparts;
     const int64_t y2rows = (bw && ws->y2_colsum && gode_opt_y2_colsum())
-        ? gode_spmm_y2_colsum_rows(f->A.items ? f->A.n_items : f->A.n_rows, f->A.items ? f->A.n_long : 0, d) : 0;
+        ? gode_spmm_y2_colsum_rows(f->A.items ? f->A.n_items - f->A.n_close : f->A.n_rows, f->A.items ? f->A.n_long : 0, d) : 0;
 
     const bool mat = ws->X[0] != nullptr && ws->X[1] != nullptr;
     auto x_out_of = [&](int g) -> float* { return (mat && (g % 4) >= 2) ? ws->X[g & 1] : nullptr; };
diff --git a/graph_odenet_amd/csrc/options.h b/graph_odenet_amd/csrc/options.h
--- a/graph_odenet_amd/csrc/options.h
+++ b/graph_odenet_amd/csrc/options.h
@@ -8,4 +8,5 @@
 int gode_opt_small_fused();
 int gode_opt_bwd_wgrad();
 int gode_opt_y2_colsum();
+int gode_opt_spmm_close_in_block();
 int gode_opt_rk_close_once();
diff --git a/graph_odenet_amd/csrc/prof.h b/graph_odenet_amd/csrc/prof.h
--- a/graph_odenet_amd/csrc/prof.h
+++ b/graph_odenet_amd/csrc/prof.h
@@ -3,3 +3,4 @@
 #include <stdint.h>
 int  gode_prof_begin(hipStream_t s, int64_t d, int64_t rows, int64_t extra, int kind = 0);
 void gode_prof_end(hipStream_t s, int slot);
+void gode_prof_note_finish();
diff --git a/graph_odenet_amd/csrc/prof.hip b/graph_odenet_amd/csrc/prof.hip
--- a/graph_odenet_amd/csrc/prof.hip
+++ b/graph_odenet_amd/csrc/prof.hip
@@ -8,6 +8,7 @@
     std::vector<hipEvent_t> ev;
     std::vector<int64_t> d, rows, extra;
     std::vector<int32_t> kind;
+    int finish_launches;
 };
 
 static GodeProf* volatile g_prof = nullptr;
@@ -15,7 +16,7 @@
 extern "C" void* gode_prof_create(int capacity) {
     if (capacity <= 0) return nullptr;
     GodeProf* p = new GodeProf();
-    p->capacity = capacity; p->count = 0;
+    p->capacity = capacity; p->count = 0; p->finish_launches = 0;
     p->ev.resize(2 * (size_t)capacity); p->d.resize(capacity); p->rows.resize(capacity); p->extra.resize(capacity); p->kind.resize(capacity);
     for (auto& e : p->ev) if (hipEventCreate(&e) != hipSuccess) { delete p; return nullptr; }
     return p;
@@ -28,7 +29,8 @@
     delete p;
 }
 extern "C" void gode_prof_enable(void* prof) { g_prof = (GodeProf*)prof; }
-extern "C" void gode_prof_reset(void* prof) { if (prof) ((GodeProf*)prof)->count = 0; }
+extern "C" void gode_prof_reset(void* prof) { if (prof) { ((GodeProf*)prof)->count = 0; ((GodeProf*)prof)->finish_launches = 0; } }
+extern "C" int gode_prof_finish_launches(void* prof) { return prof ? ((GodeProf*)prof)->finish_launches : 0; }
 extern "C" int gode_prof_count(void* prof) { return prof ? ((GodeProf*)prof)->count : 0; }
 
 extern "C" int gode_prof_read(void* prof, float* ms, int64_t* d, int64_t* rows, int64_t* extra, int max_n) {
@@ -71,3 +73,7 @@
     (void)hipEventRecord(p->ev[2 * slot + 1], s);
     p->count = slot + 1;
 }
+void gode_prof_note_finish() {
+    GodeProf* p = g_prof;
+    if (p) ++p->finish_launches;
+}
diff --git a/graph_odenet_amd/csrc/spmm.hip b/graph_odenet_amd/csrc/spmm.hip
--- a/graph_odenet_amd/csrc/spmm.hip
+++ b/graph_odenet_amd/csrc/spmm.hip
@@ -72,10 +72,11 @@
 template <int LPR, bool OUT3 = false>
 __global__ __launch_bounds__(256) void spmm_vec4_kernel(
     const int* __restrict__ rowptr, const int* __restrict__ col, const float* __restrict__ val,
-    const int4* __restrict__ items, int n_items, float* __restrict__ partial,
+    const int4* __restrict__ items, int n_items, int close_blocks, float* __restrict__ partial,
     const float* __restrict__ X, int64_t ldx, float* __restrict__ Y, int64_t ldy, Epilogue ep)
 {
     constexpr int U = 4;
+    constexpr int RPB = 256 / LPR;
     const int64_t tid = (int64_t)blockIdx.x * blockDim.x + threadIdx.x;
     const int gid = (int)(tid / LPR);
     const int lane = threadIdx.x & (LPR - 1);
@@ -117,18 +118,36 @@
             }
         }
     }
-    if (ep.colpart) {
-        float4 g = make_float4(0.f, 0.f, 0.f, 0.f);
-        if (active) {
-            if (slot < 0) g = epilogue_store4<LPR, OUT3>(ep, acc, row, lane, (int64_t)LPR * 4, Y, ldy);
-            else *reinterpret_cast<float4*>(partial + (int64_t)slot * (LPR * 4) + lane * 4) = acc;
-        }
-        block_colsum_store<LPR>(g, ep.colpart + (int64_t)blockIdx.x * (LPR * 4));
-        return;
-    }
-    if (!active) return;
-    if (slot < 0) epilogue_store4<LPR, OUT3>(ep, acc, row, lane, (int64_t)LPR * 4, Y, ldy);
-    else *reinterpret_cast<float4*>(partial + (int64_t)slot * (LPR * 4) + lane * 4) = acc;
+    const bool closing = (int)blockIdx.x < close_blocks;
+    bool emit = active && slot > -2;
+    if (closing) {
+        __shared__ float4 stage[256];
+        stage[threadIdx.x] = acc;
+        __syncthreads();
+        constexpr int NMAX = RPB < 8 ? RPB : 8;
+        const int c = -2 - slot, g0 = threadIdx.x / LPR;
+        int n = (slot <= -2 && (c & 15) == 0) ? (c >> 4) : 0;
+        if (n > RPB - g0) n = RPB - g0;
+        if (n > NMAX) n = NMAX;
+        if (n > 0) {
+            float4 t = make_float4(0.f, 0.f, 0.f, 0.f);
+#pragma unroll
+            for (int k = 0; k < NMAX; ++k) {
+                const int gk = g0 + k < RPB ? g0 + k : RPB - 1;
+                const float4 p = stage[gk * LPR + lane];
+                t.x += k < n ? p.x : 0.f; t.y += k < n ? p.y : 0.f; t.z += k < n ? p.z : 0.f; t.w += k < n ? p.w : 0.f;
+            }
+            acc = t;
+            emit = active;
+        }
+    }
+    float4 g = make_float4(0.f, 0.f, 0.f, 0.f);
+    if (emit) {
+        if (slot < 0) g = epilogue_store4<LPR, OUT3>(ep, acc, row, lane, (int64_t)LPR * 4, Y, ldy);
+        else *reinterpret_cast<float4*>(partial + (int64_t)slot * (LPR * 4) + lane * 4) = acc;
+    }
+    if (ep.colpart && !closing)
+        block_colsum_store<LPR>(g, ep.colpart + (int64_t)((int)blockIdx.x - close_blocks) * (LPR * 4));
 }
 
 template <int LPR, bool OUT3 = false>
@@ -193,29 +212,39 @@
     const bool active = gid < n_long;
     if (!active && !ep.colpart) return;
     const int4 lr = active ? long_rows[gid] : make_int4(0, 0, 0, 0);
+    const bool closed = lr.w != 0;
     float4 acc = make_float4(0.f, 0.f, 0.f, 0.f);
+    const float* pl = partial + lane * 4;
     int s = lr.y;
-    for (; s + 3 < lr.z; s += 4) {
-        const float4 p0 = *reinterpret_cast<const float4*>(partial + (int64_t)s * (LPR * 4) + lane * 4);
-        const float4 p1 = *reinterpret_cast<const float4*>(partial + (int64_t)(s + 1) * (LPR * 4) + lane * 4);
-        const float4 p2 = *reinterpret_cast<const float4*>(partial + (int64_t)(s + 2) * (LPR * 4) + lane * 4);
-        const float4 p3 = *reinterpret_cast<const float4*>(partial + (int64_t)(s + 3) * (LPR * 4) + lane * 4);
-        acc.x += p0.x; acc.y += p0.y; acc.z += p0.z; acc.w += p0.w;
-        acc.x += p1.x; acc.y += p1.y; acc.z += p1.z; acc.w += p1.w;
-        acc.x += p2.x; acc.y += p2.y; acc.z += p2.z; acc.w += p2.w;
-        acc.x += p3.x; acc.y += p3.y; acc.z += p3.z; acc.w += p3.w;
-    }
-    for (; s < lr.z; ++s) {
-        const float4 p = *reinterpret_cast<const float4*>(partial + (int64_t)s * (LPR * 4) + lane * 4);
+    const int s1 = closed ? s : lr.z;
+    for (; s + 15 < s1; s += 16) {
+        float4 p[16];
+#pragma unroll
+        for (int u = 0; u < 16; ++u) p[u] = *reinterpret_cast<const float4*>(pl + (int64_t)(s + u) * (LPR * 4));
+#pragma unroll
+        for (int u = 0; u < 16; ++u) { acc.x += p[u].x; acc.y += p[u].y; acc.z += p[u].z; acc.w += p[u].w; }
+    }
+    for (; s + 3 < s1; s += 4) {
+        float4 p[4];
+#pragma unroll
+        for (int u = 0; u < 4; ++u) p[u] = *reinterpret_cast<const float4*>(pl + (int64_t)(s + u) * (LPR * 4));
+#pragma unroll
+        for (int u = 0; u < 4; ++u) { acc.x += p[u].x; acc.y += p[u].y; acc.z += p[u].z; acc.w += p[u].w; }
+    }
+    for (; s < s1; ++s) {
+        const float4 p = *reinterpret_cast<const float4*>(pl + (int64_t)s * (LPR * 4));
         acc.x += p.x; acc.y += p.y; acc.z += p.z; acc.w += p.w;
     }
     if (ep.colpart) {
         float4 g = make_float4(0.f, 0.f, 0.f, 0.f);
-        if (active) g = epilogue_store4<LPR, OUT3>(ep, acc, lr.x, lane, (int64_t)LPR * 4, Y, ldy);
+        if (active) {
+            if (closed) g = *reinterpret_cast<const float4*>(ep.Y2 + (int64_t)lr.x * (LPR * 4) + lane * 4);
+            else g = epilogue_store4<LPR, OUT3>(ep, acc, lr.x, lane, (int64_t)LPR * 4, Y, ldy);
+        }
         block_colsum_store<LPR>(g, ep.colpart + (ep.colpart_row0 + blockIdx.x) * (LPR * 4));
         return;
     }
-    epilogue_store4<LPR, OUT3>(ep, acc, lr.x, lane, (int64_t)LPR * 4, Y, ldy);
+    if (!closed) epilogue_store4<LPR, OUT3>(ep, acc, lr.x, lane, (int64_t)LPR * 4, Y, ldy);
 }
 
 __device__ __forceinline__ void epilogue_store1(const Epilogue& ep, float z, int row, int c, int64_t d,
@@ -308,12 +337,15 @@
     }
 }
 
+struct CloseList { int n_close; const int4* long_far; int n_long_far; };
+
 template <int LPR, bool OUT3>
 int launch_vec4(const int* rowptr, const int* col, const float* val, const int4* items, int n_items,
-                const int4* long_rows, int n_long, float* partial, const float* X, int64_t ldx,
+                const int4* long_rows, int n_long, const CloseList& cl, float* partial, const float* X, int64_t ldx,
                 float* Y, int64_t ldy, const Epilogue& ep, hipStream_t s) {
+    const int n_rec = n_items - cl.n_close;
     if (LPR < 64 && n_items > 0 && n_items <= 65536) {
-        if (ep.colpart) return GODE_E_UNSUPPORTED;
+        if (ep.colpart || cl.n_close > 0) return GODE_E_UNSUPPORTED;
         const int64_t wb = ((int64_t)n_items * 64 + 255) / 256;
         const int slot = gode_prof_begin(s, (int64_t)LPR * 4, n_items, (int64_t)ep.pre.n + ep.cot.n + (ep.Y2 ? 1 : 0) + (ep.Y3 ? 1 : 0));
         hipLaunchKernelGGL((spmm_vec4_wave_kernel<LPR, OUT3>), dim3((unsigned)wb), dim3(256), 0, s,
@@ -322,6 +354,7 @@
         GODE_LAUNCH_CHECK();
         if (n_long > 0) {
             const int64_t b2 = ((int64_t)n_long * LPR + 255) / 256;
+            gode_prof_note_finish();
             hipLaunchKernelGGL((spmm_finish_vec4_kernel<LPR, OUT3>), dim3((unsigned)b2), dim3(256), 0, s,
                                long_rows, n_long, partial, Y, ldy, ep);
             GODE_LAUNCH_CHECK();
@@ -331,18 +364,22 @@
     const int64_t threads = (int64_t)n_items * LPR;
     const int64_t blocks = (threads + 255) / 256;
     if (blocks > 0) {
-        const int slot = gode_prof_begin(s, (int64_t)LPR * 4, n_items, (int64_t)ep.pre.n + ep.cot.n + (ep.Y2 ? 1 : 0) + (ep.Y3 ? 1 : 0));
+        const int slot = gode_prof_begin(s, (int64_t)LPR * 4, n_rec, (int64_t)ep.pre.n + ep.cot.n + (ep.Y2 ? 1 : 0) + (ep.Y3 ? 1 : 0));
         hipLaunchKernelGGL((spmm_vec4_kernel<LPR, OUT3>), dim3((unsigned)blocks), dim3(256), 0, s,
-                           rowptr, col, val, items, n_items, partial, X, ldx, Y, ldy, ep);
+                           rowptr, col, val, items, n_items, (int)((int64_t)cl.n_close * LPR / 256), partial, X, ldx, Y, ldy, ep);
         gode_prof_end(s, slot);
         GODE_LAUNCH_CHECK();
     }
-    if (n_long > 0) {
-        const int64_t b2 = ((int64_t)n_long * LPR + 255) / 256;
+    const bool far_only = cl.n_close > 0 && !ep.colpart;
+    const int4* lr = far_only ? cl.long_far : long_rows;
+    const int nl = far_only ? cl.n_long_far : n_long;
+    if (nl > 0) {
+        const int64_t b2 = ((int64_t)nl * LPR + 255) / 256;
         Epilogue ep2 = ep;
-        ep2.colpart_row0 = blocks;
+        ep2.colpart_row0 = blocks - (int64_t)cl.n_close * LPR / 256;
+        gode_prof_note_finish();
         hipLaunchKernelGGL((spmm_finish_vec4_kernel<LPR, OUT3>), dim3((unsigned)b2), dim3(256), 0, s,
-                           long_rows, n_long, partial, Y, ldy, ep2);
+                           lr, nl, partial, Y, ldy, ep2);
         GODE_LAUNCH_CHECK();
     }
     return 0;
@@ -359,6 +396,13 @@
     return (n_items * lpr + 255) / 256 + (n_long * lpr + 255) / 256;
 }
 
+extern "C" int gode_spmm_close_supported(int64_t n_items, int64_t d)
+{
+    if (n_items <= 65536 || d <= 0 || d % 4) return 0;
+    const int64_t lpr = d / 4;
+    return lpr <= 32 && !(lpr & (lpr - 1));
+}
+
 namespace {
 
 int spmm_csr_impl(const int32_t* rowptr, const int32_t* col, const float* val,
@@ -366,13 +410,20 @@
                   const int32_t* long_rows, int64_t n_long, float* partial,
                   const float* X, int64_t ldx, float* Y, int64_t ldy,
                   int64_t n_rows, int64_t d,
-                  const gode_spmm_epilogue_t* epi, float* K, void* stream)
+                  const gode_spmm_epilogue_t* epi, float* K, void* stream,
+                  int64_t n_close = 0, const int32_t* long_far = nullptr, int64_t n_long_far = 0)
 {
     if (n_rows < 0 || d <= 0 || ldx < d || ldy < d) return GODE_E_SHAPE;
     if (n_rows == 0) return 0;
     if (!rowptr || !col || !X || !Y) return GODE_E_NULLPTR;
     if (n_rows > INT32_MAX || d > (1 << 20)) return GODE_E_RANGE;
-    if (!items) { n_items = n_rows; n_long = 0; }
+    if (!items) { n_items = n_rows; n_long = 0; n_close = 0; }
+    if (n_close < 0 || n_long_far < 0 || n_long_far > n_long) return GODE_E_RANGE;
+    if (n_close > 0) {
+        if (n_close % 256 || n_close >= n_items) return GODE_E_RANGE;
+        if (!gode_spmm_close_supported(n_items - n_close, d)) return GODE_E_UNSUPPORTED;
+        if (n_long_far > 0 && (!long_far || !partial)) return GODE_E_NULLPTR;
+    }
     if (n_items < 0 || n_items > INT32_MAX || n_long < 0 || n_long > INT32_MAX) return GODE_E_RANGE;
     if (n_long > 0 && (!long_rows || !partial)) return GODE_E_NULLPTR;
     if (n_items * 64 >= ((int64_t)1 << 32)) return GODE_E_RANGE;
@@ -395,7 +446,7 @@
         if (ep.Y3 == Y || ep.Y3 == Y2 || ep.Y3 == K) return GODE_E_RANGE;
         for (int j = 0; j < ep.cot.n; ++j) if (ep.Y3 == ep.cot.ptr[j]) return GODE_E_RANGE;
     }
-    if (ep.colpart && ((((uintptr_t)ep.colpart) & 15) || gode_spmm_y2_colsum_rows(n_items, n_long, d) == 0)) return GODE_E_UNSUPPORTED;
+    if (ep.colpart && ((((uintptr_t)ep.colpart) & 15) || gode_spmm_y2_colsum_rows(n_items - n_close, n_long, d) == 0)) return GODE_E_UNSUPPORTED;
 
     const bool al = !(((uintptr_t)X) & 15) && !(((uintptr_t)Y) & 15) && (ldx % 4 == 0) && (ldy % 4 == 0) &&
                     (!bias || !(((uintptr_t)bias) & 15)) && (!partial || !(((uintptr_t)partial) & 15)) &&
@@ -403,10 +454,12 @@
                     !(((uintptr_t)K) & 15) && !(((uintptr_t)ep.Y3) & 15);
     const int4* it4 = reinterpret_cast<const int4*>(items);
     const int4* lr4 = reinterpret_cast<const int4*>(long_rows);
+    const CloseList cl = { (int)n_close, reinterpret_cast<const int4*>(long_far), (int)n_long_far };
+    if (n_close > 0 && !al) return GODE_E_ALIGN;
     if (al && d % 4 == 0) {
         switch (d / 4) {
-#define GODE_CASE(L) case L: return ep.Y3 ? launch_vec4<L, true>(rowptr, col, val, it4, (int)n_items, lr4, (int)n_long, partial, X, ldx, Y, ldy, ep, s) \
-                                        : launch_vec4<L, false>(rowptr, col, val, it4, (int)n_items, lr4, (int)n_long, partial, X, ldx, Y, ldy, ep, s);
+#define GODE_CASE(L) case L: return ep.Y3 ? launch_vec4<L, true>(rowptr, col, val, it4, (int)n_items, lr4, (int)n_long, cl, partial, X, ldx, Y, ldy, ep, s) \
+                                        : launch_vec4<L, false>(rowptr, col, val, it4, (int)n_items, lr4, (int)n_long, cl, partial, X, ldx, Y, ldy, ep, s);
             GODE_CASE(1) GODE_CASE(2) GODE_CASE(4) GODE_CASE(8) GODE_CASE(16) GODE_CASE(32) GODE_CASE(64)
 #undef GODE_CASE
             default: break;
@@ -429,6 +482,7 @@
     }
     if (n_long > 0) {
         const int64_t b2 = ((int64_t)n_long * G + 255) / 256;
+        gode_prof_note_finish();
         hipLaunchKernelGGL(spmm_finish_generic_kernel, dim3((unsigned)b2), dim3(256), 0, s,
                            lr4, (int)n_long, partial, Y, ldy, (int)d, G, ep);
         GODE_LAUNCH_CHECK();
@@ -461,3 +515,11 @@
     return spmm_csr_impl(rowptr, col, val, items, n_items, long_rows, n_long, partial, X, ldx, Y, ldy, n_rows, d, epi,
                          K, stream);
 }
+
+extern "C" int gode_spmm_graph_f32(const gode_graph_t* g, const float* X, int64_t ldx, float* Y, int64_t ldy, int64_t d,
+                                   const gode_spmm_epilogue_t* epi, float* K, void* stream)
+{
+    if (!g) return GODE_E_NULLPTR;
+    return spmm_csr_impl(g->rowptr, g->col, g->val, g->items, g->n_items, g->long_rows, g->n_long, g->partial, X, ldx, Y, ldy,
+                         g->n_rows, d, epi, K, stream, g->n_close, g->long_far, g->n_long_far);
+}
diff --git a/graph_odenet_amd/gcn_ode.py b/graph_odenet_amd/gcn_ode.py
--- a/graph_odenet_amd/gcn_ode.py
+++ b/graph_odenet_amd/gcn_ode.py
@@ -8,16 +8,7 @@
 
 
 def _graph_struct(g, d):
-    gs = _lib.Graph()
-    gs.rowptr, gs.col = g.rowptr.data_ptr(), g.col.data_ptr()
-    gs.val = g.val.data_ptr() if g.val is not None else None
-    gs.items, gs.n_items = (g.items.data_ptr() if g.items is not None else None), g.n_items
-    gs.long_rows = g.long_rows.data_ptr() if g.long_rows is not None else None
-    gs.n_long = g.n_long
-    part = g.partial(d)
-    gs.partial = part.data_ptr() if part is not None else None
-    gs.n_rows, gs.nnz = g.n_rows, g.nnz
-    return gs
+    return ops.graph_struct(g, d)
 
 
 class _Shared:
diff --git a/graph_odenet_amd/graph.py b/graph_odenet_amd/graph.py
--- a/graph_odenet_amd/graph.py
+++ b/graph_odenet_amd/graph.py
@@ -1,3 +1,4 @@
+import collections
 import weakref
 
 import torch
@@ -7,6 +8,50 @@
 
 def auto_split(nnz):
     return 256 if nnz >= (1 << 20) else 1024
+
+
+CLOSE_GROUP = 8
+CLOSE_ALIGN = 256
+CLOSE_PAD = (0, 0, 0, -3)
+
+CloseList = collections.namedtuple("CloseList", "items n_items n_close long_rows long_far n_long_far")
+
+
+def close_records(rowptr, items, long_rows, split):
+    dev = items.device
+    rp = rowptr.to(torch.int64)
+    deg = rp[1:] - rp[:-1]
+    nseg = torch.clamp((deg + split - 1) // split, min=1)
+    closable = (nseg >= 2) & (nseg <= CLOSE_GROUP)
+    rows_c = torch.nonzero(closable).flatten()
+    if rows_c.numel() == 0:
+        return None
+    start = torch.zeros_like(nseg)
+    groups = 0
+    for n in range(CLOSE_GROUP, 1, -1):
+        idx = torch.nonzero(nseg == n).flatten()
+        m = int(idx.numel())
+        if m == 0:
+            continue
+        per = CLOSE_GROUP // n
+        j = torch.arange(m, device=dev, dtype=torch.int64)
+        start[idx] = (groups + j // per) * CLOSE_GROUP + (j % per) * n
+        groups += (m + per - 1) // per
+    n_close = -(-groups * CLOSE_GROUP // CLOSE_ALIGN) * CLOSE_ALIGN
+    pad = torch.tensor(CLOSE_PAD, dtype=torch.int64, device=dev)
+    head = pad.repeat(n_close, 1)
+    ns = nseg[rows_c]
+    rr = torch.repeat_interleave(rows_c, ns)
+    k = torch.arange(rr.numel(), device=dev, dtype=torch.int64) - torch.repeat_interleave(torch.cumsum(ns, 0) - ns, ns)
+    begin = rp[rr] + k * split
+    end = torch.minimum(begin + split, rp[rr + 1])
+    head[start[rr] + k] = torch.stack([rr, begin, end, -2 - (k + 16 * nseg[rr])], 1)
+    tail = items.clone()
+    tail[closable[tail[:, 0]] & (tail[:, 3] >= 0)] = pad
+    lr = long_rows.clone()
+    lr[:, 3] = closable[lr[:, 0]].to(torch.int64)
+    far = lr[lr[:, 3] == 0]
+    return CloseList(torch.cat([head, tail], 0), n_close + int(items.shape[0]), n_close, lr, far, int(far.shape[0]))
 
 
 class CSRGraph:
@@ -26,6 +71,19 @@
             self.items, self.n_items, self.long_rows, self.n_long, self.n_slots = None, self.n_rows, None, 0, 0
         self._partial = {}
         self._T = None
+        self._close = False
+
+    def close_list(self):
+        if self._close is False:
+            cl = None
+            if self.items is not None and self.n_long > 0:
+                cl = close_records(self.rowptr, self.items.to(torch.int64), self.long_rows.to(torch.int64), self.split)
+            if cl is not None:
+                i32 = lambda t: t.to(torch.int32).contiguous()
+                cl = cl._replace(items=i32(cl.items), long_rows=i32(cl.long_rows),
+                                 long_far=i32(cl.long_far) if cl.n_long_far else None)
+            self._close = cl
+        return self._close
 
     def _build_items(self):
         dev = self.device
diff --git a/graph_odenet_amd/ops.py b/graph_odenet_amd/ops.py
--- a/graph_odenet_amd/ops.py
+++ b/graph_odenet_amd/ops.py
@@ -26,6 +26,38 @@
         elif t.numel() != n:
             raise ValueError("graph_odenet_amd: %s terms differ in size" % name)
     return n
+
+
+def close_list(graph, d):
+    if getattr(graph, "items", None) is None or graph.n_long == 0:
+        return None
+    lib = _lib.load()
+    if not lib.gode_spmm_close_supported(graph.n_items, int(d)) or not lib.gode_get_option(b"spmm_close_in_block"):
+        return None
+    return graph.close_list()
+
+
+def graph_struct(graph, d, close=True):
+    gs = _lib.Graph()
+    gs.rowptr, gs.col = graph.rowptr.data_ptr(), graph.col.data_ptr()
+    gs.val = graph.val.data_ptr() if graph.val is not None else None
+    cl = close_list(graph, d) if close else None
+    if cl is not None:
+        gs.items, gs.n_items, gs.n_close = cl.items.data_ptr(), cl.n_items, cl.n_close
+        gs.long_rows, gs.n_long = cl.long_rows.data_ptr(), graph.n_long
+        gs.long_far, gs.n_long_far = (cl.long_far.data_ptr() if cl.long_far is not None else None), cl.n_long_far
+    else:
+        gs.items, gs.n_items = (graph.items.data_ptr() if graph.items is not None else None), graph.n_items
+        gs.long_rows = graph.long_rows.data_ptr() if graph.long_rows is not None else None
+        gs.n_long = graph.n_long
+    part = graph.partial(d)
+    gs.partial = part.data_ptr() if part is not None else None
+    gs.n_rows, gs.nnz = graph.n_rows, graph.nnz
+    return gs
+
+
+def _aligned16(ldy, *tensors):
+    return ldy % 4 == 0 and all(t is None or t.data_ptr() % 16 == 0 for t in tensors)
 
 
 def spmm(graph, X, bias=None, relu=False, out=None, cot_terms=None, out2=None, pre_terms=None, alpha=1.0, out2_colsum=None,
@@ -86,6 +118,12 @@
                     ep.cot_out_coef[j] = float(cj)
         elif cot_out is not None:
             raise ValueError("spmm: cot_out needs cot_terms")
+    if close_list(graph, d) is not None and _aligned16(
+            ldy, X, out, bias, out2, out2_colsum, cot_out, *[t for _, t in (pre_terms or [])], *[t for _, t in (cot_terms or [])]):
+        gs = graph_struct(graph, d)
+        check(lib.gode_spmm_graph_f32(ctypes.byref(gs), ptr(X), d, ptr(out), ldy, d,
+                                      ctypes.byref(ep) if ep is not None else None, None, stream_ptr()), "gode_spmm_graph_f32")
+        return (out, out2) if cot_terms is not None else out
     partial = graph.partial(d)
     rc = lib.gode_spmm_csr_f32(ptr(graph.rowptr), ptr(graph.col), ptr(graph.val),
                                ptr(graph.items), graph.n_items,
diff --git a/include/graphode.h b/include/graphode.h
--- a/include/graphode.h
+++ b/include/graphode.h
@@ -41,6 +41,7 @@
 } gode_spmm_epilogue_t;
 
 int64_t gode_spmm_y2_colsum_rows(int64_t n_items, int64_t n_long, int64_t d);
+int     gode_spmm_close_supported(int64_t n_items, int64_t d);
 
 int gode_spmm_csr_f32(const int32_t* rowptr, const int32_t* col, const float* val,
                       const int32_t* items, int64_t n_items,
@@ -184,7 +185,12 @@
     const int32_t* items;  int64_t n_items;
     const int32_t* long_rows; int64_t n_long; float* partial;
     int64_t n_rows; int64_t nnz;
+    int64_t n_close;
+    const int32_t* long_far; int64_t n_long_far;
 } gode_graph_t;
+
+int gode_spmm_graph_f32(const gode_graph_t* g, const float* X, int64_t ldx, float* Y, int64_t ldy, int64_t d,
+                        const gode_spmm_epilogue_t* epi , float* K , void* stream);
 
 typedef struct gode_gat_proj {
     const float* ps; int64_t ld_s;
@@ -444,6 +450,7 @@
 void  gode_prof_enable(void* prof );
 void  gode_prof_reset(void* prof);
 int   gode_prof_count(void* prof);
+int   gode_prof_finish_launches(void* prof);
 int   gode_prof_read(void* prof, float* ms , int64_t* d ,
                      int64_t* rows , int64_t* extra , int max_n);
 int   gode_prof_kinds(void* prof, int32_t* kinds , int max_n);
```

After: 4.110 steps/s, median of 5. Within noise of the previous version (+0.9%).
